# joyfang1106/MRLA

Hardware: AMD Instinct MI355X
Metric: images/sec fwd+bwd resnet50_mrlal b=256 (higher is better)
Workload: dtype bf16

## Files before the change

### include/mrla_hip.h

```cpp
#ifndef MRLA_HIP_H_
#define MRLA_HIP_H_

#include <stddef.h>
#include <stdint.h>

#ifdef __cplusplus
extern "C" {
#endif

#define MRLA_OK 0
#define MRLA_EINVAL (-1)
#define MRLA_EUNSUPPORTED (-2)
#define MRLA_EHIP (-3)

enum { MRLA_F32 = 0, MRLA_BF16 = 1, MRLA_F16 = 2 };
enum { MRLA_NCHW = 0, MRLA_NHWC = 1 };
enum { MRLA_ACT_NONE = 0, MRLA_ACT_GELU = 1 };
enum { MRLA_BN_NONE = 0, MRLA_BN_TRAIN = 1, MRLA_BN_EVAL = 2 };

#define MRLA_FWD_MOMENTS 8
#define MRLA_BWD_MOMENTS 3
#define MRLA_GEMM_MOMENTS 4

#define MRLA_ABI_VERSION 5
int mrla_abi_version(void);

int mrla_light_wgrad_rows(int b, int c, int h, int w, int dtype, int layout);

int mrla_light_mom_splits(int b, int c, int h, int w, int dtype, int layout);
int mrla_tuning_row_ranges(int mode);
int mrla_light_stats_fwd(const void* x, const void* o_prev, const float* wv , float* mom,
                         int b, int c, int h, int w, int dtype, int layout, int act, void* stream);

int mrla_light_stats_fwd_fused(const void* pre, const float* pre_sc, const float* pre_sh, const void* o_prev,
                               const float* wv, float* mom, void* x_out, int b, int c, int h, int w, int dtype,
                               int layout, void* stream);

int mrla_light_pool_fused(const void* pre, const float* pre_sc, const float* pre_sh, const void* o_prev, float* part,
                          float* mom, int b, int c, int h, int w, int dtype, int layout, void* stream);
int mrla_light_apply_fwd_fused(const void* pre, const float* pre_sc, const float* pre_sh, const void* o_prev,
                               const float* wv, const float* gate, const float* sc, const float* sh, const float* lam,
                               const float* dp, void* out, int b, int c, int h, int w, int d, int res, int dtype,
                               int layout, void* stream);

int mrla_light_gate_fwd(const float* mom, const float* wq, const float* wk, int ksize, float* gate ,
                        int b, int c, int hw, int d, void* stream);

int mrla_light_bn_fwd(const float* mom, const float* gate, const float* lam, const float* gamma, const float* beta,
                      float* running_mean, float* running_var, int bn_mode, float momentum, float eps, float* sc,
                      float* sh, float* save_mean, float* save_inv, int b, int c, int hw, int d, void* stream);

int mrla_light_apply_fwd(const void* x, const void* o_prev, const float* wv, const float* gate, const float* sc,
                         const float* sh, const float* lam, const float* dp, void* out, int b, int c, int h, int w,
                         int d, int res, int dtype, int layout, int act, void* stream);

int mrla_light_bmom_splits(int b, int c, int h, int w, int dtype, int layout);
int mrla_light_stats_bwd(const void* dout, const void* x, const void* o_prev, const float* wv, const float* mom,
                         float* bmom, int b, int c, int h, int w, int dtype, int layout, int act, void* stream);

int mrla_light_bn_bwd(const float* mom, const float* bmom, const float* gate, const float* lam, const float* gamma,
                      const float* dp, const float* save_mean, const float* save_inv, int bn_mode, float* cb,
                      float* cb_lo, float* dgamma, float* dbeta, float* dlam, int b, int c, int hw, int d,
                      void* stream);

int mrla_light_gate_bwd(const float* mom, const float* bmom, const float* gate, const float* cb, const float* cb_lo,
                        const float* dp,
                        const float* wq, const float* wk, int ksize, float* dyx, float* dwqk_part, int b, int c,
                        int hw, int d, void* stream);

int mrla_light_apply_bwd_pre_sums(int b, int c, int h, int w, int dtype, int layout);
int mrla_light_apply_bwd(const void* dout, const void* x, const void* o_prev, const float* wv, const float* gate,
                         const float* cb, const float* lam, const float* dp, const float* dyx, void* dx,
                         void* do_prev, float* dwv_part, const void* pre, const float* pre_center, float* pre_tmom, int b,
                         int c, int h, int w, int d, int res, int relu_mask, int dtype, int layout, int act, void* stream);

int mrla_light_lean_supported(int b, int c, int h, int w, int dtype, int layout);
int mrla_light_stats_bwd_fused(const void* dout, const void* pre, const float* pre_sc, const float* pre_sh,
                               const void* o_prev, const float* wv, const float* mom, float* bmom, int b, int c, int h, int w,
                               int dtype, int layout, void* stream);
int mrla_light_apply_bwd_fused(const void* dout, const void* pre, const float* pre_sc, const float* pre_sh,
                               const void* o_prev, const float* wv, const float* gate, const float* cb, const float* lam,
                               const float* dp, const float* dyx, void* dx, void* do_prev, float* dwv_part,
                               const float* pre_center, float* pre_tmom, int b, int c, int h, int w, int d, int res,
                               int dtype, int layout, void* stream);


int mrla_base_gate_fwd(const float* mom, const float* wq, const float* wk, int ksize, float* k_ring, float* p_all,
                       float* q , int b, int c, int hw, int d, int T, int t, void* stream);

int mrla_base_attend_fwd(const void* x, const float* wv, void* v_ring, const float* p_all, void* attn, float* amom,
                         int b, int c, int h, int w, int d, int T, int t, int dtype, int layout, void* stream);

int mrla_bn_stats_fwd(const float* amom, const float* pivot, const float* gamma, const float* beta, float* running_mean,
                      float* running_var, int bn_mode, float momentum, float eps, float* sc, float* sh,
                      float* save_mean, float* save_inv, int b, int c, int hw, void* stream);

int mrla_bn_stats_fwd_rows(const float* rec, const float* gamma, const float* beta, float* running_mean, float* running_var,
                           int bn_mode, float momentum, float eps, float* sc, float* sh, float* save_mean, float* save_inv,
                           int rows, int c, void* stream);

int mrla_base_tail_fwd(const void* x, const void* attn, const float* sc, const float* sh, const float* dp, void* out,
                       int b, int c, int h, int w, int dtype, int layout, void* stream);

int mrla_base_tail_stats_bwd(const void* dout, const void* attn, const float* sc, const float* sh, const float* center,
                             const float* dp, float* tmom, int b, int c, int h, int w, int dtype, int layout, void* stream);

int mrla_bn_stats_bwd(const float* tmom, const float* gamma, const float* save_mean, const float* save_inv,
                      int bn_mode, int centered, float* cb, float* dgamma, float* dbeta, int b, int c, int hw, void* stream);

int mrla_base_attend_bwd(const void* dout, const void* attn, const float* sc, const float* sh, const float* dp,
                         const float* cb, const void* v_ring, void* da_ring, float* pmom, int b, int c, int h, int w,
                         int T, int t, int dtype, int layout, void* stream);

int mrla_base_gate_bwd(const float* mom, const float* pmom, const float* p_all, const float* q, const float* k_ring,
                       float* dk_ring, const float* wq, const float* wk, int ksize, float* dyx, float* dwqk_part,
                       int b, int c, int hw, int d, int T, int t, int first_touch, void* stream);

int mrla_base_value_bwd(const void* dout, const void* x, const float* wv, const void* da_ring, const float* p_all,
                        const float* dyx, void* dx, float* dwv_part, int b, int c, int h, int w, int d, int T, int t,
                        int Tc, int res, int dtype, int layout, void* stream);

int mrla_base_tile_rows(int b, int c, int h, int w, int dtype, int layout);
int mrla_base_pmom_rows(int b, int c, int h, int w, int dtype, int layout);

int mrla_base_pool_value_fwd(const void* x, const float* pre_sc, const float* pre_sh, const void* identity,
                             const float* wv, float* mom, void* x_out, void* v_slot, int b, int c, int h, int w,
                             int dtype, int layout, void* stream);

int mrla_base_pmom_reduce(const float* part, float* pmom, int b, int c, int t, int rows, void* stream);

int mrla_base_dv_combine(const void* da_ring, const float* p_all, void* dv, int b, int c, int h, int w, int d, int T,
                         int t, int Tc, int dtype, int layout, void* stream);

int mrla_base_value_bwd_pre_sums(int b, int c, int h, int w, int dtype, int layout);
int mrla_base_value_bwd_dv(const void* dout, const void* x, const float* wv, const void* dv, const float* dyx, void* dx,
                           float* dwv_part, const void* pre, const float* pre_center, float* pre_tmom, int b, int c, int h,
                           int w, int res, int dtype, int layout, void* stream);

#define MRLA_TOKEN_PARTIALS 15

int mrla_token_norm_pool(const void* x, const void* o_prev, const float* lnx_w, const float* lnx_b, float eps,
                         float* stats, float* mom, int b, int n, int c, int dtype, void* stream);

int mrla_token_apply_fwd(const void* x, const void* o_prev, const float* stats, const float* lnx_w,
                         const float* lnx_b, const float* lno_w, const float* lno_b, const float* wv,
                         const float* gate, const float* lam, void* out, int b, int n, int c, int d, int res,
                         int dtype, void* stream);

int mrla_token_part_rows(int b, int n, int c, int dtype);
int mrla_token_apply_bwd(const void* dout, const void* x, const void* o_prev, const float* stats, const float* lnx_w,
                         const float* lnx_b, const float* lno_w, const float* lno_b, const float* wv,
                         const float* gate, const float* lam, float* dxn, float* part, float* bmom, int b, int n, int c,
                         int d, int dtype, void* stream);
int mrla_token_gate_bwd(const float* mom, const float* bmom, const float* gate, const float* wq, const float* wk,
                        int ksize, float* dyx, float* dwqk_part, float* part, int b, int n, int c, int d, int dtype,
                        void* stream);
int mrla_token_ln_bwd(const void* dout, const void* x, const void* o_prev, const float* dxn, const float* dyx,
                      const float* stats, const float* lnx_w, const float* lno_w, const float* lam, void* dx,
                      void* do_prev, int b, int n, int c, int res, int dtype, void* stream);

int mrla_token_base_supported(int b, int n, int c, int dtype);
int mrla_token_base_value_fwd(const void* x, const float* stats, const float* lnx_w, const float* lnx_b, const float* wv,
                              void* v_slot, int b, int n, int c, int dtype, void* stream);
int mrla_token_base_attend_fwd(const void* v_ring, const float* p_all, const void* x, const float* stats,
                               const float* lnx_w, const float* lnx_b, void* out, float* amom, int b, int n, int c, int d,
                               int T, int t, int dtype, void* stream);
int mrla_token_base_attend_bwd(const void* dout, const void* v_ring, void* da_ring, float* pmom_part, int b, int n, int c,
                               int T, int t, int dtype, void* stream);
int mrla_token_base_gate_bwd(const float* mom, const float* pmom, const float* p_all, const float* q, const float* k_ring,
                             float* dk_ring, const float* wq, const float* wk, int ksize, float* dyx, float* dwqk_part,
                             float* part, int b, int n, int c, int d, int T, int t, int first_touch, int dtype,
                             void* stream);
int mrla_token_base_value_bwd(const void* dout, const void* x, const float* stats, const float* lnx_w, const float* lnx_b,
                              const float* wv, const void* dv, float* dxn, float* part, int b, int n, int c, int dtype,
                              void* stream);

int mrla_bn_moment_rows(int b, int c, int h, int w, int layout);
int mrla_bn_plane_moments(const void* x, float* amom , float* pivot, int b, int c, int h, int w,
                          int dtype, int layout, void* stream);
int mrla_bn_act_fwd(const void* x, const float* sc, const float* sh, int relu, void* y, int b, int c, int h, int w,
                    int dtype, int layout, void* stream);
int mrla_bn_plane_dmoments(const void* dy, const void* x, const float* sc, const float* sh, const float* center, int relu,
                           float* tmom , int b, int c, int h, int w, int dtype,
                           int layout, void* stream);
int mrla_bn_act_bwd(const void* dy, const void* x, const float* sc, const float* sh, const float* cb , int relu,
                    void* dx, int b, int c, int h, int w, int dtype, int layout, void* stream);

int mrla_bn_pool_rows(int b, int c, int h, int w, int dtype, int layout);
int mrla_bn_relu_pool_fwd(const void* x, const float* sc, const float* sh, void* out, int b, int c, int h, int w, int dtype,
                          int layout, void* stream);
int mrla_bn_relu_pool_dmoments(const void* dp, const void* x, const float* sc, const float* sh, const float* center ,
                               float* tmom, int b, int c, int h, int w, int dtype, int layout, void* stream);
int mrla_bn_relu_pool_bwd(const void* dp, const void* x, const float* sc, const float* sh, const float* cb ,
                          void* dx, int b, int c, int h, int w, int dtype, int layout, void* stream);

int mrla_conv1x1_rows(int m, int k, int n, int dtype);
int mrla_conv1x1_plan(int m, int k, int n, int dtype, int addend, int* out);
int mrla_conv1x1_fwd(const void* x, const void* w, void* y, float* mom_part, int m, int k, int n, int dtype, void* stream);

int mrla_conv1x1_add_supported(int m, int k, int n, int dtype);
int mrla_conv1x1_fwd_add(const void* x, const void* w, const void* addend, void* y, int m, int k, int n, int dtype,
                         void* stream);

int mrla_conv1x1_addend_supported(int m, int k, int n, int sh, int sw, int dtype);
int mrla_conv1x1_fwd_addend(const void* x, const void* w, const void* addend, void* y, int m, int k, int n, int b, int h,
                            int w_, int sh, int sw, int dtype, void* stream);

int mrla_conv1x1_wgrad_rows(int m, int k, int n, int dtype);
int mrla_conv1x1_wgrad_plan(int m, int k, int n, int dtype, int* out);
int mrla_conv1x1_wgrad(const void* dy, const void* x, float* part, void* dw, int m, int k, int n, int dtype, int dw_dtype,
                       void* stream);

int mrla_weight_bank_refresh(const void* table, int entries, int max_tiles, void* stream);
int mrla_weight_bank_refresh_dt(const void* table, int entries, int max_tiles, int dtype, void* stream);

int mrla_reduce_rows(const float* in, float* out, int rows, int n, void* stream);
int mrla_reduce_rows2(const float* in1, float* out1, int rows1, int n1, const float* in2, float* out2, int rows2, int n2,
                      void* stream);



int mrla_light_tail_fwd(const void* x, const float* pre_sc, const float* pre_sh, const void* o_prev, const float* wq,
                        const float* wk, int ksize, const float* wv, const float* lam, const float* gamma,
                        const float* beta, float* running_mean, float* running_var, int bn_mode, float momentum, float eps,
                        const float* dp, float* mom, void* x_out, float* gate, float* bnbuf, void* out, int b, int c,
                        int h, int w, int d, int res, int fuse, int dtype, int layout, int act, void* stream);

int mrla_light_tail_bwd(const void* dout, const void* x, const void* o_prev, const float* wq, const float* wk, int ksize,
                        const float* wv, const float* lam, const float* gamma, const float* dp, const float* mom,
                        const float* gate, const float* bnbuf, int bn_mode, float* bmom, float* small, float* dyx,
                        float* dwqk_part, float* dwv_part, int rows, void* dx, void* do_prev, const void* pre,
                        const float* pre_sc, const float* pre_sh, const float* pre_center, float* pre_tmom, float* wsum,
                        int b, int c, int h, int w, int d, int res, int relu_mask, int dtype, int layout, int act,
                        void* stream);

int mrla_bn_fwd(const void* x, const float* records, int rec_rows, float* amom, float* pivot, int rows, const float* gamma,
                const float* beta, float* running_mean, float* running_var, int bn_mode, float momentum, float eps,
                float* bnbuf, int relu, void* y, int b, int c, int h, int w, int dtype, int layout, void* stream);

int mrla_bn_bwd(const void* dy, const void* x, const float* gamma, const float* bnbuf, float* tmom, int rows, int have_tmom,
                int bn_mode, int relu, float* small, void* dx, int b, int c, int h, int w, int dtype, int layout,
                void* stream);

int mrla_stem_fwd(const void* x, float* amom, float* pivot, int rows, const float* gamma, const float* beta,
                  float* running_mean, float* running_var, int bn_mode, float momentum, float eps, float* bnbuf, void* out,
                  int b, int c, int h, int w, int dtype, int layout, void* stream);
int mrla_stem_bwd(const void* dp, const void* x, const float* gamma, const float* bnbuf, float* tmom, int rows, int bn_mode,
                  float* small, void* dx, int b, int c, int h, int w, int dtype, int layout, void* stream);

int mrla_base_layer_fwd(const void* x, const float* pre_sc, const float* pre_sh, const void* identity, const float* wq,
                        const float* wk, int ksize, const float* wv, const float* gamma, const float* beta,
                        float* running_mean, float* running_var, int bn_mode, float momentum, float eps, const float* dp,
                        float* mom, void* x_out, void* v_ring, float* k_ring, float* p_all, float* q, void* attn,
                        float* amom, int arows, float* bnbuf, void* out, int tail, int b, int c, int h, int w, int d, int T,
                        int t, int dtype, void* stream);

int mrla_base_layer_bwd(const void* dout, const void* x, const void* attn, const float* wq, const float* wk, int ksize,
                        const float* wv, const float* gamma, const float* dp, const float* mom, const float* q,
                        const float* bnbuf, int bn_mode, const void* v_ring, void* da_ring, const float* k_ring,
                        float* dk_ring, const float* p_all, float* tmom, int trows, float* small, float* ppart, int prows,
                        float* pmom, float* dyx, float* dwqk_part, void* dv, float* dwv_part, int rows, void* dx,
                        const void* pre, const float* pre_center, float* pre_tmom, float* wsum, int tail, int first_touch,
                        int res, int b, int c, int h, int w, int d, int T, int t, int Tc, int dtype, void* stream);

int mrla_token_light_fwd(const void* x, const void* o_prev, const float* lnx_w, const float* lnx_b, const float* lno_w,
                         const float* lno_b, const float* wq, const float* wk, int ksize, const float* wv,
                         const float* lam, float eps, float* stats, float* mom, float* gate, void* out, int b, int n, int c,
                         int d, int res, int dtype, void* stream);

int mrla_token_light_bwd(const void* dout, const void* x, const void* o_prev, const float* stats, const float* lnx_w,
                         const float* lnx_b, const float* lno_w, const float* lno_b, const float* wq, const float* wk,
                         int ksize, const float* wv, const float* gate, const float* lam, const float* mom, float* dxn,
                         float* part, int prow, float* bmom, float* dyx, float* dwqk_part, void* dx, void* do_prev,
                         float* sums, int b, int n, int c, int d, int res, int dtype, void* stream);

#ifdef __cplusplus
}
#endif
#endif
```

### mrla_amd/_lib.py

```python
import ctypes
import os

_HERE = os.path.dirname(os.path.abspath(__file__))
LIB_PATH = os.environ.get("MRLA_HIP_LIB") or os.path.join(_HERE, "libmrla_hip.so")

ABI_VERSION = 5
OK, EINVAL, EUNSUPPORTED, EHIP = 0, -1, -2, -3
F32, BF16, F16 = 0, 1, 2
NCHW, NHWC = 0, 1
ACT_NONE, ACT_GELU = 0, 1
BN_NONE, BN_TRAIN, BN_EVAL = 0, 1, 2
FWD_MOMENTS, BWD_MOMENTS, TOKEN_PARTIALS, GEMM_MOMENTS = 8, 3, 15, 4

_ERR = {EINVAL: "invalid argument", EUNSUPPORTED: "unsupported shape/layout for the HIP kernels",
        EHIP: "HIP runtime error at kernel launch"}

_P, _I, _F = ctypes.c_void_p, ctypes.c_int, ctypes.c_float

SIGNATURES = {
    "mrla_abi_version": [],
    "mrla_light_wgrad_rows": [_I] * 6,
    "mrla_light_stats_fwd": [_P, _P, _P, _P, _I, _I, _I, _I, _I, _I, _I, _P],
    "mrla_light_gate_fwd": [_P, _P, _P, _I, _P, _I, _I, _I, _I, _P],
    "mrla_light_bn_fwd": [_P, _P, _P, _P, _P, _P, _P, _I, _F, _F, _P, _P, _P, _P, _I, _I, _I, _I, _P],
    "mrla_light_apply_fwd": [_P, _P, _P, _P, _P, _P, _P, _P, _P, _I, _I, _I, _I, _I, _I, _I, _I, _I, _P],
    "mrla_light_stats_bwd": [_P, _P, _P, _P, _P, _P, _I, _I, _I, _I, _I, _I, _I, _P],
    "mrla_light_bmom_splits": [_I] * 6,
    "mrla_light_mom_splits": [_I] * 6,
    "mrla_tuning_row_ranges": [_I],
    "mrla_light_bn_bwd": [_P, _P, _P, _P, _P, _P, _P, _P, _I, _P, _P, _P, _P, _P, _I, _I, _I, _I, _P],
    "mrla_light_gate_bwd": [_P, _P, _P, _P, _P, _P, _P, _P, _I, _P, _P, _I, _I, _I, _I, _P],
    "mrla_light_apply_bwd_pre_sums": [_I] * 6,
    "mrla_light_apply_bwd": [_P] * 15 + [_I] * 10 + [_P],
    "mrla_light_lean_supported": [_I] * 6,
    "mrla_light_stats_bwd_fused": [_P] * 8 + [_I] * 6 + [_P],
    "mrla_light_apply_bwd_fused": [_P] * 16 + [_I] * 8 + [_P],
    "mrla_light_pool_fused": [_P] * 6 + [_I] * 6 + [_P],
    "mrla_light_apply_fwd_fused": [_P] * 11 + [_I] * 8 + [_P],
    "mrla_light_stats_fwd_fused": [_P, _P, _P, _P, _P, _P, _P, _I, _I, _I, _I, _I, _I, _P],
    "mrla_base_tile_rows": [_I] * 6,
    "mrla_base_pmom_rows": [_I] * 6,
    "mrla_base_pool_value_fwd": [_P] * 8 + [_I] * 6 + [_P],
    "mrla_base_pmom_reduce": [_P, _P, _I, _I, _I, _I, _P],
    "mrla_base_dv_combine": [_P, _P, _P] + [_I] * 10 + [_P],
    "mrla_base_value_bwd_pre_sums": [_I] * 6,
    "mrla_base_value_bwd_dv": [_P] * 10 + [_I] * 7 + [_P],
    "mrla_base_gate_fwd": [_P, _P, _P, _I, _P, _P, _P, _I, _I, _I, _I, _I, _I, _P],
    "mrla_base_attend_fwd": [_P, _P, _P, _P, _P, _P] + [_I] * 9 + [_P],
    "mrla_bn_stats_fwd": [_P, _P, _P, _P, _P, _P, _I, _F, _F, _P, _P, _P, _P, _I, _I, _I, _P],
    "mrla_bn_stats_fwd_rows": [_P, _P, _P, _P, _P, _I, _F, _F, _P, _P, _P, _P, _I, _I, _P],
    "mrla_base_tail_fwd": [_P, _P, _P, _P, _P, _P, _I, _I, _I, _I, _I, _I, _P],
    "mrla_base_tail_stats_bwd": [_P, _P, _P, _P, _P, _P, _P, _I, _I, _I, _I, _I, _I, _P],
    "mrla_bn_stats_bwd": [_P, _P, _P, _P, _I, _I, _P, _P, _P, _I, _I, _I, _P],
    "mrla_base_attend_bwd": [_P] * 9 + [_I] * 8 + [_P],
    "mrla_base_gate_bwd": [_P, _P, _P, _P, _P, _P, _P, _P, _I, _P, _P] + [_I] * 7 + [_P],
    "mrla_base_value_bwd": [_P] * 8 + [_I] * 11 + [_P],
    "mrla_token_norm_pool": [_P, _P, _P, _P, _F, _P, _P, _I, _I, _I, _I, _P],
    "mrla_token_apply_fwd": [_P] * 11 + [_I] * 6 + [_P],
    "mrla_token_part_rows": [_I] * 4,
    "mrla_token_apply_bwd": [_P] * 14 + [_I] * 5 + [_P],
    "mrla_token_gate_bwd": [_P] * 5 + [_I] + [_P] * 3 + [_I] * 5 + [_P],
    "mrla_token_ln_bwd": [_P] * 11 + [_I] * 5 + [_P],
    "mrla_token_base_supported": [_I] * 4,
    "mrla_token_base_value_fwd": [_P] * 6 + [_I] * 4 + [_P],
    "mrla_token_base_attend_fwd": [_P] * 8 + [_I] * 7 + [_P],
    "mrla_token_base_attend_bwd": [_P] * 4 + [_I] * 6 + [_P],
    "mrla_token_base_gate_bwd": [_P] * 8 + [_I] + [_P] * 3 + [_I] * 8 + [_P],
    "mrla_token_base_value_bwd": [_P] * 9 + [_I] * 4 + [_P],
    "mrla_bn_moment_rows": [_I] * 5,
    "mrla_bn_plane_moments": [_P, _P, _P, _I, _I, _I, _I, _I, _I, _P],
    "mrla_bn_act_fwd": [_P, _P, _P, _I, _P, _I, _I, _I, _I, _I, _I, _P],
    "mrla_bn_plane_dmoments": [_P, _P, _P, _P, _P, _I, _P, _I, _I, _I, _I, _I, _I, _P],
    "mrla_bn_act_bwd": [_P, _P, _P, _P, _P, _I, _P, _I, _I, _I, _I, _I, _I, _P],
    "mrla_bn_pool_rows": [_I] * 6,
    "mrla_bn_relu_pool_fwd": [_P, _P, _P, _P, _I, _I, _I, _I, _I, _I, _P],
    "mrla_bn_relu_pool_dmoments": [_P, _P, _P, _P, _P, _P, _I, _I, _I, _I, _I, _I, _P],
    "mrla_bn_relu_pool_bwd": [_P, _P, _P, _P, _P, _P, _I, _I, _I, _I, _I, _I, _P],
    "mrla_conv1x1_rows": [_I] * 4,
    "mrla_conv1x1_plan": [_I, _I, _I, _I, _I, _P],
    "mrla_conv1x1_wgrad_plan": [_I, _I, _I, _I, _P],
    "mrla_conv1x1_fwd": [_P, _P, _P, _P, _I, _I, _I, _I, _P],
    "mrla_conv1x1_add_supported": [_I] * 4,
    "mrla_conv1x1_fwd_add": [_P, _P, _P, _P, _I, _I, _I, _I, _P],
    "mrla_conv1x1_addend_supported": [_I] * 6,
    "mrla_conv1x1_fwd_addend": [_P, _P, _P, _P] + [_I] * 9 + [_P],
    "mrla_conv1x1_wgrad_rows": [_I] * 4,
    "mrla_conv1x1_wgrad": [_P, _P, _P, _P, _I, _I, _I, _I, _I, _P],
    "mrla_weight_bank_refresh": [_P, _I, _I, _P],
    "mrla_weight_bank_refresh_dt": [_P, _I, _I, _I, _P],
    "mrla_reduce_rows": [_P, _P, _I, _I, _P],
    "mrla_reduce_rows2": [_P, _P, _I, _I, _P, _P, _I, _I, _P],
    "mrla_light_tail_fwd": [_P] * 6 + [_I] + [_P] * 6 + [_I, _F, _F] + [_P] * 6 + [_I] * 10 + [_P],
    "mrla_light_tail_bwd": [_P] * 5 + [_I] + [_P] * 7 + [_I] + [_P] * 5 + [_I] + [_P] * 8 + [_I] * 10 + [_P],
    "mrla_bn_fwd": [_P, _P, _I, _P, _P, _I, _P, _P, _P, _P, _I, _F, _F, _P, _I, _P] + [_I] * 6 + [_P],
    "mrla_bn_bwd": [_P] * 5 + [_I] * 4 + [_P, _P] + [_I] * 6 + [_P],
    "mrla_stem_fwd": [_P, _P, _P, _I, _P, _P, _P, _P, _I, _F, _F, _P, _P] + [_I] * 6 + [_P],
    "mrla_stem_bwd": [_P] * 5 + [_I, _I, _P, _P] + [_I] * 6 + [_P],
    "mrla_base_layer_fwd": [_P] * 6 + [_I] + [_P] * 5 + [_I, _F, _F] + [_P] * 9 + [_I] + [_P, _P] + [_I] * 9 + [_P],
    "mrla_base_layer_bwd": ([_P] * 5 + [_I] + [_P] * 6 + [_I] + [_P] * 6 + [_I] + [_P, _P] + [_I] + [_P] * 5 + [_I] + [_P] * 5
                            + [_I] * 12 + [_P]),
    "mrla_token_light_fwd": [_P] * 8 + [_I] + [_P, _P] + [_F] + [_P] * 4 + [_I] * 6 + [_P],
    "mrla_token_light_bwd": [_P] * 10 + [_I] + [_P] * 6 + [_I] + [_P] * 6 + [_I] * 6 + [_P],
}


class MrlaHipError(RuntimeError):
    pass


_lib = None


def load():
    global _lib
    if _lib is not None:
        return _lib
    if not os.path.exists(LIB_PATH):
        raise MrlaHipError(
            f"{LIB_PATH} not found: the MRLA HIP extension is not built. Run `python -c 'import __graft_entry__ as g; "
            "g.build()'` (or `make -C mrla_amd/csrc`) -- mrla_amd has no CPU/PyTorch fallback for its operators.")
    import torch
    lib = ctypes.CDLL(LIB_PATH)
    for name, argtypes in SIGNATURES.items():
        fn = getattr(lib, name)
        fn.argtypes = argtypes
        fn.restype = ctypes.c_int
    if lib.mrla_abi_version() != ABI_VERSION:
        raise MrlaHipError(f"libmrla_hip.so reports ABI version {lib.mrla_abi_version()}, this binding is written against "
                           f"{ABI_VERSION} (MRLA_ABI_VERSION of include/mrla_hip.h); rebuild it")
    _lib = lib
    return lib


def check(rc, what):
    if rc != OK:
        raise MrlaHipError(f"{what}: {_ERR.get(rc, 'error')} (code {rc})")


def conv1x1_plan(m, k, n, addend=False, dtype=None):
    out = (ctypes.c_int * 4)()
    rc = load().mrla_conv1x1_plan(m, k, n, BF16 if dtype is None else dtype, int(addend), ctypes.cast(out, ctypes.c_void_p))
    return tuple(out) if rc == OK else None


def conv1x1_wgrad_plan(m, k, n, dtype=None):
    out = (ctypes.c_int * 6)()
    rc = load().mrla_conv1x1_wgrad_plan(m, k, n, BF16 if dtype is None else dtype, ctypes.cast(out, ctypes.c_void_p))
    return tuple(out) if rc == OK else None


def call(name, *args):
    rc = getattr(load(), name)(*args)
    check(rc, name)
```

### mrla_amd/csrc/bnact_nhwc.hip

```cpp
#include <algorithm>

#include "mrla_device.h"
#include "mrla_kernels.h"

#ifndef MRLA_REVERSE_AFFINE
#define MRLA_REVERSE_AFFINE 1
#endif

namespace mrla {

template <typename T> struct V16 { typedef T type __attribute__((ext_vector_type(16 / sizeof(T)))); };

template <typename T>
__device__ __forceinline__ void ld16(const T* __restrict__ p, float (&v)[16 / sizeof(T)]) {
  typedef typename V16<T>::type VT;
  const VT t = *reinterpret_cast<const VT*>(p);
#pragma unroll
  for (int i = 0; i < (int)(16 / sizeof(T)); ++i) v[i] = static_cast<float>(t[i]);
}
template <typename T>
__device__ __forceinline__ void st16(T* __restrict__ p, const float (&v)[16 / sizeof(T)]) {
  typedef typename V16<T>::type VT;
  VT t;
#pragma unroll
  for (int i = 0; i < (int)(16 / sizeof(T)); ++i) t[i] = static_cast<T>(v[i]);
  *reinterpret_cast<VT*>(p) = t;
}

template <typename T, int MODE>
__global__ __launch_bounds__(kThreads) void nhwc_moments_kernel(const T* __restrict__ x, const T* __restrict__ dy,
                                                                const float* __restrict__ sc, const float* __restrict__ sh,
                                                                int relu, float* __restrict__ out ,
                                                                float* __restrict__ pivot, int C, int HW, int nsplit) {
  constexpr int VEC = 16 / sizeof(T);
  constexpr int LPC = 64 / VEC;
  constexpr int PPW = kWave / LPC;
  __shared__ float red[kWaves][2][64];
  const int lane = threadIdx.x & (kWave - 1), wave = threadIdx.x / kWave;
  const int cl = (lane % LPC) * VEC;
  const int c0 = blockIdx.x * 64 + cl;
  const bool cv = c0 < C;
  const int bs = blockIdx.y, b = bs / nsplit, sp = bs - b * nsplit;
  const int npix = HW / nsplit;
  const size_t base = ((size_t)b * HW + (size_t)sp * npix) * C;
  float scv[VEC], shv[VEC];
#pragma unroll
  for (int i = 0; i < VEC; ++i) { scv[i] = (MODE && relu && cv) ? sc[c0 + i] : 0.f; shv[i] = (MODE && relu && cv) ? sh[c0 + i] : 0.f; }
  float s1[VEC], s2[VEC], pv[VEC];
#pragma unroll
  for (int i = 0; i < VEC; ++i) { s1[i] = 0.f; s2[i] = 0.f; pv[i] = 0.f; }
  if (MODE == 0 && pivot && cv) {
    ld16<T>(x + c0, pv);
    if (bs == 0 && wave == 0 && lane < LPC) {
#pragma unroll
      for (int i = 0; i < VEC; ++i) pivot[c0 + i] = pv[i];
    }
  }
  if (MODE == 1 && pivot && cv) {
#pragma unroll
    for (int i = 0; i < VEC; ++i) pv[i] = pivot[c0 + i];
  }
  if (cv) {
    for (int p = wave * PPW + lane / LPC; p < npix; p += kWaves * PPW) {
      float xv[VEC];
      ld16<T>(x + base + (size_t)p * C + c0, xv);
      if (MODE == 0) {
#pragma unroll
        for (int i = 0; i < VEC; ++i) { const float d = xv[i] - pv[i]; s1[i] += d; s2[i] = fmaf(d, d, s2[i]); }
      } else {
        float gv[VEC];
        ld16<T>(dy + base + (size_t)p * C + c0, gv);
#pragma unroll
        for (int i = 0; i < VEC; ++i) {
          const float dz = (!relu || fmaf(scv[i], xv[i], shv[i]) > 0.f) ? gv[i] : 0.f;
          s1[i] += dz;
          s2[i] = fmaf(dz, xv[i] - pv[i], s2[i]);
        }
      }
    }
  }
#pragma unroll
  for (int i = 0; i < VEC; ++i) {
    for (int off = LPC; off < kWave; off <<= 1) {
      s1[i] += __shfl_xor(s1[i], off, kWave);
      s2[i] += __shfl_xor(s2[i], off, kWave);
    }
  }
  if (lane < LPC) {
#pragma unroll
    for (int i = 0; i < VEC; ++i) { red[wave][0][cl + i] = s1[i]; red[wave][1][cl + i] = s2[i]; }
  }
  __syncthreads();
  if (threadIdx.x < 128) {
    const int k = threadIdx.x / 64, ch = threadIdx.x % 64;
    const int c = blockIdx.x * 64 + ch;
    if (c < C) {
      float s = 0.f;
#pragma unroll
      for (int wv = 0; wv < kWaves; ++wv) s += red[wv][k][ch];
      out[((size_t)bs * C + c) * 2 + k] = s;
    }
  }
}

template <typename T, bool BWD>
__global__ __launch_bounds__(kThreads) void nhwc_affine_kernel(const T* __restrict__ x, const T* __restrict__ dy,
                                                               const float* __restrict__ a, const float* __restrict__ sc,
                                                               const float* __restrict__ sh, int relu, T* __restrict__ out,
                                                               size_t total, int C) {
  constexpr int VEC = 16 / sizeof(T);
  const size_t stride = (size_t)gridDim.x * kThreads * VEC;
  const size_t first = ((size_t)blockIdx.x * kThreads + threadIdx.x) * VEC;
  const bool fixed = (stride % C) == 0;
  float scv[VEC], shv[VEC], ev[VEC], fv[VEC], hv[VEC];
  auto load_coef = [&](int c0) {
#pragma unroll
    for (int i = 0; i < VEC; ++i) {
      scv[i] = sc[c0 + i]; shv[i] = sh[c0 + i];
      if (BWD) { ev[i] = a[(c0 + i) * 3]; fv[i] = a[(c0 + i) * 3 + 1]; hv[i] = a[(c0 + i) * 3 + 2]; }
    }
  };
  if (fixed && first < total) load_coef((int)(first % C));
  for (size_t e0 = first; e0 < total; e0 += stride) {
    if (!fixed) load_coef((int)(e0 % C));
    float xv[VEC], gv[VEC], y[VEC];
    ld16<T>(x + e0, xv);
    if (BWD) ld16<T>(dy + e0, gv);
#pragma unroll
    for (int i = 0; i < VEC; ++i) {
      const float z = fmaf(scv[i], xv[i], shv[i]);
      if (!BWD) y[i] = relu ? fmaxf(z, 0.f) : z;
      else {
        const float dz = (!relu || z > 0.f) ? gv[i] : 0.f;
        y[i] = fmaf(ev[i], dz, fmaf(fv[i], xv[i], hv[i]));
      }
    }
    st16<T>(out + e0, y);
  }
}

constexpr int kUnr = 4;

template <int N>
__device__ __forceinline__ void ldf(const float* __restrict__ p, float (&v)[N]) {
  static_assert(N % 4 == 0, "vector loads of 4 floats");
#pragma unroll
  for (int i = 0; i < N; i += 4) {
    const float4 t = *reinterpret_cast<const float4*>(p + i);
    v[i] = t.x; v[i + 1] = t.y; v[i + 2] = t.z; v[i + 3] = t.w;
  }
}

template <typename T, int MODE>
__global__ __launch_bounds__(kThreads) void nhwc_moments_flat_kernel(const T* __restrict__ x, const T* __restrict__ dy,
                                                                     const float* __restrict__ sc,
                                                                     const float* __restrict__ sh, int relu,
                                                                     const float* __restrict__ dp ,
                                                                     float* __restrict__ out, float* __restrict__ pivot,
                                                                     int C, int HW, int nsplit, int CW) {
  constexpr int VEC = 16 / sizeof(T);
  __shared__ float red[2][kThreads * VEC];
  const int t = threadIdx.x;
  const int lpc = CW / VEC;
  const int ppi = kThreads / lpc;
  const int cl = (t & (lpc - 1)) * VEC, ps = t / lpc;
  const int c0 = blockIdx.x * CW + cl;
  const int bs = blockIdx.y, b = bs / nsplit, sp = bs - b * nsplit;
  const int npix = HW / nsplit;
  const float dpb = (MODE && dp) ? dp[b] : 1.f;
  const T* xp = x + ((size_t)b * HW + (size_t)sp * npix) * C + c0;
  const T* gp = MODE ? dy + ((size_t)b * HW + (size_t)sp * npix) * C + c0 : nullptr;
  float scv[VEC], shv[VEC];
  if ((MODE == 1 && relu) || (MODE == 2 && sc)) { ldf<VEC>(sc + c0, scv); ldf<VEC>(sh + c0, shv); }
  else {
#pragma unroll
    for (int i = 0; i < VEC; ++i) { scv[i] = 0.f; shv[i] = 0.f; }
  }
  float s1[VEC], s2[VEC], pv[VEC];
#pragma unroll
  for (int i = 0; i < VEC; ++i) { s1[i] = 0.f; s2[i] = 0.f; pv[i] = 0.f; }
  if (MODE == 0 && pivot) {
    ld16<T>(x + c0, pv);
    if (bs == 0 && ps == 0) {
#pragma unroll
      for (int i = 0; i < VEC; ++i) pivot[c0 + i] = pv[i];
    }
  }
  if (MODE == 1 && pivot) ldf<VEC>(pivot + c0, pv);
  auto accumulate = [&](const float (&xv)[VEC], const float (&gv)[VEC]) {
#pragma unroll
    for (int i = 0; i < VEC; ++i) {
      if (MODE == 0) { const float d = xv[i] - pv[i]; s1[i] += d; s2[i] = fmaf(d, d, s2[i]); }
      else if (MODE == 2) {
        const float z = sc ? to_f(from_f<T>(fmaf(scv[i], xv[i], shv[i]))) : xv[i];
        s1[i] += fmaxf(to_f(from_f<T>(z + gv[i])), 0.f);
      } else {
        const float dz = (!relu || fmaf(scv[i], xv[i], shv[i]) > 0.f) ? dpb * gv[i] : 0.f;
        s1[i] += dz;
        s2[i] = fmaf(dz, xv[i] - pv[i], s2[i]);
      }
    }
  };
  constexpr int UN = MODE ? kUnr : 2 * kUnr;
  int p = ps;
  for (; p + (UN - 1) * ppi < npix; p += UN * ppi) {
    float xv[UN][VEC], gv[UN][VEC];
#pragma unroll
    for (int u = 0; u < UN; ++u) {
      ld16<T>(xp + (size_t)(p + u * ppi) * C, xv[u]);
      if (MODE) ld16<T>(gp + (size_t)(p + u * ppi) * C, gv[u]);
    }
#pragma unroll
    for (int u = 0; u < UN; ++u) accumulate(xv[u], gv[u]);
  }
  for (; p < npix; p += ppi) {
    float xv[VEC], gv[VEC];
    ld16<T>(xp + (size_t)p * C, xv);
    if (MODE) ld16<T>(gp + (size_t)p * C, gv);
    accumulate(xv, gv);
  }
#pragma unroll
  for (int i = 0; i < VEC; ++i) { red[0][t * VEC + i] = s1[i]; red[1][t * VEC + i] = s2[i]; }
  __syncthreads();
  for (int j = t; j < 2 * CW; j += kThreads) {
    const int k = j / CW, ch = j - k * CW;
    float sum = 0.f;
    for (int r = 0; r < ppi; ++r) sum += red[k][r * CW + ch];
    out[((size_t)bs * C + blockIdx.x * CW + ch) * 2 + k] = sum;
  }
}

__global__ __launch_bounds__(kThreads) void nhwc_pool_finish_kernel(const float* __restrict__ part ,
                                                                    float* __restrict__ mom , int BC, int C,
                                                                    int ns) {
  const int i = blockIdx.x * kThreads + threadIdx.x;
  if (i >= BC) return;
  const int b = i / C, c = i - b * C;
  float s = 0.f;
  for (int k = 0; k < ns; ++k) s += part[(((size_t)b * ns + k) * C + c) * 2];
  mom[(size_t)i * M_REC] = s;
}

template <typename T, bool BWD>
__global__ __launch_bounds__(kThreads) void nhwc_affine_flat_kernel(const T* __restrict__ x, const T* __restrict__ dy,
                                                                    const float* __restrict__ a,
                                                                    const float* __restrict__ sc,
                                                                    const float* __restrict__ sh, int relu,
                                                                    T* __restrict__ out, size_t total, int C, int iters) {
  constexpr int VEC = 16 / sizeof(T);
  constexpr size_t STEP = (size_t)kThreads * VEC;
  const int c0 = (int)((threadIdx.x * VEC) & (unsigned)(C - 1));
  float scv[VEC], shv[VEC], cbv[BWD ? 3 * VEC : 4];
  ldf<VEC>(sc + c0, scv);
  ldf<VEC>(sh + c0, shv);
  if constexpr (BWD) ldf<3 * VEC>(a + (size_t)c0 * 3, cbv);
  const size_t bx = MRLA_REVERSE_AFFINE ? gridDim.x - 1 - blockIdx.x : blockIdx.x;
  size_t e = bx * iters * STEP + (size_t)threadIdx.x * VEC;
  auto one = [&](const float (&xv)[VEC], const float (&gv)[VEC], size_t at) {
    float y[VEC];
#pragma unroll
    for (int i = 0; i < VEC; ++i) {
      const float z = fmaf(scv[i], xv[i], shv[i]);
      if (!BWD) y[i] = relu ? fmaxf(z, 0.f) : z;
      else {
        const float dz = (!relu || z > 0.f) ? gv[i] : 0.f;
        y[i] = fmaf(cbv[3 * i], dz, fmaf(cbv[3 * i + 1], xv[i], cbv[3 * i + 2]));
      }
    }
    st16<T>(out + at, y);
  };
  int it = 0;
  for (; it + kUnr <= iters && e + (kUnr - 1) * STEP < total; it += kUnr, e += kUnr * STEP) {
    float xv[kUnr][VEC], gv[kUnr][VEC];
#pragma unroll
    for (int u = 0; u < kUnr; ++u) {
      ld16<T>(x + e + u * STEP, xv[u]);
      if (BWD) ld16<T>(dy + e + u * STEP, gv[u]);
    }
#pragma unroll
    for (int u = 0; u < kUnr; ++u) one(xv[u], gv[u], e + u * STEP);
  }
  for (; it < iters && e < total; ++it, e += STEP) {
    float xv[VEC], gv[VEC];
    ld16<T>(x + e, xv);
    if (BWD) ld16<T>(dy + e, gv);
    one(xv, gv, e);
  }
}

int nhwc_bn_splits(int B, int C, int HW) {
  (void)C;
  static const int cand[] = {1, 2, 4, 7, 8, 14, 16, 28, 32, 49, 56, 64};
  int best = 1;
  for (int s : cand) {
    if (HW % s || (s > 1 && HW / s < 16)) continue;
    best = s;
    if ((long)B * s >= 1024) break;
  }
  return best;
}

static int flat_cw(int C, int vec) {
  if (C % 64) return 0;
  int cw = 64;
  while (cw * 2 <= kThreads * vec && C % (cw * 2) == 0) cw *= 2;
  return cw;
}

#define MRLA_DISPATCH_N(DT, CALL)        \
  switch (DT) {                          \
    case MRLA_F32:  CALL(float); break;  \
    case MRLA_BF16: CALL(bf16_t); break; \
    case MRLA_F16:  CALL(f16_t); break;  \
    default: return MRLA_EINVAL;         \
  }

int launch_nhwc_moments(const void* x, const void* dy, const float* sc, const float* sh, int relu, const float* dp,
                        float* out, float* pivot, int B, int C, int HW, int dtype, int mode, hipStream_t st) {
  const int vec = 16 / (int)dtype_size(dtype);
  if (C % vec) return MRLA_EUNSUPPORTED;
  const int ns = nhwc_bn_splits(B, C, HW);
  const int cw = flat_cw(C, vec);
  if (cw) {
    const dim3 fgrid(C / cw, B * ns);
#define CALL(TT)                                                                                                       \
  if (mode) hipLaunchKernelGGL((nhwc_moments_flat_kernel<TT, 1>), fgrid, dim3(kThreads), 0, st, (const TT*)x,          \
                               (const TT*)dy, sc, sh, relu, dp, out, pivot, C, HW, ns, cw);                            \
  else      hipLaunchKernelGGL((nhwc_moments_flat_kernel<TT, 0>), fgrid, dim3(kThreads), 0, st, (const TT*)x,          \
                               (const TT*)dy, sc, sh, relu, dp, out, pivot, C, HW, ns, cw);
    MRLA_DISPATCH_N(dtype, CALL)
#undef CALL
    return hip_status(hipGetLastError());
  }
  if (dp) return MRLA_EUNSUPPORTED;
  const dim3 grid((C + 63) / 64, B * ns);
#define CALL(TT)                                                                                                     \
  if (mode) hipLaunchKernelGGL((nhwc_moments_kernel<TT, 1>), grid, dim3(kThreads), 0, st, (const TT*)x, (const TT*)dy, \
                               sc, sh, relu, out, pivot, C, HW, ns);                                                 \
  else      hipLaunchKernelGGL((nhwc_moments_kernel<TT, 0>), grid, dim3(kThreads), 0, st, (const TT*)x, (const TT*)dy, \
                               sc, sh, relu, out, pivot, C, HW, ns);
  MRLA_DISPATCH_N(dtype, CALL)
#undef CALL
  return hip_status(hipGetLastError());
}

int launch_nhwc_pool_fused(const void* pre, const float* sc, const float* sh, const void* o, float* part, float* mom,
                           int B, int C, int HW, int dtype, hipStream_t st) {
  const int vec = 16 / (int)dtype_size(dtype);
  const int cw = flat_cw(C, vec);
  if (!cw) return MRLA_EUNSUPPORTED;
  const int ns = nhwc_bn_splits(B, C, HW);
  const dim3 fgrid(C / cw, B * ns);
#define CALL(TT)                                                                                                 \
  hipLaunchKernelGGL((nhwc_moments_flat_kernel<TT, 2>), fgrid, dim3(kThreads), 0, st, (const TT*)pre, (const TT*)o, \
                     sc, sh, 0, (const float*)nullptr, part, (float*)nullptr, C, HW, ns, cw);
  MRLA_DISPATCH_N(dtype, CALL)
#undef CALL
  hipLaunchKernelGGL(nhwc_pool_finish_kernel, dim3((B * C + kThreads - 1) / kThreads), dim3(kThreads), 0, st, part, mom,
                     B * C, C, ns);
  return hip_status(hipGetLastError());
}

int launch_nhwc_affine(const void* x, const void* dy, const float* a, const float* sc, const float* sh, int relu,
                       void* out, int B, int C, int HW, int dtype, int bwd, hipStream_t st) {
  const size_t total = (size_t)B * C * HW;
  const int vec = 16 / (int)dtype_size(dtype);
  if (C % vec) return MRLA_EUNSUPPORTED;
  const size_t want = (total / vec + kThreads - 1) / kThreads;
  if ((C & (C - 1)) == 0 && C >= vec && C <= kThreads * vec) {
    const int iters = (int)std::max<size_t>(1, std::min<size_t>((want + 4095) / 4096, 64));
    const int fgrid = (int)((want + iters - 1) / iters);
#define CALL(TT)                                                                                                       \
  if (bwd) hipLaunchKernelGGL((nhwc_affine_flat_kernel<TT, true>), dim3(fgrid), dim3(kThreads), 0, st, (const TT*)x,   \
                              (const TT*)dy, a, sc, sh, relu, (TT*)out, total, C, iters);                              \
  else     hipLaunchKernelGGL((nhwc_affine_flat_kernel<TT, false>), dim3(fgrid), dim3(kThreads), 0, st, (const TT*)x,  \
                              (const TT*)dy, a, sc, sh, relu, (TT*)out, total, C, iters);
    MRLA_DISPATCH_N(dtype, CALL)
#undef CALL
    return hip_status(hipGetLastError());
  }
  const int grid = (int)std::max<size_t>(1, std::min<size_t>(want, 256 * 16));
#define CALL(TT)                                                                                                   \
  if (bwd) hipLaunchKernelGGL((nhwc_affine_kernel<TT, true>), dim3(grid), dim3(kThreads), 0, st, (const TT*)x,     \
                              (const TT*)dy, a, sc, sh, relu, (TT*)out, total, C);                                 \
  else     hipLaunchKernelGGL((nhwc_affine_kernel<TT, false>), dim3(grid), dim3(kThreads), 0, st, (const TT*)x,    \
                              (const TT*)dy, a, sc, sh, relu, (TT*)out, total, C);
  MRLA_DISPATCH_N(dtype, CALL)
#undef CALL
  return hip_status(hipGetLastError());
}

}
```

### mrla_amd/csrc/capi.hip

```cpp
#include <algorithm>
#include <atomic>
#include <mutex>

#include "mrla_device.h"
#include "mrla_kernels.h"

namespace mrla {

hipError_t lds_opt_in(const void* kernel, size_t bytes) {
  if (bytes <= 48 * 1024) return hipSuccess;
  constexpr unsigned kSlots = 1024;
  static std::atomic<uintptr_t> keys[kSlots];
  static std::atomic<int> granted[kSlots];
  static std::mutex raise_mutex;
  int dev = 0;
  if (hipGetDevice(&dev) != hipSuccess) return hipErrorInvalidDevice;
  const uintptr_t key = reinterpret_cast<uintptr_t>(kernel) ^ ((uintptr_t)(dev + 1) << 52);
  unsigned i = (unsigned)((key >> 4) * 0x9E3779B1u) % kSlots;
  int slot = -1;
  for (unsigned probe = 0; probe < kSlots; ++probe, i = (i + 1) % kSlots) {
    uintptr_t k = keys[i].load(std::memory_order_acquire);
    if (k == 0 && keys[i].compare_exchange_strong(k, key, std::memory_order_acq_rel)) k = key;
    if (k == key) { slot = (int)i; break; }
  }
// ... 392 lines not shown

int mrla_base_pmom_rows(int b, int c, int h, int w, int dtype, int layout) {
  if (bad_dims(b, c, h, w) || bad_dtype(dtype)) return MRLA_EINVAL;
  if (layout == MRLA_NCHW) return b;
  if (layout != MRLA_NHWC) return MRLA_EINVAL;
  if (!base_nhwc_supported(c, dtype)) return MRLA_EUNSUPPORTED;
  return b * base_nhwc_pmom_tiles(b, c, h * w, dtype);
}

int mrla_base_pool_value_fwd(const void* x, const float* pre_sc, const float* pre_sh, const void* identity,
                             const float* wv, float* mom, void* x_out, void* v_slot, int b, int c, int h, int w,
                             int dtype, int layout, void* stream) {
  if (!x || !wv || !mom || !v_slot || bad_dims(b, c, h, w) || bad_dtype(dtype)) return MRLA_EINVAL;
  if ((identity == nullptr) != (x_out == nullptr)) return MRLA_EINVAL;
  if ((pre_sc == nullptr) != (pre_sh == nullptr) || (pre_sc && !identity)) return MRLA_EINVAL;
  if (layout != MRLA_NHWC) return MRLA_EUNSUPPORTED;
  return launch_light_stats_fwd_nhwc(x, identity, wv, mom, x_out, pre_sc, pre_sh, v_slot, b, c, h, w, dtype,
                                     MRLA_ACT_NONE, (hipStream_t)stream);
}

int mrla_base_pmom_reduce(const float* part, float* pmom, int b, int c, int t, int rows, void* stream) {
  if (!part || !pmom || b <= 0 || c <= 0 || t <= 0 || rows <= 0 || rows % b) return MRLA_EINVAL;
  return launch_base_pmom_reduce(part, pmom, b, c, t, rows / b, (hipStream_t)stream);
}

int mrla_base_dv_combine(const void* da_ring, const float* p_all, void* dv, int b, int c, int h, int w, int d, int T,
                         int t, int Tc, int dtype, int layout, void* stream) {
  if (!da_ring || !p_all || !dv || bad_dims(b, c, h, w) || bad_dtype(dtype) || d <= 0 || c % d || bad_ring(T, t) ||
      Tc < t || Tc > T)
    return MRLA_EINVAL;
  if (layout != MRLA_NHWC) return MRLA_EUNSUPPORTED;
  return launch_base_dv_combine_nhwc(da_ring, p_all, dv, b, c, h * w, d, T, t, Tc, dtype, (hipStream_t)stream);
}

int mrla_base_value_bwd_pre_sums(int b, int c, int h, int w, int dtype, int layout) {
  if (bad_dims(b, c, h, w) || bad_dtype(dtype)) return MRLA_EINVAL;
  if (layout != MRLA_NHWC && layout != MRLA_NCHW) return MRLA_EINVAL;
  return (layout == MRLA_NHWC && c % kWave == 0) ? 1 : MRLA_EUNSUPPORTED;
}

int mrla_base_value_bwd_dv(const void* dout, const void* x, const float* wv, const void* dv, const float* dyx, void* dx,
                           float* dwv_part, const void* pre, const float* pre_center, float* pre_tmom, int b, int c, int h,
                           int w, int res, int dtype, int layout, void* stream) {
  if (!dout || !x || !wv || !dv || !dyx || !dx || !dwv_part || bad_dims(b, c, h, w) || bad_dtype(dtype))
    return MRLA_EINVAL;
  if ((pre == nullptr) != (pre_tmom == nullptr) || (pre_tmom && !(res & 2))) return MRLA_EINVAL;
  if (layout != MRLA_NHWC) return MRLA_EUNSUPPORTED;
  if (c % kWave == 0)
    return launch_base_value_bwd_wide(dout, x, wv, dv, dyx, dx, dwv_part, pre, pre_center, pre_tmom, b, c, h, w, res, dtype,
                                      (hipStream_t)stream);
  return launch_base_value_bwd_nhwc(dout, x, wv, dv, dyx, dx, dwv_part, pre, pre_center, pre_tmom, b, c, h, w, res, dtype,
                                    (hipStream_t)stream);
}

static int token_side(int n) {
  if (n < 2) return 0;
  int s = 1;
  while ((s + 1) * (s + 1) <= n - 1) ++s;
  return s * s == n - 1 ? s : 0;
}

int mrla_token_norm_pool(const void* x, const void* o_prev, const float* lnx_w, const float* lnx_b, float eps,
                         float* stats, float* mom, int b, int n, int c, int dtype, void* stream) {
  if (!x || !lnx_w || !lnx_b || !stats || !mom || b <= 0 || c <= 0 || bad_dtype(dtype) || !token_side(n))
    return MRLA_EINVAL;
  return launch_token_norm_pool(x, o_prev, lnx_w, lnx_b, eps, stats, mom, b, n, c, dtype, (hipStream_t)stream);
}

int mrla_token_apply_fwd(const void* x, const void* o_prev, const float* stats, const float* lnx_w,
                         const float* lnx_b, const float* lno_w, const float* lno_b, const float* wv,
                         const float* gate, const float* lam, void* out, int b, int n, int c, int d, int res,
                         int dtype, void* stream) {
  if (!x || !o_prev || !stats || !lnx_w || !lnx_b || !lno_w || !lno_b || !wv || !gate || !lam || !out || b <= 0 ||
      c <= 0 || d <= 0 || c % d || bad_dtype(dtype) || !token_side(n))
    return MRLA_EINVAL;
  return launch_token_apply_fwd(x, o_prev, stats, lnx_w, lnx_b, lno_w, lno_b, wv, gate, lam, out, b, n, c,
                                token_side(n), d, res, dtype, (hipStream_t)stream);
}

int mrla_token_part_rows(int b, int n, int c, int dtype) {
  if (b <= 0 || c <= 0 || bad_dtype(dtype) || !token_side(n)) return MRLA_EINVAL;
  return b * token_bands_bwd(b, c, token_side(n));
}

int mrla_token_apply_bwd(const void* dout, const void* x, const void* o_prev, const float* stats, const float* lnx_w,
                         const float* lnx_b, const float* lno_w, const float* lno_b, const float* wv,
                         const float* gate, const float* lam, float* dxn, float* part, float* bmom, int b, int n, int c,
                         int d, int dtype, void* stream) {
  if (!dout || !x || !o_prev || !stats || !lnx_w || !lnx_b || !lno_w || !lno_b || !wv || !gate || !lam || !dxn ||
      !part || !bmom || b <= 0 || c <= 0 || d <= 0 || c % d || bad_dtype(dtype) || !token_side(n))
    return MRLA_EINVAL;
  return launch_token_apply_bwd(dout, x, o_prev, stats, lnx_w, lnx_b, lno_w, lno_b, wv, gate, lam, dxn, part, bmom, b, n,
                                c, token_side(n), d, dtype, (hipStream_t)stream);
}

int mrla_token_gate_bwd(const float* mom, const float* bmom, const float* gate, const float* wq, const float* wk,
                        int ksize, float* dyx, float* dwqk_part, float* part, int b, int n, int c, int d, int dtype,
                        void* stream) {
  if (!mom || !bmom || !gate || !wq || !wk || !dyx || !dwqk_part || !part || b <= 0 || c <= 0 || d <= 0 || c % d ||
      ksize <= 0 || !(ksize & 1) || bad_dtype(dtype) || !token_side(n))
    return MRLA_EINVAL;
  return launch_gate_bwd(mom, bmom, gate, nullptr, nullptr, nullptr, wq, wk, ksize, dyx, dwqk_part, b, c, n - 1, d,
                         (hipStream_t)stream, part, token_bands_bwd(b, c, token_side(n)));
}

int mrla_token_ln_bwd(const void* dout, const void* x, const void* o_prev, const float* dxn, const float* dyx,
                      const float* stats, const float* lnx_w, const float* lno_w, const float* lam, void* dx,
                      void* do_prev, int b, int n, int c, int res, int dtype, void* stream) {
  if (!dout || !x || !dxn || !stats || !lnx_w || !dx || b <= 0 || c <= 0 || bad_dtype(dtype) || !token_side(n) ||
      (o_prev && (!lno_w || !lam || !do_prev)))
    return MRLA_EINVAL;
  return launch_token_ln_bwd(dout, x, o_prev, dxn, dyx, stats, lnx_w, lno_w, lam, dx, do_prev, b, n, c, res, dtype,
                             (hipStream_t)stream);
}

int mrla_token_base_supported(int b, int n, int c, int dtype) {
  if (b <= 0 || c <= 0 || bad_dtype(dtype) || !token_side(n)) return MRLA_EINVAL;
  return (token_nhwc_applies(c) && base_nhwc_supported(c, dtype)) ? 1 : 0;
}

int mrla_token_base_value_fwd(const void* x, const float* stats, const float* lnx_w, const float* lnx_b, const float* wv,
                              void* v_slot, int b, int n, int c, int dtype, void* stream) {
  if (!x || !stats || !lnx_w || !lnx_b || !wv || !v_slot || b <= 0 || c <= 0 || bad_dtype(dtype) || !token_side(n))
    return MRLA_EINVAL;
  return launch_token_value_fwd_nhwc(x, stats, lnx_w, lnx_b, wv, v_slot, b, n, c, token_side(n), dtype,
                                     (hipStream_t)stream);
}

int mrla_token_base_attend_fwd(const void* v_ring, const float* p_all, const void* x, const float* stats,
                               const float* lnx_w, const float* lnx_b, void* out, float* amom, int b, int n, int c, int d,
                               int T, int t, int dtype, void* stream) {
  if (!v_ring || !p_all || !x || !stats || !lnx_w || !lnx_b || !out || !amom || b <= 0 || c <= 0 || d <= 0 || c % d ||
      bad_dtype(dtype) || !token_side(n) || bad_ring(T, t))
    return MRLA_EINVAL;
  const int rc = launch_base_attend_fwd_nhwc(v_ring, p_all, out, amom, b, c, n - 1, d, T, t, dtype, (hipStream_t)stream, c, c);
  if (rc != MRLA_OK) return rc;
  return launch_token_cls_fwd(x, stats, lnx_w, lnx_b, out, b, n, c, dtype, (hipStream_t)stream);
}

int mrla_token_base_attend_bwd(const void* dout, const void* v_ring, void* da_ring, float* pmom_part, int b, int n, int c,
                               int T, int t, int dtype, void* stream) {
  if (!dout || !v_ring || !da_ring || !pmom_part || b <= 0 || c <= 0 || bad_dtype(dtype) || !token_side(n) || bad_ring(T, t))
    return MRLA_EINVAL;
  return launch_base_attend_bwd_nhwc(dout, nullptr, nullptr, nullptr, nullptr, nullptr, v_ring, da_ring, pmom_part, b, c,
                                     n - 1, T, t, dtype, (hipStream_t)stream, c, c);
}

int mrla_token_base_gate_bwd(const float* mom, const float* pmom, const float* p_all, const float* q, const float* k_ring,
                             float* dk_ring, const float* wq, const float* wk, int ksize, float* dyx, float* dwqk_part,
                             float* part, int b, int n, int c, int d, int T, int t, int first_touch, int dtype,
                             void* stream) {
  if (!mom || !pmom || !p_all || !q || !k_ring || !dk_ring || !wq || !wk || !dyx || !dwqk_part || !part || b <= 0 ||
      c <= 0 || d <= 0 || c % d || ksize <= 0 || !(ksize & 1) || bad_dtype(dtype) || !token_side(n) || bad_ring(T, t))
    return MRLA_EINVAL;
  return launch_base_gate_bwd(mom, pmom, p_all, q, k_ring, dk_ring, wq, wk, ksize, dyx, dwqk_part, b, c, n - 1, d, T, t,
                              first_touch, (hipStream_t)stream, part, token_bands_bwd(b, c, token_side(n)));
}

int mrla_token_base_value_bwd(const void* dout, const void* x, const float* stats, const float* lnx_w, const float* lnx_b,
                              const float* wv, const void* dv, float* dxn, float* part, int b, int n, int c, int dtype,
                              void* stream) {
  if (!dout || !x || !stats || !lnx_w || !lnx_b || !wv || !dv || !dxn || !part || b <= 0 || c <= 0 || bad_dtype(dtype) ||
      !token_side(n))
    return MRLA_EINVAL;
  return launch_token_value_bwd_nhwc(dout, x, stats, lnx_w, lnx_b, wv, dv, dxn, part, b, n, c, token_side(n), dtype,
                                     (hipStream_t)stream);
}

int mrla_bn_plane_moments(const void* x, float* amom, float* pivot, int b, int c, int h, int w, int dtype, int layout,
                          void* stream) {
  if (!x || !amom || bad_dims(b, c, h, w) || bad_dtype(dtype)) return MRLA_EINVAL;
  if (layout == MRLA_NHWC)
    return launch_nhwc_moments(x, nullptr, nullptr, nullptr, 0, nullptr, amom, pivot, b, c, h * w, dtype, 0,
                               (hipStream_t)stream);
  if (layout != MRLA_NCHW) return MRLA_EINVAL;
  return launch_plane_moments(x, amom, pivot, b, c, h * w, dtype, (hipStream_t)stream);
}

int mrla_bn_act_fwd(const void* x, const float* sc, const float* sh, int relu, void* y, int b, int c, int h, int w,
                    int dtype, int layout, void* stream) {
  if (!x || !sc || !sh || !y || bad_dims(b, c, h, w) || bad_dtype(dtype)) return MRLA_EINVAL;
  if (layout == MRLA_NHWC)
    return launch_nhwc_affine(x, nullptr, nullptr, sc, sh, relu, y, b, c, h * w, dtype, 0, (hipStream_t)stream);
  if (layout != MRLA_NCHW) return MRLA_EINVAL;
  return launch_affine_act(x, nullptr, nullptr, sc, sh, relu, y, b, c, h * w, dtype, 0, (hipStream_t)stream);
}

int mrla_bn_plane_dmoments(const void* dy, const void* x, const float* sc, const float* sh, const float* center, int relu,
                           float* tmom, int b, int c, int h, int w, int dtype, int layout, void* stream) {
  if (!dy || !x || !sc || !sh || !tmom || bad_dims(b, c, h, w) || bad_dtype(dtype)) return MRLA_EINVAL;
  if (layout == MRLA_NHWC)
    return launch_nhwc_moments(x, dy, sc, sh, relu, nullptr, tmom, const_cast<float*>(center), b, c, h * w, dtype, 1,
                               (hipStream_t)stream);
  if (layout != MRLA_NCHW) return MRLA_EINVAL;
  return launch_plane_dmoments(dy, x, sc, sh, center, relu, tmom, b, c, h * w, dtype, (hipStream_t)stream);
}

int mrla_bn_act_bwd(const void* dy, const void* x, const float* sc, const float* sh, const float* cb, int relu,
                    void* dx, int b, int c, int h, int w, int dtype, int layout, void* stream) {
  if (!dy || !x || !sc || !sh || !cb || !dx || bad_dims(b, c, h, w) || bad_dtype(dtype)) return MRLA_EINVAL;
  if (layout == MRLA_NHWC)
    return launch_nhwc_affine(x, dy, cb, sc, sh, relu, dx, b, c, h * w, dtype, 1, (hipStream_t)stream);
  if (layout != MRLA_NCHW) return MRLA_EINVAL;
  return launch_affine_act(x, dy, cb, sc, sh, relu, dx, b, c, h * w, dtype, 1, (hipStream_t)stream);
}

int mrla_bn_pool_rows(int b, int c, int h, int w, int dtype, int layout) {
  if (bad_dims(b, c, h, w) || bad_dtype(dtype)) return MRLA_EINVAL;
  if (layout != MRLA_NHWC) return layout == MRLA_NCHW ? MRLA_EUNSUPPORTED : MRLA_EINVAL;
  return bn_pool_rows(b, c, h, w);
}

int mrla_bn_relu_pool_fwd(const void* x, const float* sc, const float* sh, void* out, int b, int c, int h, int w, int dtype,
                          int layout, void* stream) {
  if (!x || !sc || !sh || !out || bad_dims(b, c, h, w) || bad_dtype(dtype)) return MRLA_EINVAL;
  if (layout != MRLA_NHWC) return layout == MRLA_NCHW ? MRLA_EUNSUPPORTED : MRLA_EINVAL;
  return launch_bn_relu_pool_fwd(x, sc, sh, out, b, c, h, w, dtype, (hipStream_t)stream);
}

int mrla_bn_relu_pool_dmoments(const void* dp, const void* x, const float* sc, const float* sh, const float* center,
                               float* tmom, int b, int c, int h, int w, int dtype, int layout, void* stream) {
  if (!dp || !x || !sc || !sh || !tmom || bad_dims(b, c, h, w) || bad_dtype(dtype)) return MRLA_EINVAL;
  if (layout != MRLA_NHWC) return layout == MRLA_NCHW ? MRLA_EUNSUPPORTED : MRLA_EINVAL;
  return launch_bn_relu_pool_dmoments(dp, x, sc, sh, center, tmom, b, c, h, w, dtype, (hipStream_t)stream);
}

int mrla_bn_relu_pool_bwd(const void* dp, const void* x, const float* sc, const float* sh, const float* cb, void* dx, int b,
                          int c, int h, int w, int dtype, int layout, void* stream) {
  if (!dp || !x || !sc || !sh || !cb || !dx || bad_dims(b, c, h, w) || bad_dtype(dtype)) return MRLA_EINVAL;
  if (layout != MRLA_NHWC) return layout == MRLA_NCHW ? MRLA_EUNSUPPORTED : MRLA_EINVAL;
  return launch_bn_relu_pool_bwd(dp, x, sc, sh, cb, dx, b, c, h, w, dtype, (hipStream_t)stream);
}

int mrla_conv1x1_rows(int m, int k, int n, int dtype) {
  if (m <= 0 || k <= 0 || n <= 0 || bad_dtype(dtype)) return MRLA_EINVAL;
  if (dtype != MRLA_BF16 && dtype != MRLA_F16) return MRLA_EUNSUPPORTED;
  return conv1x1_rows(m, k, n);
}

int mrla_conv1x1_plan(int m, int k, int n, int dtype, int addend, int* out) {
  if (m <= 0 || k <= 0 || n <= 0 || bad_dtype(dtype) || !out) return MRLA_EINVAL;
  if (dtype != MRLA_BF16 && dtype != MRLA_F16) return MRLA_EUNSUPPORTED;
  return conv1x1_plan(m, k, n, addend, out);
}

int mrla_conv1x1_wgrad_plan(int m, int k, int n, int dtype, int* out) {
  if (m <= 0 || k <= 0 || n <= 0 || bad_dtype(dtype) || !out) return MRLA_EINVAL;
  if (dtype != MRLA_BF16 && dtype != MRLA_F16) return MRLA_EUNSUPPORTED;
  return conv1x1_wgrad_plan(m, k, n, out);
}

int mrla_conv1x1_fwd(const void* x, const void* w, void* y, float* mom_part, int m, int k, int n, int dtype, void* stream) {
  if (!x || !w || !y || m <= 0 || k <= 0 || n <= 0 || bad_dtype(dtype)) return MRLA_EINVAL;
  if (dtype != MRLA_BF16 && dtype != MRLA_F16) return MRLA_EUNSUPPORTED;
  return launch_conv1x1_fwd(x, w, y, mom_part, m, k, n, dtype, (hipStream_t)stream);
}

int mrla_conv1x1_add_supported(int m, int k, int n, int dtype) {
  if (m <= 0 || k <= 0 || n <= 0 || bad_dtype(dtype)) return MRLA_EINVAL;
  if (dtype != MRLA_BF16 && dtype != MRLA_F16) return MRLA_EUNSUPPORTED;
  return conv1x1_wide_rows(m, k, n) > 0 ? 1 : MRLA_EUNSUPPORTED;
}

int mrla_conv1x1_fwd_add(const void* x, const void* w, const void* addend, void* y, int m, int k, int n, int dtype,
                         void* stream) {
  if (!x || !w || !addend || !y || m <= 0 || k <= 0 || n <= 0 || bad_dtype(dtype)) return MRLA_EINVAL;
  if (dtype != MRLA_BF16 && dtype != MRLA_F16) return MRLA_EUNSUPPORTED;
  return launch_conv1x1_wide(x, w, addend, y, nullptr, m, k, n, dtype, (hipStream_t)stream);
}

static bool bad_addend_geometry(int m, int b, int h, int w, int sh, int sw) {
  return b <= 0 || h <= 0 || w <= 0 || sh <= 0 || sw <= 0 || (long long)b * h * w != (long long)m;
}

int mrla_conv1x1_addend_supported(int m, int k, int n, int sh, int sw, int dtype) {
  if (m <= 0 || k <= 0 || n <= 0 || sh <= 0 || sw <= 0 || bad_dtype(dtype)) return MRLA_EINVAL;
  if (dtype != MRLA_BF16 && dtype != MRLA_F16) return MRLA_EUNSUPPORTED;
  return conv1x1_addend_supported(m, k, n) ? 1 : MRLA_EUNSUPPORTED;
}

int mrla_conv1x1_fwd_addend(const void* x, const void* w, const void* addend, void* y, int m, int k, int n, int b, int h,
                            int w_, int sh, int sw, int dtype, void* stream) {
  if (!x || !w || !addend || !y || m <= 0 || k <= 0 || n <= 0 || bad_dtype(dtype) || bad_addend_geometry(m, b, h, w_, sh, sw))
    return MRLA_EINVAL;
  if (dtype != MRLA_BF16 && dtype != MRLA_F16) return MRLA_EUNSUPPORTED;
  return launch_conv1x1_addend(x, w, addend, y, m, k, n, b, h, w_, sh, sw, dtype, (hipStream_t)stream);
}

int mrla_conv1x1_wgrad_rows(int m, int k, int n, int dtype) {
  if (m <= 0 || k <= 0 || n <= 0 || bad_dtype(dtype)) return MRLA_EINVAL;
  if (dtype != MRLA_BF16 && dtype != MRLA_F16) return MRLA_EUNSUPPORTED;
  return conv1x1_wgrad_rows(m, k, n);
}

int mrla_conv1x1_wgrad(const void* dy, const void* x, float* part, void* dw, int m, int k, int n, int dtype, int dw_dtype,
                       void* stream) {
  if (!dy || !x || !part || !dw || m <= 0 || k <= 0 || n <= 0 || bad_dtype(dtype)) return MRLA_EINVAL;
  if (dw_dtype != MRLA_BF16 && dw_dtype != MRLA_F16 && dw_dtype != MRLA_F32) return MRLA_EINVAL;
  if ((dw_dtype == MRLA_F16 && dtype != MRLA_F16) || (dw_dtype == MRLA_BF16 && dtype == MRLA_F16)) return MRLA_EINVAL;
  if (dtype != MRLA_BF16 && dtype != MRLA_F16) return MRLA_EUNSUPPORTED;
  return launch_conv1x1_wgrad(dy, x, part, dw, dw_dtype == MRLA_F32, m, k, n, dtype, (hipStream_t)stream);
}

int mrla_weight_bank_refresh(const void* table, int entries, int max_tiles, void* stream) {
  if (!table || entries <= 0 || max_tiles <= 0) return MRLA_EINVAL;
  return launch_weight_bank_refresh((const long long*)table, entries, max_tiles, MRLA_BF16, (hipStream_t)stream);
}

int mrla_weight_bank_refresh_dt(const void* table, int entries, int max_tiles, int dtype, void* stream) {
  if (!table || entries <= 0 || max_tiles <= 0 || bad_dtype(dtype)) return MRLA_EINVAL;
  if (dtype != MRLA_BF16 && dtype != MRLA_F16) return MRLA_EUNSUPPORTED;
  return launch_weight_bank_refresh((const long long*)table, entries, max_tiles, dtype, (hipStream_t)stream);
}

int mrla_reduce_rows(const float* in, float* out, int rows, int n, void* stream) {
  if (!in || !out || rows <= 0 || n <= 0) return MRLA_EINVAL;
  return launch_reduce_rows(in, out, rows, n, (hipStream_t)stream);
}

int mrla_reduce_rows2(const float* in1, float* out1, int rows1, int n1, const float* in2, float* out2, int rows2, int n2,
                      void* stream) {
  if (!in1 || !out1 || !in2 || !out2 || rows1 <= 0 || n1 <= 0 || rows2 <= 0 || n2 <= 0) return MRLA_EINVAL;
  return launch_reduce_rows2(in1, out1, rows1, n1, in2, out2, rows2, n2, (hipStream_t)stream);
}

}
```

### mrla_amd/csrc/conv1x1_wgrad.hip

```cpp
#include <algorithm>

#include "conv1x1_elem.h"
#include "mrla_device.h"
#include "mrla_kernels.h"

namespace mrla {
namespace {

typedef short wg_s16x4 __attribute__((ext_vector_type(4)));
typedef c1_f32x16 wg_f32x16;
typedef __attribute__((address_space(3))) wg_s16x4* lds_s16x4_ptr;

constexpr int kPC = 32;
constexpr int kWgStages = 4;
constexpr int kWgWaves = 4;
#define MRLA_WG_FLAGS 0x00020000
constexpr int kWgTarget = 256;

template <int TN, int TK, int PC>
struct WgGeo {
  static constexpr int WN = (TN >= 256 && TK <= 64) ? 4 : (TK >= 256 && TN <= 64) ? 1 : 2;
  static constexpr int WK = kWgWaves / WN;
  static constexpr int WTN = TN / WN, WTK = TK / WK;
  static constexpr int BN = WTN / 32, BK = WTK / 32;
  static constexpr int NIY = TN / 64 * (PC / 32), NIX = TK / 64 * (PC / 32);
  static constexpr int YB = PC * TN * 2, XB = PC * TK * 2;
  static constexpr int SB = YB + XB;
  static_assert(BN >= 1 && BK >= 1 && BN * BK <= 8, "wave tile");
};

template <int CPR>
__device__ __forceinline__ int swz(int row) { return CPR >= 16 ? ((row & 3) << 2) : (((row >> 1) & 1) << 2); }

template <int CPR>
__device__ __forceinline__ int tr_offset(int lane, int row0, int ch0) {
  const int g = lane >> 4, q = (lane >> 2) & 3, p = lane & 3;
  const int row = row0 + 8 * (g >> 1) + q;
  const int col = ch0 + 16 * (g & 1) + 4 * p;
  return row * (CPR * 16) + ((((col >> 3) ^ swz<CPR>(row))) << 4) + ((col >> 2) & 1) * 8;
}

struct Frag {
  wg_s16x4 lo, hi;
};
template <int CPR>
__device__ __forceinline__ void frag_issue(Frag& f, unsigned addr) {
  asm volatile("ds_read_b64_tr_b16 %0, %2\n\tds_read_b64_tr_b16 %1, %2 offset:%3"
               : "=&v"(f.lo), "=&v"(f.hi)
               : "v"(addr), "n"(4 * CPR * 16));
}
template <int N>
__device__ __forceinline__ void frag_fence(Frag& f, bool wait) {
  if (wait) asm volatile("s_waitcnt lgkmcnt(%2)" : "+v"(f.lo), "+v"(f.hi) : "n"(N) : "memory");
  else asm volatile("" : "+v"(f.lo), "+v"(f.hi)::"memory");
}
template <typename T>
__device__ __forceinline__ typename Elem16<T>::x8 frag_value(const Frag& f) {
  return __builtin_bit_cast(typename Elem16<T>::x8, __builtin_shufflevector(f.lo, f.hi, 0, 1, 2, 3, 4, 5, 6, 7));
}
__device__ __forceinline__ unsigned wg_lds_addr(const void* p) {
  return (unsigned)(size_t)((__attribute__((address_space(3))) const char*)p);
}

template <typename T, int TN, int TK, int ST, int PC>
__device__ __forceinline__ void conv1x1_wgrad_body(const T* __restrict__ dY, const T* __restrict__ X,
                                                   float* __restrict__ part, int M, int N, int K, int chunks_per_wg,
                                                   int nsplits) {
#if defined(__HIP_DEVICE_COMPILE__)
  typedef WgGeo<TN, TK, PC> G;
  constexpr int CPRY = TN / 8, CPRX = TK / 8;
  extern __shared__ __align__(16) unsigned char smem_raw[];
  const int lane = threadIdx.x & (kWave - 1);
  const int wave = __builtin_amdgcn_readfirstlane(threadIdx.x / kWave);
  const int tiles_k = K / TK, tiles = (N / TN) * tiles_k;
  const int per = gridDim.x >> 3;
  const int vid = (blockIdx.x & 7) * per + (blockIdx.x >> 3);
  if (vid >= tiles * nsplits) return;
  const int split = vid / tiles, tile = vid - split * tiles;
  const int tn = tile / tiles_k, tk = tile - tn * tiles_k;
  const int n0 = tn * TN, k0 = tk * TK;
  const int chunks_total = (M + PC - 1) / PC;
  const int c_begin = split * chunks_per_wg;
  const int nch = min(chunks_per_wg, chunks_total - c_begin);

  const auto rsY = __builtin_amdgcn_make_buffer_rsrc(const_cast<T*>(dY), 0, (int)((size_t)M * N * 2), MRLA_WG_FLAGS);
  const auto rsX = __builtin_amdgcn_make_buffer_rsrc(const_cast<T*>(X), 0, (int)((size_t)M * K * 2), MRLA_WG_FLAGS);
  unsigned voffY[G::NIY], voffX[G::NIX];
#pragma unroll
  for (int i = 0; i < G::NIY; ++i) {
    const int u = wave + kWgWaves * i, row = u * (64 / CPRY) + lane / CPRY, cp = lane % CPRY;
    voffY[i] = (unsigned)(((size_t)c_begin * PC + row) * N * 2 + (n0 + ((cp ^ swz<CPRY>(row)) << 3)) * 2);
  }
#pragma unroll
  for (int i = 0; i < G::NIX; ++i) {
    const int u = wave + kWgWaves * i, row = u * (64 / CPRX) + lane / CPRX, cp = lane % CPRX;
    voffX[i] = (unsigned)(((size_t)c_begin * PC + row) * K * 2 + (k0 + ((cp ^ swz<CPRX>(row)) << 3)) * 2);
  }
  const unsigned advY = (unsigned)PC * N * 2, advX = (unsigned)PC * K * 2;
  int issued = 0;
  auto issue = [&](int stage) {
    unsigned char* sb = smem_raw + stage * G::SB;
    const unsigned kill = issued++ < nch ? 0u : 0x80000000u;
#pragma unroll
    for (int i = 0; i < G::NIY; ++i) {
      __builtin_amdgcn_raw_ptr_buffer_load_lds(rsY, (lds_void_ptr)(sb + (wave + kWgWaves * i) * 1024), 16, voffY[i] | kill, 0, 0, 0);
      voffY[i] += advY;
    }
#pragma unroll
    for (int i = 0; i < G::NIX; ++i) {
      __builtin_amdgcn_raw_ptr_buffer_load_lds(rsX, (lds_void_ptr)(sb + G::YB + (wave + kWgWaves * i) * 1024), 16, voffX[i] | kill, 0, 0, 0);
      voffX[i] += advX;
    }
  };

  const int wn = wave / G::WK, wk = wave - wn * G::WK;
  const unsigned lds0 = wg_lds_addr(smem_raw);
  unsigned offA[G::BN], offB[G::BK];
#pragma unroll
  for (int i = 0; i < G::BN; ++i) offA[i] = lds0 + tr_offset<CPRY>(lane, 0, wn * G::WTN + i * 32);
#pragma unroll
  for (int j = 0; j < G::BK; ++j) offB[j] = lds0 + G::YB + tr_offset<CPRX>(lane, 0, wk * G::WTK + j * 32);

  wg_f32x16 acc[G::BN][G::BK];
#pragma unroll
  for (int i = 0; i < G::BN; ++i)
#pragma unroll
    for (int j = 0; j < G::BK; ++j)
#pragma unroll
      for (int e = 0; e < 16; ++e) acc[i][j][e] = 0.f;

  constexpr int KSN = PC / 16, NF = 2 * (G::BN + G::BK), NI = G::NIY + G::NIX;
  static_assert(KSN % 2 == 0 && ST >= 3, "fragment double buffer / stages");
  Frag fa[2][G::BN], fb[2][G::BK];
  auto read_step = [&](int buf, unsigned sbo, int ks) {
#pragma unroll
    for (int i = 0; i < G::BN; ++i) frag_issue<CPRY>(fa[buf][i], offA[i] + sbo + ks * 16 * CPRY * 16);
#pragma unroll
    for (int j = 0; j < G::BK; ++j) frag_issue<CPRX>(fb[buf][j], offB[j] + sbo + ks * 16 * CPRX * 16);
  };
  auto mfma_step = [&](int buf) {
#pragma unroll
    for (int i = 0; i < G::BN; ++i)
#pragma unroll
      for (int j = 0; j < G::BK; ++j)
        Elem16<T>::mfma(acc[i][j], frag_value<T>(fa[buf][i]), frag_value<T>(fb[buf][j]));
  };
#pragma unroll
  for (int j = 0; j < ST - 1; ++j) issue(j);
  asm volatile("s_waitcnt vmcnt(%0)" ::"n"((ST - 2) * NI) : "memory");
  __builtin_amdgcn_s_barrier();
  asm volatile("" ::: "memory");
  read_step(0, 0, 0);
  int stage = 0, nxt = ST - 1;
  for (int c = 0; c < nch; ++c) {
    const unsigned sbo = stage * G::SB;
    stage = stage + 1 == ST ? 0 : stage + 1;
#pragma unroll
    for (int ks = 0; ks < KSN; ++ks) {
      const int cur = ks & 1;
      int pending = NF;
      if (ks + 1 < KSN) {
        read_step(cur ^ 1, sbo, ks + 1);
      } else if (c + 1 < nch) {
        asm volatile("s_waitcnt vmcnt(%0)" ::"n"((ST - 3) * NI) : "memory");
        __builtin_amdgcn_s_barrier();
        asm volatile("" ::: "memory");
        issue(nxt);
        nxt = nxt + 1 == ST ? 0 : nxt + 1;
        read_step(0, stage * G::SB, 0);
      } else {
        pending = 0;
      }
#pragma unroll
      for (int i = 0; i < G::BN; ++i) {
        if (pending) frag_fence<NF>(fa[cur][i], i == 0); else frag_fence<0>(fa[cur][i], i == 0);
      }
#pragma unroll
      for (int j = 0; j < G::BK; ++j) frag_fence<0>(fb[cur][j], false);
      mfma_step(cur);
    }
  }

  float* po = part + ((size_t)split * N + n0 + wn * G::WTN) * K + k0 + wk * G::WTK + (lane & 31);
  const int h = lane >> 5;
#pragma unroll
  for (int i = 0; i < G::BN; ++i)
#pragma unroll
    for (int j = 0; j < G::BK; ++j)
#pragma unroll
      for (int e = 0; e < 16; ++e)
        po[(size_t)(i * 32 + 8 * (e >> 2) + 4 * h + (e & 3)) * K + j * 32] = acc[i][j][e];
#endif
}

template <int TN, int TK, int ST, int PC>
__global__ __launch_bounds__(kWgWaves* kWave) void conv1x1_wgrad_kernel(const bf16_t* __restrict__ dY,
                                                                        const bf16_t* __restrict__ X,
                                                                        float* __restrict__ part, int M, int N, int K,
                                                                        int chunks_per_wg, int nsplits) {
  conv1x1_wgrad_body<bf16_t, TN, TK, ST, PC>(dY, X, part, M, N, K, chunks_per_wg, nsplits);
}
template <int TN, int TK, int ST, int PC>
__global__ __launch_bounds__(kWgWaves* kWave) void conv1x1_wgrad_f16_kernel(const f16_t* __restrict__ dY,
                                                                            const f16_t* __restrict__ X,
                                                                            float* __restrict__ part, int M, int N, int K,
                                                                            int chunks_per_wg, int nsplits) {
  conv1x1_wgrad_body<f16_t, TN, TK, ST, PC>(dY, X, part, M, N, K, chunks_per_wg, nsplits);
}

template <typename TO>
__device__ __forceinline__ void conv1x1_wgrad_reduce_body(const float* __restrict__ part, TO* __restrict__ dW, int splits,
                                                          int NK) {
  __shared__ float4 red[16][16];
  const int q = threadIdx.x & 15, g = threadIdx.x >> 4;
  const int e = blockIdx.x * 64 + q * 4;
  const float4* src = reinterpret_cast<const float4*>(part + e);
  const size_t pitch = (size_t)NK / 4;
  float4 a = {0.f, 0.f, 0.f, 0.f}, b = a;
  int s = g;
  for (; s + 16 < splits; s += 32) {
    const float4 u = src[(size_t)s * pitch], v = src[(size_t)(s + 16) * pitch];
    a.x += u.x; a.y += u.y; a.z += u.z; a.w += u.w;
    b.x += v.x; b.y += v.y; b.z += v.z; b.w += v.w;
  }
  if (s < splits) {
    const float4 u = src[(size_t)s * pitch];
    a.x += u.x; a.y += u.y; a.z += u.z; a.w += u.w;
  }
  red[g][q] = float4{a.x + b.x, a.y + b.y, a.z + b.z, a.w + b.w};
  __syncthreads();
  if (threadIdx.x < 64) {
    const int qq = threadIdx.x >> 2, cc = threadIdx.x & 3;
    float t = 0.f;
#pragma unroll
    for (int i = 0; i < 16; ++i) t += reinterpret_cast<const float*>(&red[i][qq])[cc];
    dW[blockIdx.x * 64 + threadIdx.x] = from_f<TO>(t);
  }
}
template <typename TO>
__global__ __launch_bounds__(256) void conv1x1_wgrad_reduce_kernel(const float* __restrict__ part, TO* __restrict__ dW,
                                                                   int splits, int NK) {
  conv1x1_wgrad_reduce_body<TO>(part, dW, splits, NK);
}
__global__ __launch_bounds__(256) void conv1x1_wgrad_reduce_f16_kernel(const float* __restrict__ part, f16_t* __restrict__ dW,
                                                                       int splits, int NK) {
  conv1x1_wgrad_reduce_body<f16_t>(part, dW, splits, NK);
}

struct WgPlan {
  int tn = 0, tk = 0, tiles = 0, splits = 0, chunks_per_wg = 0;
};

WgPlan wgrad_plan(int M, int K, int N) {
  WgPlan p;
  if (M <= 0 || N % 64 || K % 64 || (size_t)M * std::max(N, K) * 2 >= (size_t)1 << 31) return p;
  int tn = N % 256 == 0 ? 256 : N % 128 == 0 ? 128 : 64;
  int tk = K % 256 == 0 ? 256 : K % 128 == 0 ? 128 : 64;
  while (tn * tk > 32768) {
    if (tn >= tk) tn /= 2; else tk /= 2;
  }
  p.tn = tn; p.tk = tk;
  p.tiles = (N / tn) * (K / tk);
  const int chunks = (M + kPC - 1) / kPC;
  const int want = std::max(1, std::min(chunks, (kWgTarget + p.tiles - 1) / p.tiles));
  p.chunks_per_wg = (chunks + want - 1) / want;
  p.splits = (chunks + p.chunks_per_wg - 1) / p.chunks_per_wg;
  return p;
}

template <int TN, int TK, int ST, int PC>
int launch_tile(const WgPlan& p, const void* dy, const void* x, float* part, int M, int K, int N, int dtype, hipStream_t st) {
  typedef WgGeo<TN, TK, PC> G;
  const size_t lds = (size_t)ST * G::SB;
  const dim3 grid((p.tiles * p.splits + 7) / 8 * 8), block(kWgWaves * kWave);
  if (dtype == MRLA_F16) {
    if (lds_opt_in(reinterpret_cast<const void*>(conv1x1_wgrad_f16_kernel<TN, TK, ST, PC>), lds) != hipSuccess) return MRLA_EHIP;
    hipLaunchKernelGGL((conv1x1_wgrad_f16_kernel<TN, TK, ST, PC>), grid, block, lds, st, (const f16_t*)dy, (const f16_t*)x, part,
                       M, N, K, p.chunks_per_wg, p.splits);
  } else {
    if (lds_opt_in(reinterpret_cast<const void*>(conv1x1_wgrad_kernel<TN, TK, ST, PC>), lds) != hipSuccess) return MRLA_EHIP;
    hipLaunchKernelGGL((conv1x1_wgrad_kernel<TN, TK, ST, PC>), grid, block, lds, st, (const bf16_t*)dy, (const bf16_t*)x, part,
                       M, N, K, p.chunks_per_wg, p.splits);
  }
  return MRLA_OK;
}

}

int conv1x1_wgrad_rows(int M, int K, int N) {
  const WgPlan p = wgrad_plan(M, K, N);
  return p.tiles ? p.splits : MRLA_EUNSUPPORTED;
}

int conv1x1_wgrad_plan(int M, int K, int N, int* out) {
  const WgPlan p = wgrad_plan(M, K, N);
  if (!p.tiles) return MRLA_EUNSUPPORTED;
  out[0] = p.chunks_per_wg; out[1] = kWgStages; out[2] = p.tn; out[3] = p.tk; out[4] = p.splits; out[5] = p.tiles;
  return MRLA_OK;
}

int launch_conv1x1_wgrad(const void* dy, const void* x, float* part, void* dw, int dw_f32, int M, int K, int N, int dtype,
                         hipStream_t st) {
  const WgPlan p = wgrad_plan(M, K, N);
  if (!p.tiles || (dtype != MRLA_BF16 && dtype != MRLA_F16)) return MRLA_EUNSUPPORTED;
  int rc = MRLA_EUNSUPPORTED;
#define MRLA_WG_TILE(A, B) \
  if (p.tn == A && p.tk == B) rc = launch_tile<A, B, kWgStages, kPC>(p, dy, x, part, M, K, N, dtype, st);
  MRLA_WG_TILE(64, 64) MRLA_WG_TILE(64, 128) MRLA_WG_TILE(64, 256) MRLA_WG_TILE(128, 64) MRLA_WG_TILE(128, 128)
  MRLA_WG_TILE(128, 256) MRLA_WG_TILE(256, 64) MRLA_WG_TILE(256, 128)
#undef MRLA_WG_TILE
  if (rc != MRLA_OK) return rc;
  const int NK = N * K;
  if (dw_f32)
    hipLaunchKernelGGL(conv1x1_wgrad_reduce_kernel<float>, dim3(NK / 64), dim3(256), 0, st, part, (float*)dw, p.splits, NK);
  else if (dtype == MRLA_F16)
    hipLaunchKernelGGL(conv1x1_wgrad_reduce_f16_kernel, dim3(NK / 64), dim3(256), 0, st, part, (f16_t*)dw, p.splits, NK);
  else
    hipLaunchKernelGGL(conv1x1_wgrad_reduce_kernel<bf16_t>, dim3(NK / 64), dim3(256), 0, st, part, (bf16_t*)dw, p.splits, NK);
  return hip_status(hipGetLastError());
}

}
```

### mrla_amd/csrc/mrla_device.h

```cpp
#pragma once
#include <hip/hip_runtime.h>
#include <stdint.h>

namespace mrla {

typedef __bf16 bf16_t;
typedef _Float16 f16_t;

typedef uint32_t u32x4 __attribute__((ext_vector_type(4)));

constexpr int kWave = 64;
constexpr int kThreads = 256;
constexpr int kWaves = kThreads / kWave;

enum { M_SX = 0, M_SV = 1, M_SO = 2, M_SVV = 3, M_SVO = 4, M_SOO = 5, M_N = 6, M_PV = 6, M_PO = 7, M_REC = 8 };
enum { D_D = 0, D_DV = 1, D_DO = 2, D_N = 3 };
constexpr int kTokPartLnxW = 10, kTokPartLnxB = 11, kTokPartHat = 14, kTokParts = 15;

struct RawMoments { double sv, so, svv, svo, soo; };
__device__ __forceinline__ RawMoments raw_moments(const float* __restrict__ m, double n) {
  const double pv = m[M_PV], po = m[M_PO], a = m[M_SV], b = m[M_SO];
  RawMoments r;
  r.sv = a + n * pv;
  r.so = b + n * po;
  r.svv = (double)m[M_SVV] + 2.0 * pv * a + n * pv * pv;
  r.svo = (double)m[M_SVO] + pv * b + po * a + n * pv * po;
  r.soo = (double)m[M_SOO] + 2.0 * po * b + n * po * po;
  return r;
}
__device__ __forceinline__ void rebase_moments(float (&a)[M_N], float n, float pv, float po, float qv, float qo) {
  const float dv = pv - qv, d_o = po - qo;
  a[M_SVV] += 2.f * dv * a[M_SV] + n * dv * dv;
  a[M_SOO] += 2.f * d_o * a[M_SO] + n * d_o * d_o;
  a[M_SVO] += d_o * a[M_SV] + dv * a[M_SO] + n * dv * d_o;
  a[M_SV] += n * dv;
  a[M_SO] += n * d_o;
}

template <typename T> __device__ __forceinline__ float to_f(T v) { return static_cast<float>(v); }
template <typename T> __device__ __forceinline__ T from_f(float v) { return static_cast<T>(v); }

__device__ __forceinline__ float lane_prev(float v) {
  return __int_as_float(__builtin_amdgcn_update_dpp(0, __float_as_int(v), 0x138, 0xf, 0xf, false));
}
__device__ __forceinline__ float lane_next(float v) {
  return __int_as_float(__builtin_amdgcn_update_dpp(0, __float_as_int(v), 0x130, 0xf, 0xf, false));
}

#define MRLA_DPP_ADD(v, ctrl, row_mask, bank_mask) \
  (v) += __int_as_float(__builtin_amdgcn_update_dpp(0, __float_as_int(v), (ctrl), (row_mask), (bank_mask), true))

__device__ __forceinline__ float seg_sum(float v, int lane, int ws) {
  if (ws >= 8) {
    MRLA_DPP_ADD(v, 0x111, 0xf, 0xf);
    MRLA_DPP_ADD(v, 0x112, 0xf, 0xf);
    MRLA_DPP_ADD(v, 0x114, 0xf, 0xf);
    if (ws >= 16) MRLA_DPP_ADD(v, 0x118, 0xf, 0xf);
    if (ws >= 32) MRLA_DPP_ADD(v, 0x142, 0xa, 0xf);
    if (ws >= 64) MRLA_DPP_ADD(v, 0x143, 0xc, 0xf);
    return v;
  }
  for (int off = 1; off < ws; off <<= 1) {
    const float t = __shfl_xor(v, off, kWave);
    v += t;
  }
  return v;
}

__device__ __forceinline__ float wave_sum(float v) {
  MRLA_DPP_ADD(v, 0x111, 0xf, 0xf);
  MRLA_DPP_ADD(v, 0x112, 0xf, 0xf);
  MRLA_DPP_ADD(v, 0x114, 0xf, 0xf);
  MRLA_DPP_ADD(v, 0x118, 0xf, 0xf);
  MRLA_DPP_ADD(v, 0x142, 0xa, 0xf);
  MRLA_DPP_ADD(v, 0x143, 0xc, 0xf);
  return __int_as_float(__builtin_amdgcn_readlane(__float_as_int(v), 63));
}
__device__ __forceinline__ double wave_sum(double v) {
#pragma unroll
  for (int off = kWave / 2; off > 0; off >>= 1) v += __shfl_xor(v, off, kWave);
  return v;
}

__device__ __forceinline__ float erf_f(float a) {
  const float t = fminf(fabsf(a), 10.0f), s = t * t;
  float r = fmaf(-1.72853470e-5f, t, 3.83197126e-4f);
  const float q = fmaf(-3.88396438e-3f, t, 2.42546219e-2f);
  r = fmaf(r, s, q);
  r = fmaf(r, t, -1.06777877e-1f);
  r = fmaf(r, t, -6.34846687e-1f);
  r = fmaf(r, t, -1.28717512e-1f);
  r = fmaf(r, t, -t);
  const float big = copysignf(1.0f - __expf(r), a);
  float p = -5.96761703e-4f;
  p = fmaf(p, s, 4.99119423e-3f);
  p = fmaf(p, s, -2.67681349e-2f);
  p = fmaf(p, s, 1.12819925e-1f);
  p = fmaf(p, s, -3.76125336e-1f);
  p = fmaf(p, s, 1.28379166e-1f);
  const float small = fmaf(p, a, a);
  return t > 0.927734375f ? big : small;
}

__device__ __forceinline__ float gelu_f(float u) { return 0.5f * u * (1.0f + erf_f(u * 0.70710678118654752440f)); }
__device__ __forceinline__ float gelu_grad_f(float u) {
  const float cdf = 0.5f * (1.0f + erf_f(u * 0.70710678118654752440f));
  const float pdf = 0.39894228040143267794f * __expf(-0.5f * u * u);
  return cdf + u * pdf;
}

template <typename T>
__device__ __forceinline__ void slab_load(T* __restrict__ dst, const T* __restrict__ src, int n, int tid) {
  constexpr int VEC = 16 / sizeof(T);
  if ((reinterpret_cast<uintptr_t>(src) & 15) == 0) {
    const int nv = n / VEC;
    const u32x4* __restrict__ s4 = reinterpret_cast<const u32x4*>(src);
    u32x4* __restrict__ d4 = reinterpret_cast<u32x4*>(dst);
#pragma unroll 2
    for (int i = tid; i < nv; i += kThreads) d4[i] = __builtin_nontemporal_load(&s4[i]);
    for (int i = nv * VEC + tid; i < n; i += kThreads) dst[i] = src[i];
  } else {
    for (int i = tid; i < n; i += kThreads) dst[i] = src[i];
  }
}

typedef __attribute__((address_space(3))) void* lds_void_ptr;

template <typename T>
__device__ __forceinline__ void slab_prefetch(T* __restrict__ dst, const T* __restrict__ src, int n, int tid) {
  const int bytes = n * (int)sizeof(T);
  if ((reinterpret_cast<uintptr_t>(src) & 15) == 0 && (bytes & 15) == 0) {
    const int lane = tid & (kWave - 1), wave = tid / kWave;
    const char* s = reinterpret_cast<const char*>(src);
    char* d = reinterpret_cast<char*>(dst);
    const int nchunks = (bytes + 1023) >> 10;
    for (int ch = wave; ch < nchunks; ch += kWaves) {
      const int off = (ch << 10) + (lane << 4);
      if (off < bytes)
        __builtin_amdgcn_global_load_lds(reinterpret_cast<const void*>(s + off),
                                         (lds_void_ptr)(d + (ch << 10)), 16, 0, 0);
    }
  } else {
    slab_load(dst, src, n, tid);
  }
}

__device__ __forceinline__ void wait_async_copies() { asm volatile("s_waitcnt vmcnt(0)" ::: "memory"); }

template <typename T>
__device__ __forceinline__ void slab_store(T* __restrict__ dst, const T* __restrict__ src, int n, int tid) {
  constexpr int VEC = 16 / sizeof(T);
  if ((reinterpret_cast<uintptr_t>(dst) & 15) == 0) {
    const int nv = n / VEC;
    const u32x4* __restrict__ s4 = reinterpret_cast<const u32x4*>(src);
    u32x4* __restrict__ d4 = reinterpret_cast<u32x4*>(dst);
#pragma unroll 2
    for (int i = tid; i < nv; i += kThreads) d4[i] = s4[i];
    for (int i = nv * VEC + tid; i < n; i += kThreads) dst[i] = src[i];
  } else {
    for (int i = tid; i < n; i += kThreads) dst[i] = src[i];
  }
}

}
```

### mrla_amd/csrc/mrla_kernels.h

```cpp
#pragma once
#include <hip/hip_runtime.h>
#include <stddef.h>
#include <stdint.h>

#include "../../include/mrla_hip.h"

namespace mrla {

constexpr int kMaxTasksPerWave = 4;

struct SlabGeo {
  int B, C, H, W, HW;
  int CP;
  int slabs;
  int WS;
  int PW;
  int NG;
  int NB;
  int RB;
  int BG;
  int astride;
};

inline size_t dtype_size(int dtype) { return dtype == MRLA_F32 ? 4 : 2; }

inline int hip_status(hipError_t e) { return e == hipSuccess ? MRLA_OK : MRLA_EHIP; }

hipError_t lds_opt_in(const void* kernel, size_t bytes);

int make_slab_geo(SlabGeo* g, int B, int C, int H, int W, int dtype, int arrays, int bg_hint);

int launch_light_stats_fwd_nchw(const void* x, const void* o, const float* wv, float* mom, void* xout,
                                const float* psc, const float* psh, const SlabGeo& g, int dtype, int act,
                                hipStream_t st);
int launch_light_apply_fwd_nchw(const void* x, const void* o, const float* wv, const float* gate, const float* sc,
                                const float* sh, const float* lam, const float* dp, void* out, const SlabGeo& g,
                                int d, int res, int dtype, int act, hipStream_t st);
int launch_light_stats_bwd_nchw(const void* dout, const void* x, const void* o, const float* wv, const float* mom,
                                float* bmom, const SlabGeo& g, int dtype, int act, hipStream_t st);
int launch_light_apply_bwd_nchw(const void* dout, const void* x, const void* o, const float* wv, const float* gate,
                                const float* cb, const float* lam, const float* dp, const float* dyx, void* dx,
                                void* dprev, float* dwv_part, const SlabGeo& g, int d, int res, int relu, int dtype,
                                int act, hipStream_t st);

int launch_gate_fwd(const float* mom, const float* wq, const float* wk, int ks, float* gate, int B, int C, int HW,
                    int d, hipStream_t st);
int launch_bn_fwd(const float* mom, const float* gate, const float* lam, const float* gamma, const float* beta,
                  float* run_mean, float* run_var, int training, float momentum, float eps, float* sc, float* sh,
                  float* save_mean, float* save_inv, int B, int C, int HW, int d, hipStream_t st);
int launch_bn_bwd(const float* mom, const float* bmom, const float* gate, const float* lam, const float* gamma,
                  const float* dp, const float* save_mean, const float* save_inv, int training, float* cb, float* cb_lo,
                  float* dgamma, float* dbeta, float* dlam, int B, int C, int HW, int d, hipStream_t st);
int launch_gate_bwd(const float* mom, const float* bmom, const float* gate, const float* cb, const float* cb_lo,
                    const float* dp, const float* wq, const float* wk, int ks, float* dyx, float* dwqk_part, int B, int C, int HW,
                    int d, hipStream_t st, float* tok_part = nullptr, int tok_bands = 0);
int nhwc_set_row_cut_mode(int mode);
int nhwc_wgrad_ranges(int B, int C, int H, int W);
int nhwc_bmom_ranges(int B, int C, int H, int W);
int nhwc_mom_ranges(int B, int C, int H, int W);
int launch_reduce_rows(const float* in, float* out, int rows, int n, hipStream_t st);
int launch_fold_rows(float* buf, int rows, int n, hipStream_t st);
int launch_reduce_rows2(const float* in1, float* out1, int rows1, int n1, const float* in2, float* out2, int rows2, int n2,
                        hipStream_t st);


int launch_base_gate_fwd(const float* mom, const float* wq, const float* wk, int ks, float* Kring, float* Pall,
                         float* q, int B, int C, int HW, int d, int T, int t, hipStream_t st);
int launch_base_attend_fwd(const void* x, const float* wv, void* Vring, const float* Pall, void* attn, float* amom,
                           const SlabGeo& g, int d, int T, int t, int dtype, hipStream_t st);
int launch_plain_bn_fwd(const float* amom, const float* gamma, const float* beta, float* run_mean, float* run_var,
                        int training, float momentum, float eps, float* sc, float* sh, float* save_mean,
                        float* save_inv, const float* pivot, int B, int C, int HW, hipStream_t st);
int launch_plain_bn_fwd_rec(const float* rec, const float* gamma, const float* beta, float* run_mean, float* run_var,
                            int training, float momentum, float eps, float* sc, float* sh, float* save_mean,
                            float* save_inv, int R, int C, hipStream_t st);
int launch_plain_bn_bwd(const float* tmom, const float* gamma, const float* save_mean, const float* save_inv,
                        int training, int centered, float* cb, float* dgamma, float* dbeta, int B, int C, int HW,
                        hipStream_t st);
int launch_base_tail_fwd(const void* x, const void* attn, const float* sc, const float* sh, const float* dp, void* out,
                         int B, int C, int HW, int dtype, hipStream_t st);
int launch_base_tail_stats_bwd(const void* dout, const void* attn, const float* sc, const float* sh, const float* dp,
                               float* tmom, const SlabGeo& g, int dtype, hipStream_t st);
int launch_base_attend_bwd(const void* dout, const void* attn, const float* sc, const float* sh, const float* dp,
                           const float* cb, const void* Vring, void* dAring, float* pmom, const SlabGeo& g, int T,
                           int t, int dtype, hipStream_t st);
int launch_base_gate_bwd(const float* mom, const float* pmom, const float* Pall, const float* q, const float* Kring,
                         float* dKring, const float* wq, const float* wk, int ks, float* dyx, float* dwqk_part, int B,
                         int C, int HW, int d, int T, int t, int first_touch, hipStream_t st, float* tok_part = nullptr,
                         int tok_bands = 0);
int launch_base_value_bwd(const void* dout, const void* x, const float* wv, const void* dAring, const float* Pall,
                          const float* dyx, void* dx, float* dwv_part, const SlabGeo& g, int d, int T, int t, int Tc,
                          int res, int dtype, hipStream_t st);


bool token_nhwc_applies(int C);
int token_bands(int B, int C, int side);
int token_bands_bwd(int B, int C, int side);
int launch_token_apply_fwd_nhwc(const void* x, const void* o, const float* stats, const float* wx, const float* bx,
                                const float* wo, const float* bo, const float* wv, const float* gate, const float* lam,
                                void* out, int B, int n, int C, int side, int d, int res, int dtype, hipStream_t st);
int launch_token_apply_bwd_nhwc(const void* dout, const void* x, const void* o, const float* stats, const float* wx,
                                const float* bx, const float* wo, const float* bo, const float* wv, const float* gate,
                                const float* lam, float* dxn, float* part, float* bmom, int B, int n, int C, int side,
                                int d, int dtype, hipStream_t st);

bool base_nhwc_supported(int C, int dtype);
int base_nhwc_tiles(int B, int C, int HW, int dtype);
int base_nhwc_pmom_tiles(int B, int C, int HW, int dtype);
int launch_base_attend_fwd_nhwc(const void* Vring, const float* Pall, void* attn, float* amom_part, int B, int C, int HW,
                                int d, int T, int t, int dtype, hipStream_t st, int ext_gap = 0, int ext_off = 0);
int launch_base_dv_combine_nhwc(const void* dAring, const float* Pall, void* dv, int B, int C, int HW, int d, int T,
                                int t, int Tc, int dtype, hipStream_t st);
int launch_base_tail_fwd_nhwc(const void* x, const void* attn, const float* sc, const float* sh, const float* dp,
                              void* out, int B, int C, int HW, int dtype, hipStream_t st);
int launch_base_attend_bwd_nhwc(const void* dout, const void* attn, const float* sc, const float* sh, const float* dp,
                                const float* cb, const void* Vring, void* dAring, float* pmom_part, int B, int C, int HW,
                                int T, int t, int dtype, hipStream_t st, int ext_gap = 0, int ext_off = 0);
int launch_base_pmom_reduce(const float* part, float* pmom, int B, int C, int t, int tiles, hipStream_t st);
int launch_base_value_bwd_wide(const void* dout, const void* x, const float* wv, const void* dv, const float* dyx, void* dx,
                               float* dwv_part, const void* pre, const float* pre_center, float* pre_tmom, int B, int C,
                               int H, int W, int res, int dtype, hipStream_t st);
int launch_base_value_bwd_nhwc(const void* dout, const void* x, const float* wv, const void* dv, const float* dyx,
                               void* dx, float* dwv_part, const void* pre, const float* pre_center, float* pre_tmom, int B,
                               int C, int H, int W, int res, int dtype, hipStream_t st);


int launch_token_value_fwd_nhwc(const void* x, const float* stats, const float* wx, const float* bx, const float* wv,
                                void* vslot, int B, int n, int C, int side, int dtype, hipStream_t st);
int launch_token_cls_fwd(const void* x, const float* stats, const float* wx, const float* bx, void* out, int B, int n,
                         int C, int dtype, hipStream_t st);
int launch_token_value_bwd_nhwc(const void* dout, const void* x, const float* stats, const float* wx, const float* bx,
                                const float* wv, const void* dv, float* dxn, float* part, int B, int n, int C, int side,
                                int dtype, hipStream_t st);
int launch_token_norm_pool(const void* x, const void* o, const float* wx, const float* bx, float eps, float* stats,
                           float* mom, int B, int n, int C, int dtype, hipStream_t st);
int launch_token_apply_fwd(const void* x, const void* o, const float* stats, const float* wx, const float* bx,
                           const float* wo, const float* bo, const float* wv, const float* gate, const float* lam,
                           void* out, int B, int n, int C, int side, int d, int res, int dtype, hipStream_t st);
int launch_token_apply_bwd(const void* dout, const void* x, const void* o, const float* stats, const float* wx,
                           const float* bx, const float* wo, const float* bo, const float* wv, const float* gate,
                           const float* lam, float* dxn, float* part, float* bmom, int B, int n, int C, int side, int d,
                           int dtype, hipStream_t st);
int launch_token_ln_bwd(const void* dout, const void* x, const void* o, const float* dxn, const float* dyx,
                        const float* stats, const float* wx, const float* wo, const float* lam, void* dx, void* dprev, int B,
                        int n, int C, int res, int dtype, hipStream_t st);


int launch_plane_moments(const void* x, float* amom, float* pivot, int B, int C, int HW, int dtype, hipStream_t st);
int launch_plane_dmoments(const void* dy, const void* x, const float* sc, const float* sh, const float* center, int relu,
                          float* tmom, int B, int C, int HW, int dtype, hipStream_t st);
int launch_affine_act(const void* x, const void* dy, const float* a, const float* sc, const float* sh, int relu,
                      void* out, int B, int C, int HW, int dtype, int bwd, hipStream_t st);


int nhwc_images_per_group(int B, int C, int W);
int conv1x1_rows(int M, int K, int N);
int conv1x1_plan(int M, int K, int N, int add, int* out);
int launch_conv1x1_fwd(const void* x, const void* w, void* y, float* part, int M, int K, int N, int dtype, hipStream_t st);
int conv1x1_addend_supported(int M, int K, int N);
int launch_conv1x1_addend(const void* x, const void* w, const void* addend, void* y, int M, int K, int N, int b, int h, int wd,
                          int sh, int sw, int dtype, hipStream_t st);
int bn_pool_rows(int B, int C, int H, int W);
int launch_bn_relu_pool_fwd(const void* x, const float* sc, const float* sh, void* out, int B, int C, int H, int W,
                            int dtype, hipStream_t st);
int launch_bn_relu_pool_dmoments(const void* dp, const void* x, const float* sc, const float* sh, const float* center,
                                 float* tmom, int B, int C, int H, int W, int dtype, hipStream_t st);
int launch_bn_relu_pool_bwd(const void* dp, const void* x, const float* sc, const float* sh, const float* cb, void* dx,
                            int B, int C, int H, int W, int dtype, hipStream_t st);
int conv1x1_wide_rows(int M, int K, int N);
int conv1x1_wide_plan(int M, int K, int N, int add, int* out);
int launch_conv1x1_wide(const void* x, const void* w, const void* addend, void* y, float* part, int M, int K, int N,
                        int dtype, hipStream_t st);
int launch_conv1x1_wide_sparse(const void* x, const void* w, const void* addend, void* y, int M, int K, int N, int b, int h,
                               int wd, int sh, int sw, int dtype, hipStream_t st);
int conv1x1_kstream_supported(int M, int K, int N);
int conv1x1_kstream_stages(int M, int K, int N);
int conv1x1_kstream_rows(int M, int K, int N);
int launch_conv1x1_kstream(const void* x, const void* w, void* y, float* part, int M, int K, int N, int dtype, hipStream_t st);
int launch_conv1x1_kstream_addend(const void* x, const void* w, const void* addend, void* y, int M, int K, int N, int b, int h,
                                  int wd, int sh, int sw, int dtype, hipStream_t st);
int conv1x1_wgrad_rows(int M, int K, int N);
int conv1x1_wgrad_plan(int M, int K, int N, int* out);
int launch_conv1x1_wgrad(const void* dy, const void* x, float* part, void* dw, int dw_f32, int M, int K, int N, int dtype,
                         hipStream_t st);
int launch_weight_bank_refresh(const long long* table, int entries, int max_tiles, int dtype, hipStream_t st);
int launch_light_stats_fwd_wide(const void* x, const void* o, const float* wv, float* mom, void* xout, const float* psc,
                                const float* psh, void* vout, int B, int C, int H, int W, int dtype, int act,
                                hipStream_t st, bool fused_no_x = false, int mom_ranges = 1);
int launch_light_apply_fwd_wide(const void* x, const void* o, const float* wv, const float* gate, const float* sc,
                                const float* sh, const float* lam, const float* dp, void* out, int B, int C, int H,
                                int W, int d, int res, int dtype, int act, hipStream_t st);
int launch_light_apply_fwd_pre_wide(const void* pre, const void* o, const float* psc, const float* psh, const float* wv,
                                    const float* gate, const float* sc, const float* sh, const float* lam,
                                    const float* dp, void* out, int B, int C, int H, int W, int d, int res, int dtype,
                                    hipStream_t st);
int launch_light_apply_bwd_wide(const void* dout, const void* x, const void* o, const float* wv, const float* gate,
                                const float* cb, const float* lam, const float* dp, const float* dyx, void* dx,
                                void* dprev, float* dwv_part, const void* pre, const float* pre_center, float* pre_tmom,
                                int B, int C, int H, int W, int d, int res, int relu, int dtype, int act, hipStream_t st);
int launch_light_stats_bwd_wide(const void* dout, const void* x, const void* o, const float* wv, const float* mom,
                                float* bmom, int B, int C, int H, int W, int dtype, int act, hipStream_t st);
int light_lean_supported(int B, int C, int H, int W, int dtype);
int launch_light_stats_bwd_lean_wide(const void* dout, const void* pre, const void* o, const float* wv, const float* psc,
                                     const float* psh, const float* mom, float* bmom, int B, int C, int H, int W, int dtype,
                                     hipStream_t st);
int launch_light_apply_bwd_lean_wide(const void* dout, const void* pre, const void* o, const float* wv, const float* psc,
                                     const float* psh, const float* gate, const float* cb, const float* lam,
                                     const float* dp, const float* dyx, void* dx, void* dprev, float* dwv_part,
                                     const float* pre_center, float* pre_tmom, int B, int C, int H, int W, int d, int res,
                                     int dtype, hipStream_t st);
int launch_light_stats_fwd_nhwc(const void* x, const void* o, const float* wv, float* mom, void* xout,
                                const float* psc, const float* psh, void* vout, int B, int C, int H, int W, int dtype,
                                int act, hipStream_t st, bool fused_no_x = false, int mom_ranges = 1);
int launch_light_apply_fwd_nhwc(const void* x, const void* o, const float* wv, const float* gate, const float* sc,
                                const float* sh, const float* lam, const float* dp, void* out, int B, int C, int H,
                                int W, int d, int res, int dtype, int act, hipStream_t st);
int launch_light_stats_bwd_nhwc(const void* dout, const void* x, const void* o, const float* wv, const float* mom,
                                float* bmom, int B, int C, int H, int W, int dtype, int act, hipStream_t st);
int launch_light_apply_bwd_nhwc(const void* dout, const void* x, const void* o, const float* wv, const float* gate,
                                const float* cb, const float* lam, const float* dp, const float* dyx, void* dx,
                                void* dprev, float* dwv_part, const void* pre, const float* pre_center, float* pre_tmom,
                                int B, int C, int H, int W, int d, int res, int relu, int dtype, int act, hipStream_t st);
int nhwc_bn_splits(int B, int C, int HW);
int launch_nhwc_pool_fused(const void* pre, const float* sc, const float* sh, const void* o, float* part, float* mom,
                           int B, int C, int HW, int dtype, hipStream_t st);
int launch_light_apply_fwd_pre_nhwc(const void* pre, const void* o, const float* psc, const float* psh, const float* wv,
                                    const float* gate, const float* sc, const float* sh, const float* lam,
                                    const float* dp, void* out, int B, int C, int H, int W, int d, int res, int dtype,
                                    hipStream_t st);
int launch_nhwc_moments(const void* x, const void* dy, const float* sc, const float* sh, int relu, const float* dp,
                        float* out, float* pivot, int B, int C, int HW, int dtype, int mode, hipStream_t st);
int launch_nhwc_affine(const void* x, const void* dy, const float* a, const float* sc, const float* sh, int relu,
                       void* out, int B, int C, int HW, int dtype, int bwd, hipStream_t st);

}
```

### mrla_amd/csrc/sequences.hip

```cpp
#include "mrla_kernels.h"

#define MRLA_TRY(call)          \
  do {                          \
    const int rc_ = (call);     \
    if (rc_ != MRLA_OK) return rc_; \
  } while (0)

extern "C" {

int mrla_light_tail_fwd(const void* x, const float* pre_sc, const float* pre_sh, const void* o_prev, const float* wq,
                        const float* wk, int ksize, const float* wv, const float* lam, const float* gamma,
                        const float* beta, float* running_mean, float* running_var, int bn_mode, float momentum, float eps,
                        const float* dp, float* mom, void* x_out, float* gate, float* bnbuf, void* out, int b, int c,
                        int h, int w, int d, int res, int fuse, int dtype, int layout, int act, void* stream) {
  if (bn_mode != MRLA_BN_NONE && !bnbuf) return MRLA_EINVAL;
  if (fuse && ((fuse == 1 && !x_out) || act != MRLA_ACT_NONE)) return MRLA_EINVAL;
  const void* xt = x;
  if (fuse == 2) {
    if (mrla_light_lean_supported(b, c, h, w, dtype, layout) != 1) return MRLA_EUNSUPPORTED;
    MRLA_TRY(mrla_light_stats_fwd_fused(x, pre_sc, pre_sh, o_prev, wv, mom, nullptr, b, c, h, w, dtype, layout, stream));
    xt = nullptr;
  } else if (fuse) {
    MRLA_TRY(mrla_light_stats_fwd_fused(x, pre_sc, pre_sh, o_prev, wv, mom, x_out, b, c, h, w, dtype, layout, stream));
    xt = x_out;
  } else {
    MRLA_TRY(mrla_light_stats_fwd(x, o_prev, wv, mom, b, c, h, w, dtype, layout, act, stream));
  }
  MRLA_TRY(mrla_light_gate_fwd(mom, wq, wk, ksize, gate, b, c, h * w, d, stream));
  const float *sc = nullptr, *sh = nullptr;
  if (bn_mode != MRLA_BN_NONE) {
    MRLA_TRY(mrla_light_bn_fwd(mom, gate, lam, gamma, beta, running_mean, running_var, bn_mode, momentum, eps, bnbuf,
                               bnbuf + c, bnbuf + 2 * (size_t)c, bnbuf + 3 * (size_t)c, b, c, h * w, d, stream));
    sc = bnbuf;
    sh = bnbuf + c;
  }
  if (fuse == 2)
    return mrla_light_apply_fwd_fused(x, pre_sc, pre_sh, o_prev, wv, gate, sc, sh, lam, dp, out, b, c, h, w, d, res, dtype,
                                      layout, stream);
  return mrla_light_apply_fwd(xt, o_prev, wv, gate, sc, sh, lam, dp, out, b, c, h, w, d, res, dtype, layout, act, stream);
}

int mrla_light_tail_bwd(const void* dout, const void* x, const void* o_prev, const float* wq, const float* wk, int ksize,
                        const float* wv, const float* lam, const float* gamma, const float* dp, const float* mom,
                        const float* gate, const float* bnbuf, int bn_mode, float* bmom, float* small, float* dyx,
                        float* dwqk_part, float* dwv_part, int rows, void* dx, void* do_prev, const void* pre,
                        const float* pre_sc, const float* pre_sh, const float* pre_center, float* pre_tmom, float* wsum,
                        int b, int c, int h, int w, int d, int res, int relu_mask, int dtype, int layout, int act,
                        void* stream) {
  if (!small || !wsum || rows <= 0 || ksize <= 0) return MRLA_EINVAL;
  const bool has_bn = bn_mode != MRLA_BN_NONE;
  if (has_bn && (!bnbuf || !gamma)) return MRLA_EINVAL;
  const size_t C = (size_t)c;
  float *cb = small, *dgamma = small + 4 * C, *dbeta = small + 5 * C, *dlam = small + 6 * C, *cb_lo = small + 7 * C;
  const bool lean = x == nullptr;
  if (lean && (!pre || !relu_mask || act != MRLA_ACT_NONE)) return MRLA_EINVAL;
  if (lean) MRLA_TRY(mrla_light_stats_bwd_fused(dout, pre, pre_sc, pre_sh, o_prev, wv, mom, bmom, b, c, h, w, dtype, layout, stream));
  else MRLA_TRY(mrla_light_stats_bwd(dout, x, o_prev, wv, mom, bmom, b, c, h, w, dtype, layout, act, stream));
  MRLA_TRY(mrla_light_bn_bwd(mom, bmom, gate, lam, has_bn ? gamma : nullptr, dp, has_bn ? bnbuf + 2 * C : nullptr,
                             has_bn ? bnbuf + 3 * C : nullptr, bn_mode, cb, cb_lo, has_bn ? dgamma : nullptr,
                             has_bn ? dbeta : nullptr, lam ? dlam : nullptr, b, c, h * w, d, stream));
  MRLA_TRY(mrla_light_gate_bwd(mom, bmom, gate, cb, cb_lo, dp, wq, wk, ksize, dyx, dwqk_part, b, c, h * w, d, stream));
  if (lean)
    MRLA_TRY(mrla_light_apply_bwd_fused(dout, pre, pre_sc, pre_sh, o_prev, wv, gate, cb, lam, dp, dyx, dx, do_prev, dwv_part,
                                        pre_center, pre_tmom, b, c, h, w, d, res, dtype, layout, stream));
  else
    MRLA_TRY(mrla_light_apply_bwd(dout, x, o_prev, wv, gate, cb, lam, dp, dyx, dx, do_prev, dwv_part, pre, pre_center,
                                  pre_tmom, b, c, h, w, d, res, relu_mask, dtype, layout, act, stream));
  return mrla_reduce_rows2(dwv_part, wsum, rows, c * 9, dwqk_part, wsum + 9 * C, b, 2 * ksize, stream);
}

int mrla_bn_fwd(const void* x, const float* records, int rec_rows, float* amom, float* pivot, int rows, const float* gamma,
                const float* beta, float* running_mean, float* running_var, int bn_mode, float momentum, float eps,
                float* bnbuf, int relu, void* y, int b, int c, int h, int w, int dtype, int layout, void* stream) {
  if (!bnbuf || (bn_mode != MRLA_BN_TRAIN && bn_mode != MRLA_BN_EVAL)) return MRLA_EINVAL;
  const size_t C = (size_t)c;
  if (records) {
    if (bn_mode != MRLA_BN_TRAIN) return MRLA_EINVAL;
    MRLA_TRY(mrla_bn_stats_fwd_rows(records, gamma, beta, running_mean, running_var, bn_mode, momentum, eps, bnbuf,
                                    bnbuf + C, bnbuf + 2 * C, bnbuf + 3 * C, rec_rows, c, stream));
  } else {
    if (!amom || rows <= 0 || ((long)b * h * w) % rows) return MRLA_EINVAL;
    const bool train = bn_mode == MRLA_BN_TRAIN;
    if (train) MRLA_TRY(mrla_bn_plane_moments(x, amom, pivot, b, c, h, w, dtype, layout, stream));
    MRLA_TRY(mrla_bn_stats_fwd(amom, train ? pivot : nullptr, gamma, beta, running_mean, running_var, bn_mode, momentum,
                               eps, bnbuf, bnbuf + C, bnbuf + 2 * C, bnbuf + 3 * C, rows, c, (int)((long)b * h * w / rows),
                               stream));
  }
  if (!y) return MRLA_OK;
  return mrla_bn_act_fwd(x, bnbuf, bnbuf + C, relu, y, b, c, h, w, dtype, layout, stream);
}

int mrla_bn_bwd(const void* dy, const void* x, const float* gamma, const float* bnbuf, float* tmom, int rows, int have_tmom,
                int bn_mode, int relu, float* small, void* dx, int b, int c, int h, int w, int dtype, int layout,
                void* stream) {
  if (!bnbuf || !tmom || !small || rows <= 0 || ((long)b * h * w) % rows) return MRLA_EINVAL;
  const size_t C = (size_t)c;
  if (!have_tmom)
    MRLA_TRY(mrla_bn_plane_dmoments(dy, x, bnbuf, bnbuf + C, bnbuf + 2 * C, relu, tmom, b, c, h, w, dtype, layout, stream));
  MRLA_TRY(mrla_bn_stats_bwd(tmom, gamma, bnbuf + 2 * C, bnbuf + 3 * C, bn_mode, 1, small, small + 3 * C, small + 4 * C, rows,
                             c, (int)((long)b * h * w / rows), stream));
  return mrla_bn_act_bwd(dy, x, bnbuf, bnbuf + C, small, relu, dx, b, c, h, w, dtype, layout, stream);
}

int mrla_stem_fwd(const void* x, float* amom, float* pivot, int rows, const float* gamma, const float* beta,
                  float* running_mean, float* running_var, int bn_mode, float momentum, float eps, float* bnbuf, void* out,
                  int b, int c, int h, int w, int dtype, int layout, void* stream) {
  if (!bnbuf || !amom || rows <= 0 || ((long)b * h * w) % rows || (bn_mode != MRLA_BN_TRAIN && bn_mode != MRLA_BN_EVAL))
    return MRLA_EINVAL;
  const size_t C = (size_t)c;
  const bool train = bn_mode == MRLA_BN_TRAIN;
  if (train) MRLA_TRY(mrla_bn_plane_moments(x, amom, pivot, b, c, h, w, dtype, layout, stream));
  MRLA_TRY(mrla_bn_stats_fwd(amom, train ? pivot : nullptr, gamma, beta, running_mean, running_var, bn_mode, momentum, eps,
                             bnbuf, bnbuf + C, bnbuf + 2 * C, bnbuf + 3 * C, rows, c, (int)((long)b * h * w / rows), stream));
  return mrla_bn_relu_pool_fwd(x, bnbuf, bnbuf + C, out, b, c, h, w, dtype, layout, stream);
}

int mrla_stem_bwd(const void* dp, const void* x, const float* gamma, const float* bnbuf, float* tmom, int rows, int bn_mode,
                  float* small, void* dx, int b, int c, int h, int w, int dtype, int layout, void* stream) {
  if (!bnbuf || !tmom || !small || rows <= 0 || ((long)b * h * w) % rows) return MRLA_EINVAL;
  const size_t C = (size_t)c;
  MRLA_TRY(mrla_bn_relu_pool_dmoments(dp, x, bnbuf, bnbuf + C, bnbuf + 2 * C, tmom, b, c, h, w, dtype, layout, stream));
  MRLA_TRY(mrla_bn_stats_bwd(tmom, gamma, bnbuf + 2 * C, bnbuf + 3 * C, bn_mode, 1, small, small + 3 * C, small + 4 * C, rows, c,
                             (int)((long)b * h * w / rows), stream));
  if (!dx) return MRLA_OK;
  return mrla_bn_relu_pool_bwd(dp, x, bnbuf, bnbuf + C, small, dx, b, c, h, w, dtype, layout, stream);
}

int mrla_base_layer_fwd(const void* x, const float* pre_sc, const float* pre_sh, const void* identity, const float* wq,
                        const float* wk, int ksize, const float* wv, const float* gamma, const float* beta,
                        float* running_mean, float* running_var, int bn_mode, float momentum, float eps, const float* dp,
                        float* mom, void* x_out, void* v_ring, float* k_ring, float* p_all, float* q, void* attn,
                        float* amom, int arows, float* bnbuf, void* out, int tail, int b, int c, int h, int w, int d, int T,
                        int t, int dtype, void* stream) {
  if (!v_ring || t <= 0 || t > T || arows <= 0 || (tail && (!bnbuf || !out))) return MRLA_EINVAL;
  const size_t C = (size_t)c, slot = (size_t)b * h * w * C * mrla::dtype_size(dtype);
  void* v_slot = (char*)v_ring + (size_t)(t - 1) * slot;
  MRLA_TRY(mrla_base_pool_value_fwd(x, pre_sc, pre_sh, identity, wv, mom, x_out, v_slot, b, c, h, w, dtype, MRLA_NHWC, stream));
  MRLA_TRY(mrla_base_gate_fwd(mom, wq, wk, ksize, k_ring, p_all, q, b, c, h * w, d, T, t, stream));
  MRLA_TRY(mrla_base_attend_fwd(nullptr, wv, v_ring, p_all, attn, amom, b, c, h, w, d, T, t, dtype, MRLA_NHWC, stream));
  if (!tail) return MRLA_OK;
  if (((long)b * h * w) % arows) return MRLA_EINVAL;
  MRLA_TRY(mrla_bn_stats_fwd(amom, nullptr, gamma, beta, running_mean, running_var, bn_mode, momentum, eps, bnbuf, bnbuf + C,
                             bnbuf + 2 * C, bnbuf + 3 * C, arows, c, (int)((long)b * h * w / arows), stream));
  return mrla_base_tail_fwd(identity ? x_out : x, attn, bnbuf, bnbuf + C, dp, out, b, c, h, w, dtype, MRLA_NHWC, stream);
}

int mrla_base_layer_bwd(const void* dout, const void* x, const void* attn, const float* wq, const float* wk, int ksize,
                        const float* wv, const float* gamma, const float* dp, const float* mom, const float* q,
                        const float* bnbuf, int bn_mode, const void* v_ring, void* da_ring, const float* k_ring,
                        float* dk_ring, const float* p_all, float* tmom, int trows, float* small, float* ppart, int prows,
                        float* pmom, float* dyx, float* dwqk_part, void* dv, float* dwv_part, int rows, void* dx,
                        const void* pre, const float* pre_center, float* pre_tmom, float* wsum, int tail, int first_touch,
                        int res, int b, int c, int h, int w, int d, int T, int t, int Tc, int dtype, void* stream) {
  if (!wsum || rows <= 0 || prows <= 0 || ksize <= 0) return MRLA_EINVAL;
  const size_t C = (size_t)c;
  const float *sc = nullptr, *sh = nullptr, *cb = nullptr;
  if (tail) {
    if (!bnbuf || !small || !tmom || trows <= 0 || ((long)b * h * w) % trows) return MRLA_EINVAL;
    sc = bnbuf;
    sh = bnbuf + C;
    cb = small;
    MRLA_TRY(mrla_base_tail_stats_bwd(dout, attn, sc, sh, bnbuf + 2 * C, dp, tmom, b, c, h, w, dtype, MRLA_NHWC, stream));
    MRLA_TRY(mrla_bn_stats_bwd(tmom, gamma, bnbuf + 2 * C, bnbuf + 3 * C, bn_mode, 1, small, small + 3 * C, small + 4 * C,
                               trows, c, (int)((long)b * h * w / trows), stream));
  }
  MRLA_TRY(mrla_base_attend_bwd(dout, attn, sc, sh, dp, cb, v_ring, da_ring, ppart, b, c, h, w, T, t, dtype, MRLA_NHWC, stream));
  MRLA_TRY(mrla_base_pmom_reduce(ppart, pmom, b, c, t, prows, stream));
  MRLA_TRY(mrla_base_gate_bwd(mom, pmom, p_all, q, k_ring, dk_ring, wq, wk, ksize, dyx, dwqk_part, b, c, h * w, d, T, t,
                              first_touch, stream));
  MRLA_TRY(mrla_base_dv_combine(da_ring, p_all, dv, b, c, h, w, d, T, t, Tc, dtype, MRLA_NHWC, stream));
  MRLA_TRY(mrla_base_value_bwd_dv(dout, x, wv, dv, dyx, dx, dwv_part, pre, pre_center, pre_tmom, b, c, h, w, res, dtype,
                                  MRLA_NHWC, stream));
  return mrla_reduce_rows2(dwv_part, wsum, rows, c * 9, dwqk_part, wsum + 9 * C, b, 2 * ksize, stream);
}

int mrla_token_light_fwd(const void* x, const void* o_prev, const float* lnx_w, const float* lnx_b, const float* lno_w,
                         const float* lno_b, const float* wq, const float* wk, int ksize, const float* wv,
                         const float* lam, float eps, float* stats, float* mom, float* gate, void* out, int b, int n, int c,
                         int d, int res, int dtype, void* stream) {
  MRLA_TRY(mrla_token_norm_pool(x, o_prev, lnx_w, lnx_b, eps, stats, mom, b, n, c, dtype, stream));
  MRLA_TRY(mrla_light_gate_fwd(mom, wq, wk, ksize, gate, b, c, n - 1, d, stream));
  return mrla_token_apply_fwd(x, o_prev, stats, lnx_w, lnx_b, lno_w, lno_b, wv, gate, lam, out, b, n, c, d, res, dtype,
                              stream);
}

int mrla_token_light_bwd(const void* dout, const void* x, const void* o_prev, const float* stats, const float* lnx_w,
                         const float* lnx_b, const float* lno_w, const float* lno_b, const float* wq, const float* wk,
                         int ksize, const float* wv, const float* gate, const float* lam, const float* mom, float* dxn,
                         float* part, int prow, float* bmom, float* dyx, float* dwqk_part, void* dx, void* do_prev,
                         float* sums, int b, int n, int c, int d, int res, int dtype, void* stream) {
  if (!sums || prow <= 0 || ksize <= 0) return MRLA_EINVAL;
  MRLA_TRY(mrla_token_apply_bwd(dout, x, o_prev, stats, lnx_w, lnx_b, lno_w, lno_b, wv, gate, lam, dxn, part, bmom, b, n, c,
                                d, dtype, stream));
  MRLA_TRY(mrla_token_gate_bwd(mom, bmom, gate, wq, wk, ksize, dyx, dwqk_part, part, b, n, c, d, dtype, stream));
  MRLA_TRY(mrla_token_ln_bwd(dout, x, o_prev, dxn, dyx, stats, lnx_w, lno_w, lam, dx, do_prev, b, n, c, res, dtype, stream));
  const size_t np = (size_t)c * MRLA_TOKEN_PARTIALS;
  return mrla_reduce_rows2(part, sums, prow, (int)np, dwqk_part, sums + np, b, 2 * ksize, stream);
}

}
```

### mrla_amd/functional.py

```python
import contextlib
import ctypes
import threading
import weakref
from math import log

import torch

from . import _lib as L

_DT = {torch.float32: L.F32, torch.bfloat16: L.BF16, torch.float16: L.F16}


def k_size_for(c):
    t = int(abs((log(c, 2) + 1) / 2.0))
    return t if t % 2 else t + 1


class KernelTimer:

    def __init__(self, names=None):
        self.names = None if names is None else set(names)
        self.records = []

    def summary(self):
        out = {}
        for name, nbytes, e0, e1, alg, path in self.records:
            d = out.setdefault(name, dict(launches=0, ms=0.0, bytes=0, bytes_alg=0, bytes_path=0))
            d["launches"] += 1
            d["ms"] += e0.elapsed_time(e1)
            d["bytes"] += nbytes
            d["bytes_alg"] += nbytes if alg is None else alg
            d["bytes_path"] += path
        return out


TIMER = None
SEQUENCES = True


LEAN = False


SHORTCUT_ADDEND = True


def _seq():
    return SEQUENCES and TIMER is None


def _seq_call(name, *args):
    L.call(name, *args)


def _call(name, nbytes, *args, entry=None, alg=None, path=0):
    t = TIMER
    if t is not None and (t.names is None or name in t.names):
        e0, e1 = torch.cuda.Event(enable_timing=True), torch.cuda.Event(enable_timing=True)
        e0.record()
        L.call(entry or name, *args)
        e1.record()
        t.records.append((name, nbytes, e0, e1, alg, path))
    else:
        L.call(entry or name, *args)


def _ptr(t):
    return t.data_ptr() if t is not None else None


class _Bookkeeping:
    def __init__(self, n_drop_paths, bank=None):
        self.counters, self.n_dp, self.table, self.key, self.next = [], int(n_drop_paths), None, None, 0
        self.bank = bank

    def drop_path_row(self, batch, drop_prob, device):
        key = (batch, float(drop_prob), str(device))
        if self.table is None or self.key != key or self.next >= self.n_dp:
            keep = 1.0 - drop_prob
            self.table = torch.floor(keep + torch.rand((self.n_dp, batch), dtype=torch.float32, device=device)) / keep
            self.key, self.next = key, 0
        row = self.table[self.next]
        self.next += 1
        return row


_TLS = threading.local()


def current_bookkeeping():
    return getattr(_TLS, "book", None)


@contextlib.contextmanager
def batched_bookkeeping(n_drop_paths=0, bank=None):
    prev, book = current_bookkeeping(), _Bookkeeping(n_drop_paths, bank)
    _TLS.book = book
    try:
        yield book
    finally:
        _TLS.book = prev
        if book.counters:
            torch._foreach_add_(book.counters, 1)


def bump_batch_counter(bn):
    momentum = bn.momentum
    if bn.num_batches_tracked is not None:
        book = current_bookkeeping()
        if book is not None and momentum is not None:
            book.counters.append(bn.num_batches_tracked)
        else:
            bn.num_batches_tracked.add_(1)
            if momentum is None:
                momentum = 1.0 / float(bn.num_batches_tracked)
    return momentum


_raw_stream = getattr(torch._C, "_cuda_getCurrentRawStream", None)
_graph_task = getattr(torch._C, "_current_graph_task_id", None)


def _graph_task_id():
    return _graph_task() if _graph_task is not None else -1


def _stream():
    if _raw_stream is not None:
        return _raw_stream(torch.cuda.current_device())
    return torch.cuda.current_stream().cuda_stream


def _f32(t):
    if t is None:
        return None
    t = t.detach()
    if t.dtype != torch.float32:
        t = t.float()
    return t.contiguous()


def _grad_like(g, shape, stride):
    g = g.contiguous()
    dims = [(n, s) for n, s in zip(shape, stride) if n > 1]
    expect, row_major = 1, True
    for n, s in reversed(dims):
        row_major &= s == expect
        expect *= n
    if row_major:
        return g.as_strided(shape, stride)
    return torch.empty_strided(shape, stride, dtype=g.dtype, device=g.device).copy_(g.view(shape))


def _on_device(fn):
    import functools

    @functools.wraps(fn)
    def wrapped(ctx, x, *args):
        if isinstance(x, torch.Tensor) and x.is_cuda and x.device.index != torch.cuda.current_device():
            with torch.cuda.device(x.device):
                return fn(ctx, x, *args)
        return fn(ctx, x, *args)
    return wrapped


class _RunningStats:

    def __init__(self, rm, rv, c, what):
        for t in (rm, rv):
            if t is None or not t.is_cuda or t.numel() != c:
                raise L.MrlaHipError(f"{what}: running statistics must be CUDA tensors with {c} elements")
        self.src = (rm, rv)
        ok = all(t.dtype == torch.float32 and t.is_contiguous() for t in (rm, rv))
        self.rm, self.rv = (rm, rv) if ok else (rm.detach().float().contiguous(), rv.detach().float().contiguous())
        self.copy_back = not ok

    def finish(self, updated):
        if self.copy_back and updated:
            with torch.no_grad():
                self.src[0].copy_(self.rm)
                self.src[1].copy_(self.rv)


def _require_cuda(x, what):
    if not x.is_cuda:
        raise L.MrlaHipError(f"{what}: got a {x.device} tensor. mrla_amd runs only on an AMD GPU through libmrla_hip.so; "
                             "the CPU restatement lives in oracle/ and is test infrastructure, not a fallback.")
    if x.dtype not in _DT:
        raise L.MrlaHipError(f"{what}: unsupported dtype {x.dtype}")


_CL = torch.channels_last


def _layout_of(x, want=None):
    if want is None:
        if x.is_contiguous():
            return L.NCHW, x
        if x.dim() == 4 and x.is_contiguous(memory_format=_CL):
            return L.NHWC, x
        return L.NCHW, x.contiguous()
    if want == L.NHWC:
        return L.NHWC, x.contiguous(memory_format=_CL)
    return L.NCHW, x.contiguous()


class _DeferredBnBox:
    __slots__ = ("ptr", "shape", "tmom", "rows", "center", "ref", "version")

    def __init__(self):
        self.ptr = self.shape = self.tmom = self.rows = self.ref = self.version = None
        self.center = None

    def put(self, dpre, tmom, rows):
        if (dpre.numel() // dpre.shape[1]) % rows:
            tmom, rows = tmom.sum(0, keepdim=True, dtype=torch.float64).float(), 1
        self.ptr, self.shape, self.tmom, self.rows = dpre.data_ptr(), tuple(dpre.shape), tmom, rows
        self.ref, self.version = weakref.ref(dpre), dpre._version

    def take(self, dy):
        alive = self.ref() if self.ref is not None else None
        ok = (self.tmom is not None and alive is not None and dy.data_ptr() == self.ptr and tuple(dy.shape) == self.shape
              and dy._version == self.version)
        tmom, rows = self.tmom, self.rows
        self.ptr = self.shape = self.tmom = self.rows = self.ref = self.version = None
        return (tmom, rows) if ok else None


class LightConfig:
    __slots__ = ("d", "bn_mode", "momentum", "eps", "res", "act", "fuse", "pre_affine", "pre_box", "infer")

    def __init__(self, d, bn_mode=L.BN_NONE, momentum=0.1, eps=1e-5, res=0, act=L.ACT_NONE, fuse=False, pre_affine=None,
                 pre_box=None):
        self.d, self.bn_mode, self.momentum, self.eps, self.res, self.act = d, bn_mode, momentum, eps, res, act
        self.pre_affine = pre_affine
        self.pre_box = pre_box
        self.infer = False
        self.fuse = fuse


class _LightFn(torch.autograd.Function):

    @staticmethod
    @_on_device
    def forward(ctx, x, o_prev, wq, wk, wv, lam, gamma, beta, running_mean, running_var, dp, cfg):
        _require_cuda(x, "mrla light forward")
        layout, xc = _layout_of(x)
        b, c, h, w = xc.shape
        d = cfg.d
        via_nhwc = layout == L.NCHW and L.load().mrla_light_wgrad_rows(b, c, h, w, _DT[xc.dtype], L.NCHW) == L.EUNSUPPORTED
        if via_nhwc:
            layout, xc = L.NHWC, xc.contiguous(memory_format=_CL)
        if c % d:
            raise L.MrlaHipError(f"channels ({c}) not divisible by dim_perhead ({d})")
        oc = None
        if o_prev is not None:
            if o_prev.shape != x.shape or o_prev.dtype != x.dtype:
                raise L.MrlaHipError("o_prev must match x in shape and dtype")
            oc = _layout_of(o_prev, layout)[1]
        dt = _DT[xc.dtype]
        dev = xc.device
        wq32, wk32 = _f32(wq).reshape(-1), _f32(wk).reshape(-1)
        wv32 = _f32(wv).reshape(c, 9)
        lam32 = _f32(lam).reshape(-1) if lam is not None else None
        dp32 = _f32(dp).reshape(-1) if dp is not None else None
        ks = wq32.numel()
        G = c // d
        st = _stream()

        msplits = L.load().mrla_light_mom_splits(b, c, h, w, dt, layout)
        L.check(min(msplits, 0), "mrla_light_mom_splits")
        mom = torch.empty((msplits, b, c, L.FWD_MOMENTS), dtype=torch.float32, device=dev)
        if cfg.fuse and (oc is None or cfg.act != L.ACT_NONE):
            raise L.MrlaHipError("the fused relu(pre + o_prev) producer needs o_prev and no activation on V")
        if (cfg.fuse and layout == L.NHWC and cfg.bn_mode != L.BN_TRAIN and c % 64 == 0
                and cfg.infer):
            psc, psh = cfg.pre_affine if cfg.pre_affine is not None else (None, None)
            rows = L.load().mrla_bn_moment_rows(b, c, h, w, layout)
            part = torch.empty((rows, c, 2), dtype=torch.float32, device=dev)
            _call("mrla_light_pool_fused", xc.numel() * xc.element_size() * 2, _ptr(xc), _ptr(psc), _ptr(psh), _ptr(oc),
                  _ptr(part), _ptr(mom), b, c, h, w, dt, layout, st)
            gate = torch.empty((b, G), dtype=torch.float32, device=dev)
            _call("mrla_light_gate_fwd", 0, _ptr(mom), _ptr(wq32), _ptr(wk32), ks, _ptr(gate), b, c, h * w, d, st)
            bnbuf = None
            if cfg.bn_mode != L.BN_NONE:
                gamma32, beta32 = _f32(gamma), _f32(beta)
                rs = _RunningStats(running_mean, running_var, c, "mrla light forward")
                bnbuf = torch.empty((4, c), dtype=torch.float32, device=dev)
                _call("mrla_light_bn_fwd", 0, _ptr(mom), _ptr(gate), _ptr(lam32), _ptr(gamma32), _ptr(beta32),
                       _ptr(rs.rm), _ptr(rs.rv), cfg.bn_mode, float(cfg.momentum), float(cfg.eps),
                       _ptr(bnbuf[0]), _ptr(bnbuf[1]), _ptr(bnbuf[2]), _ptr(bnbuf[3]), b, c, h * w, d, st)
            out = torch.empty_like(xc)
            _call("mrla_light_apply_fwd_fused", xc.numel() * xc.element_size() * 3, _ptr(xc), _ptr(psc), _ptr(psh),
                  _ptr(oc), _ptr(wv32), _ptr(gate), _ptr(bnbuf[0]) if bnbuf is not None else None,
                  _ptr(bnbuf[1]) if bnbuf is not None else None, _ptr(lam32), _ptr(dp32), _ptr(out), b, c, h, w, d,
                  cfg.res, dt, layout, st, path=xc.numel() * xc.element_size() * 3)
            return out.contiguous() if via_nhwc else out
        pre = None
        lean = bool(LEAN and cfg.fuse and not via_nhwc and L.load().mrla_light_lean_supported(b, c, h, w, dt, layout) == 1)
        nb = xc.numel() * xc.element_size()
        if _seq():
            psc = psh = None
            if cfg.fuse:
                pre, xc = xc, (None if lean else torch.empty_like(xc))
                psc, psh = cfg.pre_affine if cfg.pre_affine is not None else (None, None)
            gate = torch.empty((b, G), dtype=torch.float32, device=dev)
            bnbuf = gamma32 = beta32 = rs = None
            if cfg.bn_mode != L.BN_NONE:
                gamma32, beta32 = _f32(gamma), _f32(beta)
                rs = _RunningStats(running_mean, running_var, c, "mrla light forward")
                bnbuf = torch.empty((4, c), dtype=torch.float32, device=dev)
            out = torch.empty_like(oc if lean else xc)
            _seq_call("mrla_light_tail_fwd", _ptr(pre if cfg.fuse else xc), _ptr(psc), _ptr(psh), _ptr(oc), _ptr(wq32),
                      _ptr(wk32), ks, _ptr(wv32), _ptr(lam32), _ptr(gamma32), _ptr(beta32),
                      _ptr(rs.rm) if rs is not None else None, _ptr(rs.rv) if rs is not None else None, cfg.bn_mode,
                      float(cfg.momentum), float(cfg.eps), _ptr(dp32), _ptr(mom), _ptr(xc) if (cfg.fuse and not lean) else None,
                      _ptr(gate), _ptr(bnbuf), _ptr(out), b, c, h, w, d, cfg.res, (2 if lean else int(cfg.fuse)), dt, layout,
                      cfg.act, st)
            if rs is not None:
                rs.finish(cfg.bn_mode == L.BN_TRAIN)
        else:
            if cfg.fuse:
                pre, xc = xc, (None if lean else torch.empty_like(xc))
                psc, psh = cfg.pre_affine if cfg.pre_affine is not None else (None, None)
                _call("mrla_light_stats_fwd_fused", nb * (2 if lean else 3), _ptr(pre), _ptr(psc), _ptr(psh),
                      _ptr(oc), _ptr(wv32), _ptr(mom), _ptr(xc), b, c, h, w, dt, layout, st)
            else:
                _call("mrla_light_stats_fwd", xc.numel() * xc.element_size() * (2 if oc is not None else 1), _ptr(xc),
                      _ptr(oc), _ptr(wv32), _ptr(mom), b, c, h, w, dt, layout, cfg.act, st)
            gate = torch.empty((b, G), dtype=torch.float32, device=dev)
            _call("mrla_light_gate_fwd", 0, _ptr(mom), _ptr(wq32), _ptr(wk32), ks, _ptr(gate), b, c, h * w, d, st)
            bnbuf = gamma32 = None
            if cfg.bn_mode != L.BN_NONE:
                gamma32, beta32 = _f32(gamma), _f32(beta)
                rs = _RunningStats(running_mean, running_var, c, "mrla light forward")
                bnbuf = torch.empty((4, c), dtype=torch.float32, device=dev)
                _call("mrla_light_bn_fwd", 0, _ptr(mom), _ptr(gate), _ptr(lam32), _ptr(gamma32), _ptr(beta32),
                       _ptr(rs.rm), _ptr(rs.rv), cfg.bn_mode, float(cfg.momentum), float(cfg.eps),
                       _ptr(bnbuf[0]), _ptr(bnbuf[1]), _ptr(bnbuf[2]), _ptr(bnbuf[3]), b, c, h * w, d, st)
                rs.finish(cfg.bn_mode == L.BN_TRAIN)
            if lean:
                out = torch.empty_like(oc)
                _call("mrla_light_apply_fwd_fused", nb * 3, _ptr(pre), _ptr(psc), _ptr(psh), _ptr(oc), _ptr(wv32), _ptr(gate),
                      _ptr(bnbuf[0]) if bnbuf is not None else None, _ptr(bnbuf[1]) if bnbuf is not None else None,
                      _ptr(lam32), _ptr(dp32), _ptr(out), b, c, h, w, d, cfg.res, dt, layout, st, path=nb * 3)
            else:
                out = torch.empty_like(xc)
# ... 717 lines not shown
        else:
            tmom = torch.empty((rows, c, 2), dtype=torch.float32, device=dev)
        small = torch.empty((5, c), dtype=torch.float32, device=dev)
        dx = torch.empty_like(xc)
        mode = L.BN_TRAIN if ctx.training else L.BN_EVAL
        if _seq():
            _seq_call("mrla_bn_bwd", _ptr(dy), _ptr(xc), _ptr(gamma32), _ptr(bnbuf), _ptr(tmom), rows, int(handed is not None),
                      mode, ctx.relu, _ptr(small), _ptr(dx), b, c, h, w, dt, layout, st)
        else:
            if handed is None:
                _call("mrla_bn_plane_dmoments", xc.numel() * es * 2, _ptr(dy), _ptr(xc), _ptr(bnbuf[0]), _ptr(bnbuf[1]),
                      _ptr(bnbuf[2]), ctx.relu, _ptr(tmom), b, c, h, w, dt, layout, st)
            cb = small[:3].view(c, 3)
            _call("mrla_bn_stats_bwd", 0, _ptr(tmom), _ptr(gamma32), _ptr(bnbuf[2]), _ptr(bnbuf[3]), mode, 1, _ptr(cb),
                  _ptr(small[3]), _ptr(small[4]), rows, c, b * h * w // rows, st)
            _call("mrla_bn_act_bwd", xc.numel() * es * 3, _ptr(dy), _ptr(xc), _ptr(bnbuf[0]), _ptr(bnbuf[1]), _ptr(cb), ctx.relu,
                  _ptr(dx), b, c, h, w, dt, layout, st)
        return dx, small[3].to(ctx.gdtype), small[4].to(ctx.gdtype), None, None, None, None, None, None, None, None, None


def bn_act(x, bn, relu, defer=False, pre_moments=None):
    if (type(bn) is torch.nn.BatchNorm2d and bn.affine and bn.track_running_stats and x.is_cuda and x.dim() == 4
            and x.dtype in _DT and (x.is_contiguous() or x.is_contiguous(memory_format=_CL))):
        training = bn.training
        momentum = bump_batch_counter(bn) if training else bn.momentum
        if defer:
            box = _DeferredBnBox()
            y, buf = _BnActFn.apply(x, bn.weight, bn.bias, bn.running_mean, bn.running_var, training, momentum or 0.0,
                                    bn.eps, False, True, pre_moments, box)
            y._mrla_affine = (buf[0], buf[1])
            y._mrla_bn_box = box
            return y
        return _BnActFn.apply(x, bn.weight, bn.bias, bn.running_mean, bn.running_var, training, momentum or 0.0, bn.eps,
                              relu, False, pre_moments)
    y = bn(x)
    return torch.relu(y) if relu else y


class _BnReluPoolFn(torch.autograd.Function):

    @staticmethod
    @_on_device
    def forward(ctx, x, gamma, beta, running_mean, running_var, training, momentum, eps):
        _require_cuda(x, "fused bn/relu/maxpool forward")
        layout, xc = _layout_of(x, L.NHWC)
        b, c, h, w = xc.shape
        dt, dev, st = _DT[xc.dtype], xc.device, _stream()
        gamma32, beta32 = _f32(gamma), _f32(beta)
        rs = _RunningStats(running_mean, running_var, c, "fused bn/relu/maxpool forward")
        bnbuf = torch.empty((4, c), dtype=torch.float32, device=dev)
        rows = L.load().mrla_bn_moment_rows(b, c, h, w, layout)
        amom = torch.empty((rows, c, 2), dtype=torch.float32, device=dev)
        pivot = torch.empty((c,), dtype=torch.float32, device=dev) if training else None
        ho, wo = (h - 1) // 2 + 1, (w - 1) // 2 + 1
        out = torch.empty((b, c, ho, wo), dtype=xc.dtype, device=dev, memory_format=_CL)
        mode = L.BN_TRAIN if training else L.BN_EVAL
        if _seq():
            _seq_call("mrla_stem_fwd", _ptr(xc), _ptr(amom), _ptr(pivot), rows, _ptr(gamma32), _ptr(beta32), _ptr(rs.rm),
                      _ptr(rs.rv), mode, float(momentum), float(eps), _ptr(bnbuf), _ptr(out), b, c, h, w, dt, layout, st)
        else:
            if training:
                _call("mrla_bn_plane_moments", xc.numel() * xc.element_size(), _ptr(xc), _ptr(amom), _ptr(pivot), b, c, h, w, dt,
                      layout, st)
            _call("mrla_bn_stats_fwd", 0, _ptr(amom), _ptr(pivot), _ptr(gamma32), _ptr(beta32), _ptr(rs.rm), _ptr(rs.rv),
                   mode, float(momentum), float(eps), _ptr(bnbuf[0]), _ptr(bnbuf[1]), _ptr(bnbuf[2]), _ptr(bnbuf[3]), rows, c,
                   b * h * w // rows, st)
            _call("mrla_bn_relu_pool_fwd", (xc.numel() + out.numel()) * xc.element_size(), _ptr(xc), _ptr(bnbuf[0]),
                  _ptr(bnbuf[1]), _ptr(out), b, c, h, w, dt, layout, st)
        rs.finish(training)
        ctx.training, ctx.gdtype = training, gamma.dtype
        ctx.save_for_backward(xc, gamma32, bnbuf)
        return out

    @staticmethod
    @_on_device
    def backward(ctx, dp):
        xc, gamma32, bnbuf = ctx.saved_tensors
        b, c, h, w = xc.shape
        dt, dev, st = _DT[xc.dtype], xc.device, _stream()
        if dp.dtype != xc.dtype:
            dp = dp.to(xc.dtype)
        dp = _layout_of(dp, L.NHWC)[1]
        es = xc.element_size()
        rows = L.load().mrla_bn_pool_rows(b, c, h, w, dt, L.NHWC)
        L.check(min(rows, 0), "mrla_bn_pool_rows")
        tmom = torch.empty((rows, c, 2), dtype=torch.float32, device=dev)
        small = torch.empty((5, c), dtype=torch.float32, device=dev)
        dx = torch.empty_like(xc) if ctx.needs_input_grad[0] else None
        mode = L.BN_TRAIN if ctx.training else L.BN_EVAL
        if _seq():
            _seq_call("mrla_stem_bwd", _ptr(dp), _ptr(xc), _ptr(gamma32), _ptr(bnbuf), _ptr(tmom), rows, mode, _ptr(small),
                      _ptr(dx), b, c, h, w, dt, L.NHWC, st)
        else:
            _call("mrla_bn_relu_pool_dmoments", (xc.numel() + dp.numel()) * es, _ptr(dp), _ptr(xc), _ptr(bnbuf[0]), _ptr(bnbuf[1]),
                  _ptr(bnbuf[2]), _ptr(tmom), b, c, h, w, dt, L.NHWC, st)
            cb = small[:3].view(c, 3)
            _call("mrla_bn_stats_bwd", 0, _ptr(tmom), _ptr(gamma32), _ptr(bnbuf[2]), _ptr(bnbuf[3]), mode, 1, _ptr(cb),
                  _ptr(small[3]), _ptr(small[4]), rows, c, b * h * w // rows, st)
            if dx is not None:
                _call("mrla_bn_relu_pool_bwd", (2 * xc.numel() + dp.numel()) * es, _ptr(dp), _ptr(xc), _ptr(bnbuf[0]),
                      _ptr(bnbuf[1]), _ptr(cb), _ptr(dx), b, c, h, w, dt, L.NHWC, st)
        return dx, small[3].to(ctx.gdtype), small[4].to(ctx.gdtype), None, None, None, None, None


def bn_relu_maxpool(x, bn, pool):
    def _pair(v):
        return tuple(v) if isinstance(v, (tuple, list)) else (v, v)
    if (type(bn) is torch.nn.BatchNorm2d and bn.affine and bn.track_running_stats and type(pool) is torch.nn.MaxPool2d
            and _pair(pool.kernel_size) == (3, 3) and _pair(pool.stride) == (2, 2) and _pair(pool.padding) == (1, 1)
            and _pair(pool.dilation) == (1, 1) and not pool.ceil_mode and not pool.return_indices
            and x.is_cuda and x.dim() == 4 and x.dtype in _DT and x.is_contiguous(memory_format=_CL)
            and x.data_ptr() % 16 == 0
            and L.load().mrla_bn_pool_rows(x.shape[0], x.shape[1], x.shape[2], x.shape[3], _DT[x.dtype], L.NHWC) > 0):
        training = bn.training
        momentum = bump_batch_counter(bn) if training else bn.momentum
        return _BnReluPoolFn.apply(x, bn.weight, bn.bias, bn.running_mean, bn.running_var, training, momentum or 0.0, bn.eps)
    return pool(bn_act(x, bn, relu=True))


class WeightBank:

    def __init__(self, convs):
        self.convs = [c for c in convs if self.eligible(c)]
        self.key = self.sig = None
        self.dtype = torch.bfloat16
        self.captured = False
        self.entries = {}

    def invalidate(self):
        self.key = None

    @staticmethod
    def eligible(conv):
        return (type(conv) is torch.nn.Conv2d and conv.kernel_size == (1, 1)
                and conv.padding == (0, 0) and conv.dilation == (1, 1) and conv.groups == 1 and conv.bias is None
                and conv.in_channels % 64 == 0 and conv.out_channels % 64 == 0)

    def _build(self, live, dtype):
        dev = live[0].weight.device
        total = sum(c.weight.numel() for c in live)
        self.dtype = dtype
        self.flat = torch.empty((2, total), dtype=dtype, device=dev)
        rows, off, self.entries, self.max_tiles = [], 0, {}, 1
        for c in live:
            n, k = c.out_channels, c.in_channels
            w16, w16t = self.flat[0, off:off + n * k].view(n, k), self.flat[1, off:off + n * k].view(k, n)
            rows.append([c.weight.data_ptr(), w16.data_ptr(), w16t.data_ptr(), (n << 32) | k])
            self.entries[id(c)] = (w16, w16t)
            self.max_tiles = max(self.max_tiles, (n // 64) * (k // 64))
            off += n * k
        self.table = torch.tensor(rows, dtype=torch.int64).to(dev)
        self.n = len(rows)

    def refresh(self, dtype=None):
        if dtype is None:
            dtype = torch.get_autocast_dtype("cuda") if torch.is_autocast_enabled("cuda") else torch.bfloat16
            if dtype not in (torch.bfloat16, torch.float16):
                dtype = torch.bfloat16
        elif dtype not in (torch.bfloat16, torch.float16):
            raise ValueError(f"WeightBank.refresh: dtype must be torch.bfloat16 or torch.float16, got {dtype}")
        live = [c for c in self.convs if c.weight.is_cuda and c.weight.dtype == torch.float32
                and (c.weight.is_contiguous() or c.weight.is_contiguous(memory_format=_CL))]
        if not live:
            self.entries = {}
            return self
        sig = (dtype,) + tuple((id(c), c.weight.data_ptr()) for c in live)
        capturing = torch.cuda.is_current_stream_capturing()
        if sig != self.sig:
            if capturing:
                raise L.MrlaHipError("WeightBank: first use (or moved parameters, or a change of dtype) inside a HIP graph "
                                     "capture; run one forward of the model eagerly before capturing it (in the precision of the capture)")
            self._build(live, dtype)
            self.sig, self.key = sig, None
        key = tuple(c.weight._version for c in live)
        self.captured = self.captured or capturing
        if key != self.key or self.captured or torch.is_grad_enabled():
            with torch.cuda.device(self.table.device):
                L.call("mrla_weight_bank_refresh_dt", _ptr(self.table), self.n, self.max_tiles, _DT[self.dtype], _stream())
            self.key = key
        return self

    def get(self, conv, dtype=torch.bfloat16):
        return self.entries.get(id(conv)) if dtype == self.dtype else None


class _Conv1x1Fn(torch.autograd.Function):

    @staticmethod
    @_on_device
    def forward(ctx, x, w, want_moments, passthrough=False, w16=None, w16t=None, sub=None):
        ctx.set_materialize_grads(False)
        ctx.sub = tuple(sub) if (passthrough and sub is not None) else None
        b, k, h, wd = x.shape
        n = w.shape[0]
        m = b * h * wd
        dev, st = x.device, _stream()
        ctx.wshape, ctx.wstride, ctx.wdtype = w.shape, w.stride(), w.dtype
        if w16 is not None:
            w = w16
        else:
            w = w.reshape(n, k)
            if not w.is_contiguous():
                w = w.contiguous()
        part = None
        rows = L.load().mrla_conv1x1_rows(m, k, n, _DT[x.dtype])
        if rows >= 0:
            y = torch.empty((b, n, h, wd), dtype=x.dtype, device=dev, memory_format=_CL)
            if want_moments and rows > 0:
                part = torch.empty((rows, n, L.GEMM_MOMENTS), dtype=torch.float32, device=dev)
            _call("mrla_conv1x1_fwd", (x.numel() + y.numel()) * x.element_size(), _ptr(x), _ptr(w), _ptr(y), _ptr(part), m, k,
                  n, _DT[x.dtype], st)
        else:
            y = torch.nn.functional.conv2d(x, w.view(n, k, 1, 1))
        ctx.save_for_backward(x, w, w16t)
        if part is None:
            part = torch.empty(0, device=dev)
        ctx.mark_non_differentiable(part)
        if ctx.sub is not None:
            return y, part, x[:, :, ::ctx.sub[0], ::ctx.sub[1]].contiguous(memory_format=_CL)
        if passthrough:
            return y, part, x
        return y, part

    @staticmethod
    @_on_device
    def backward(ctx, dy, _dpart=None, d_through=None):
        x, w, w16t = ctx.saved_tensors
        sub = ctx.sub
        sh, sw = sub if sub is not None else (1, 1)
        if dy is None:
            if d_through is not None and sub is not None:
                d_through = _scatter_subsample(d_through, x.shape, sh, sw, _CL)
            return (d_through if ctx.needs_input_grad[0] else None), None, None, None, None, None, None
        dy = dy.contiguous(memory_format=_CL)
        n, k = w.shape
        b, _, h, wd = x.shape
        m = b * h * wd
        lib, dt = L.load(), _DT[x.dtype]
        need_x, need_w = ctx.needs_input_grad[0], ctx.needs_input_grad[1]
        gx = gw = None
        same = dy.dtype == x.dtype and dy.data_ptr() % 16 == 0
        if d_through is not None and (d_through.dtype != x.dtype or not d_through.is_contiguous(memory_format=_CL)
                                      or d_through.data_ptr() % 16):
            d_through = d_through.to(x.dtype).contiguous(memory_format=_CL)
        if need_x and same and lib.mrla_conv1x1_rows(m, n, k, dt) >= 0:
            gx = torch.empty_like(x)
            wt = w16t if w16t is not None else w.t().contiguous()
            if d_through is not None and SHORTCUT_ADDEND and lib.mrla_conv1x1_addend_supported(m, n, k, sh, sw, dt) == 1:
                _call("mrla_conv1x1_bwd_data", (dy.numel() + gx.numel() + d_through.numel()) * x.element_size(), _ptr(dy),
                      _ptr(wt), _ptr(d_through), _ptr(gx), m, n, k, b, h, wd, sh, sw, dt, _stream(),
                      entry="mrla_conv1x1_fwd_addend")
                d_through = None
            elif d_through is not None and lib.mrla_conv1x1_add_supported(m, n, k, dt) == 1:
                if sub is not None:
                    d_through, sub = _scatter_subsample(d_through, x.shape, sh, sw, _CL), None
                _call("mrla_conv1x1_bwd_data", (dy.numel() + 2 * gx.numel()) * x.element_size(), _ptr(dy), _ptr(wt),
                      _ptr(d_through), _ptr(gx), m, n, k, dt, _stream(), entry="mrla_conv1x1_fwd_add")
                d_through = None
            else:
                _call("mrla_conv1x1_bwd_data", (dy.numel() + gx.numel()) * x.element_size(), _ptr(dy), _ptr(wt), _ptr(gx),
                      None, m, n, k, dt, _stream(), entry="mrla_conv1x1_fwd")
            need_x = False
        if need_w and same and w.dtype == x.dtype and ctx.wdtype in (x.dtype, torch.float32):
            rows = lib.mrla_conv1x1_wgrad_rows(m, k, n, dt)
            if rows > 0:
                part = torch.empty((rows, n, k), dtype=torch.float32, device=x.device)
                gw = torch.empty((n, k), dtype=ctx.wdtype, device=x.device)
                _call("mrla_conv1x1_wgrad", (dy.numel() + x.numel()) * x.element_size(), _ptr(dy), _ptr(x), _ptr(part),
                      _ptr(gw), m, k, n, dt, _DT[ctx.wdtype], _stream())
                need_w = False
        if need_x or need_w:
            gx2, gw2, _ = torch.ops.aten.convolution_backward(dy, x, w.view(n, k, 1, 1), None, (1, 1), (0, 0), (1, 1), False,
                                                              (0, 0), 1, [need_x, need_w, False])
            gx = gx2 if need_x else gx
            gw = gw2.reshape(n, k) if need_w else gw
        if d_through is not None and ctx.needs_input_grad[0]:
            if sub is not None:
                d_through = _scatter_subsample(d_through, x.shape, sh, sw, _CL)
            gx = gx + d_through
        if gw is not None:
            gw = _grad_like(gw.to(ctx.wdtype), ctx.wshape, ctx.wstride)
        return gx, gw, None, None, None, None, None


def _scatter_subsample(g, shape, sh, sw, fmt):
    dx = torch.empty(shape, dtype=g.dtype, device=g.device, memory_format=fmt).zero_()
    dx[:, :, ::sh, ::sw] = g
    return dx


class _SubsampleFn(torch.autograd.Function):

    @staticmethod
    def forward(ctx, x, sh, sw):
        ctx.shape, ctx.s = x.shape, (sh, sw)
        ctx.fmt = _CL if x.is_contiguous(memory_format=_CL) and not x.is_contiguous() else torch.contiguous_format
        return x[:, :, ::sh, ::sw].contiguous(memory_format=ctx.fmt)

    @staticmethod
    def backward(ctx, g):
        return _scatter_subsample(g, ctx.shape, ctx.s[0], ctx.s[1], ctx.fmt), None, None


def _strided_1x1(conv):
    return (type(conv) is torch.nn.Conv2d and conv.kernel_size == (1, 1) and conv.stride != (1, 1)
            and conv.padding == (0, 0) and conv.dilation == (1, 1) and conv.groups == 1 and conv.bias is None)


def conv1x1_applies(conv, x, strided=False):
    if not (type(conv) is torch.nn.Conv2d and conv.kernel_size == (1, 1) and (strided or conv.stride == (1, 1))
            and conv.padding == (0, 0) and conv.dilation == (1, 1) and conv.groups == 1 and conv.bias is None):
        return False
    if not (x.is_cuda and x.dim() == 4 and x.dtype in ((torch.bfloat16,) if strided else (torch.bfloat16, torch.float16))
            and x.is_contiguous(memory_format=_CL)
            and x.data_ptr() % 16 == 0):
        return False
    b, k, h, w = x.shape
    if k != conv.in_channels:
        return False
    if strided and strided != "pre":
        h, w = (h + conv.stride[0] - 1) // conv.stride[0], (w + conv.stride[1] - 1) // conv.stride[1]
    lib, m, n, dt = L.load(), b * h * w, conv.out_channels, _DT[x.dtype]
    if lib.mrla_conv1x1_rows(m, k, n, dt) >= 0:
        return True
    return torch.is_grad_enabled() and conv.weight.requires_grad and lib.mrla_conv1x1_wgrad_rows(m, k, n, dt) > 0


def shortcut_subsample(downsample, x):
    if not (isinstance(downsample, torch.nn.Sequential) and len(downsample) == 2 and _strided_1x1(downsample[0])):
        return None
    if not (torch.is_tensor(x) and x.dim() == 4 and conv1x1_applies(downsample[0], x, True)):
        return None
    return tuple(downsample[0].stride)


def conv_bn_act(x, conv, bn, relu, defer=False, passthrough=False, subsample=None, presampled=False):
    def second(t):
        return _SubsampleFn.apply(t, subsample[0], subsample[1]) if subsample is not None else t

    fused_bn = (type(bn) is torch.nn.BatchNorm2d and bn.affine and bn.track_running_stats)
    strided = (_strided_1x1(conv) and not passthrough and x.dim() == 4
               and conv1x1_applies(conv, x, "pre" if presampled else True))
    if strided or conv1x1_applies(conv, x):
        if strided and not presampled:
            x = _SubsampleFn.apply(x, conv.stride[0], conv.stride[1])
        wt, w16, w16t = conv.weight, None, None
        if wt.dtype != x.dtype:
            book = current_bookkeeping()
            held = book.bank.get(conv, x.dtype) if (book is not None and book.bank is not None and wt.dtype == torch.float32) else None
            if held is not None:
                w16, w16t = held
            else:
                wt = wt.to(x.dtype)
        if passthrough and torch.is_grad_enabled() and x.requires_grad:
            y, part, through = _Conv1x1Fn.apply(x, wt, bool(fused_bn and bn.training), True, w16, w16t, subsample)
            return bn_act(y, bn, relu, defer, pre_moments=part if part.numel() else None), through
        y, part = _Conv1x1Fn.apply(x, wt, bool(fused_bn and bn.training), False, w16, w16t)
        out = bn_act(y, bn, relu, defer, pre_moments=part if part.numel() else None)
        return (out, second(x)) if passthrough else out
    if presampled:
        return bn_act(torch.nn.functional.conv2d(x, conv.weight), bn, relu, defer)
    if _strided_1x1(conv) and not passthrough and x.dim() == 4 and x.is_cuda:
        xs = _SubsampleFn.apply(x, conv.stride[0], conv.stride[1])
        return bn_act(torch.nn.functional.conv2d(xs, conv.weight), bn, relu, defer)
    out = bn_act(conv(x), bn, relu, defer)
    return (out, second(x)) if passthrough else out
```

Baseline: 8424.

## Fuse BN-activation backward into 1x1 conv weight-gradient kernel

```diff
diff --git a/include/mrla_hip.h b/include/mrla_hip.h
--- a/include/mrla_hip.h
+++ b/include/mrla_hip.h
@@ -211,6 +211,11 @@
 int mrla_conv1x1_wgrad(const void* dy, const void* x, float* part, void* dw, int m, int k, int n, int dtype, int dw_dtype,
                        void* stream);
 
+int mrla_conv1x1_wgrad_bn_supported(int m, int k, int n, int dtype);
+int mrla_conv1x1_wgrad_bn(const void* g, const void* xb, const float* sc, const float* sh, const float* cb , int relu,
+                          void* dy_out, const void* x, float* part, void* dw, int m, int k, int n, int dtype, int dw_dtype,
+                          void* stream);
+
 int mrla_weight_bank_refresh(const void* table, int entries, int max_tiles, void* stream);
 int mrla_weight_bank_refresh_dt(const void* table, int entries, int max_tiles, int dtype, void* stream);
 
diff --git a/mrla_amd/_lib.py b/mrla_amd/_lib.py
--- a/mrla_amd/_lib.py
+++ b/mrla_amd/_lib.py
@@ -86,6 +86,8 @@
     "mrla_conv1x1_fwd_addend": [_P, _P, _P, _P] + [_I] * 9 + [_P],
     "mrla_conv1x1_wgrad_rows": [_I] * 4,
     "mrla_conv1x1_wgrad": [_P, _P, _P, _P, _I, _I, _I, _I, _I, _P],
+    "mrla_conv1x1_wgrad_bn_supported": [_I] * 4,
+    "mrla_conv1x1_wgrad_bn": [_P, _P, _P, _P, _P, _I, _P, _P, _P, _P, _I, _I, _I, _I, _I, _P],
     "mrla_weight_bank_refresh": [_P, _I, _I, _P],
     "mrla_weight_bank_refresh_dt": [_P, _I, _I, _I, _P],
     "mrla_reduce_rows": [_P, _P, _I, _I, _P],
diff --git a/mrla_amd/csrc/bnact_nhwc.hip b/mrla_amd/csrc/bnact_nhwc.hip
--- a/mrla_amd/csrc/bnact_nhwc.hip
+++ b/mrla_amd/csrc/bnact_nhwc.hip
@@ -1,4 +1,5 @@
 #include <algorithm>
+#include <type_traits>
 
 #include "mrla_device.h"
 #include "mrla_kernels.h"
@@ -133,6 +134,7 @@
       else {
         const float dz = (!relu || z > 0.f) ? gv[i] : 0.f;
         y[i] = fmaf(ev[i], dz, fmaf(fv[i], xv[i], hv[i]));
+        if constexpr (sizeof(T) == 2 && !std::is_same<T, bf16_t>::value) y[i] = as_f32_result(y[i]);
       }
     }
     st16<T>(out + e0, y);
@@ -265,6 +267,7 @@
       else {
         const float dz = (!relu || z > 0.f) ? gv[i] : 0.f;
         y[i] = fmaf(cbv[3 * i], dz, fmaf(cbv[3 * i + 1], xv[i], cbv[3 * i + 2]));
+        if constexpr (sizeof(T) == 2 && !std::is_same<T, bf16_t>::value) y[i] = as_f32_result(y[i]);
       }
     }
     st16<T>(out + at, y);
diff --git a/mrla_amd/csrc/capi.hip b/mrla_amd/csrc/capi.hip
--- a/mrla_amd/csrc/capi.hip
+++ b/mrla_amd/csrc/capi.hip
@@ -718,6 +718,26 @@
   return launch_conv1x1_wgrad(dy, x, part, dw, dw_dtype == MRLA_F32, m, k, n, dtype, (hipStream_t)stream);
 }
 
+int mrla_conv1x1_wgrad_bn_supported(int m, int k, int n, int dtype) {
+  if (m <= 0 || k <= 0 || n <= 0 || bad_dtype(dtype)) return MRLA_EINVAL;
+  if (dtype != MRLA_BF16 && dtype != MRLA_F16) return MRLA_EUNSUPPORTED;
+  return conv1x1_wgrad_bn_supported(m, k, n);
+}
+
+int mrla_conv1x1_wgrad_bn(const void* g, const void* xb, const float* sc, const float* sh, const float* cb, int relu,
+                          void* dy_out, const void* x, float* part, void* dw, int m, int k, int n, int dtype, int dw_dtype,
+                          void* stream) {
+  if (!g || !xb || !sc || !sh || !cb || !dy_out || !x || !part || !dw || m <= 0 || k <= 0 || n <= 0 || bad_dtype(dtype))
+    return MRLA_EINVAL;
+  if (dw_dtype != MRLA_BF16 && dw_dtype != MRLA_F16 && dw_dtype != MRLA_F32) return MRLA_EINVAL;
+  if ((dw_dtype == MRLA_F16 && dtype != MRLA_F16) || (dw_dtype == MRLA_BF16 && dtype == MRLA_F16)) return MRLA_EINVAL;
+  if (dtype != MRLA_BF16 && dtype != MRLA_F16) return MRLA_EUNSUPPORTED;
+  if (((uintptr_t)sc | (uintptr_t)sh | (uintptr_t)cb) & 15) return MRLA_EINVAL;
+  if (dy_out == g || dy_out == xb) return MRLA_EINVAL;
+  return launch_conv1x1_wgrad_bn(g, xb, sc, sh, cb, relu, dy_out, x, part, dw, dw_dtype == MRLA_F32, m, k, n, dtype,
+                                 (hipStream_t)stream);
+}
+
 int mrla_weight_bank_refresh(const void* table, int entries, int max_tiles, void* stream) {
   if (!table || entries <= 0 || max_tiles <= 0) return MRLA_EINVAL;
   return launch_weight_bank_refresh((const long long*)table, entries, max_tiles, MRLA_BF16, (hipStream_t)stream);
diff --git a/mrla_amd/csrc/conv1x1_wgrad.hip b/mrla_amd/csrc/conv1x1_wgrad.hip
--- a/mrla_amd/csrc/conv1x1_wgrad.hip
+++ b/mrla_amd/csrc/conv1x1_wgrad.hip
@@ -1,4 +1,5 @@
 #include <algorithm>
+#include <type_traits>
 
 #include "conv1x1_elem.h"
 #include "mrla_device.h"
@@ -62,13 +63,37 @@
   return (unsigned)(size_t)((__attribute__((address_space(3))) const char*)p);
 }
 
-template <typename T, int TN, int TK, int ST, int PC>
+struct WgBnArgs {
+  const void* xb;
+  const float *cb, *sc, *sh;
+  void* dy_out;
+  int relu;
+};
+
+__device__ __forceinline__ void wg_read16(u32x4& v, unsigned addr) {
+  asm volatile("ds_read_b128 %0, %1" : "=&v"(v) : "v"(addr));
+}
+template <int OFF>
+__device__ __forceinline__ void wg_read16_at(u32x4& v, unsigned addr) {
+  asm volatile("ds_read_b128 %0, %1 offset:%2" : "=&v"(v) : "v"(addr), "n"(OFF));
+}
+__device__ __forceinline__ void wg_write16(unsigned addr, const u32x4& v) {
+  asm volatile("ds_write_b128 %0, %1" ::"v"(addr), "v"(v) : "memory");
+}
+__device__ __forceinline__ void wg_fence16(u32x4& v, bool wait) {
+  if (wait) asm volatile("s_waitcnt lgkmcnt(0)" : "+v"(v) : : "memory");
+  else asm volatile("" : "+v"(v) : : "memory");
+}
+
+template <typename T, int TN, int TK, int ST, int PC, bool BN>
 __device__ __forceinline__ void conv1x1_wgrad_body(const T* __restrict__ dY, const T* __restrict__ X,
                                                    float* __restrict__ part, int M, int N, int K, int chunks_per_wg,
-                                                   int nsplits) {
+                                                   int nsplits, const WgBnArgs& bn) {
 #if defined(__HIP_DEVICE_COMPILE__)
   typedef WgGeo<TN, TK, PC> G;
   constexpr int CPRY = TN / 8, CPRX = TK / 8;
+  constexpr int SB = G::SB + (BN ? G::YB : 0);
+  static_assert(G::SB < 65536, "ds offset field");
   extern __shared__ __align__(16) unsigned char smem_raw[];
   const int lane = threadIdx.x & (kWave - 1);
   const int wave = __builtin_amdgcn_readfirstlane(threadIdx.x / kWave);
@@ -97,13 +122,17 @@
     voffX[i] = (unsigned)(((size_t)c_begin * PC + row) * K * 2 + (k0 + ((cp ^ swz<CPRX>(row)) << 3)) * 2);
   }
   const unsigned advY = (unsigned)PC * N * 2, advX = (unsigned)PC * K * 2;
+  const auto rsB = __builtin_amdgcn_make_buffer_rsrc(const_cast<void*>(BN ? bn.xb : nullptr), 0,
+                                                     BN ? (int)((size_t)M * N * 2) : 0, MRLA_WG_FLAGS);
   int issued = 0;
   auto issue = [&](int stage) {
-    unsigned char* sb = smem_raw + stage * G::SB;
+    unsigned char* sb = smem_raw + stage * SB;
     const unsigned kill = issued++ < nch ? 0u : 0x80000000u;
 #pragma unroll
     for (int i = 0; i < G::NIY; ++i) {
       __builtin_amdgcn_raw_ptr_buffer_load_lds(rsY, (lds_void_ptr)(sb + (wave + kWgWaves * i) * 1024), 16, voffY[i] | kill, 0, 0, 0);
+      if constexpr (BN)
+        __builtin_amdgcn_raw_ptr_buffer_load_lds(rsB, (lds_void_ptr)(sb + G::SB + (wave + kWgWaves * i) * 1024), 16, voffY[i] | kill, 0, 0, 0);
       voffY[i] += advY;
     }
 #pragma unroll
@@ -129,8 +158,80 @@
 #pragma unroll
       for (int e = 0; e < 16; ++e) acc[i][j][e] = 0.f;
 
-  constexpr int KSN = PC / 16, NF = 2 * (G::BN + G::BK), NI = G::NIY + G::NIX;
-  static_assert(KSN % 2 == 0 && ST >= 3, "fragment double buffer / stages");
+  float cbv[BN ? 24 : 1], scv[BN ? 8 : 1], shv[BN ? 8 : 1];
+  unsigned tbase[BN ? G::NIY : 1], toff = 0;
+  const auto rsO = __builtin_amdgcn_make_buffer_rsrc(BN ? bn.dy_out : nullptr, 0, BN ? (int)((size_t)M * N * 2) : 0,
+                                                     MRLA_WG_FLAGS);
+  const unsigned tlimit = (unsigned)((size_t)M * N * 2);
+  const unsigned skill = tk == 0 ? 0u : 0x80000000u;
+  if constexpr (BN) {
+    const int row0 = wave * (64 / CPRY) + lane / CPRY;
+    const int cch = n0 + (((lane % CPRY) ^ swz<CPRY>(row0)) << 3);
+#pragma unroll
+    for (int i = 0; i < G::NIY; ++i) tbase[i] = voffY[i];
+    const float4* c4 = reinterpret_cast<const float4*>(bn.cb + (size_t)cch * 3);
+    const float4* s4 = reinterpret_cast<const float4*>(bn.sc + cch);
+    const float4* h4 = reinterpret_cast<const float4*>(bn.sh + cch);
+#pragma unroll
+    for (int q = 0; q < 6; ++q) {
+      const float4 v = c4[q];
+      cbv[4 * q] = v.x; cbv[4 * q + 1] = v.y; cbv[4 * q + 2] = v.z; cbv[4 * q + 3] = v.w;
+    }
+#pragma unroll
+    for (int q = 0; q < 2; ++q) {
+      const float4 u = s4[q], v = h4[q];
+      scv[4 * q] = u.x; scv[4 * q + 1] = u.y; scv[4 * q + 2] = u.z; scv[4 * q + 3] = u.w;
+      shv[4 * q] = v.x; shv[4 * q + 1] = v.y; shv[4 * q + 2] = v.z; shv[4 * q + 3] = v.w;
+    }
+#pragma unroll
+    for (int q = 0; q < 24; ++q) asm volatile("" : "+v"(cbv[q]));
+#pragma unroll
+    for (int q = 0; q < 8; ++q) asm volatile("" : "+v"(scv[q]), "+v"(shv[q]));
+  }
+  const int relu = BN ? bn.relu : 0;
+  auto rewrite = [&](unsigned sbo) {
+    u32x4 gq[G::NIY], xq[G::NIY];
+    const unsigned at = lds0 + sbo + wave * 1024 + lane * 16;
+#pragma unroll
+    for (int i = 0; i < G::NIY; ++i) {
+      wg_read16(gq[i], at + i * (kWgWaves * 1024));
+      wg_read16_at<G::SB>(xq[i], at + i * (kWgWaves * 1024));
+    }
+#pragma unroll
+    for (int i = 0; i < G::NIY; ++i) {
+      wg_fence16(gq[i], i == 0);
+      wg_fence16(xq[i], false);
+    }
+#pragma unroll
+    for (int i = 0; i < G::NIY; ++i) {
+      const unsigned off = tbase[i] + toff;
+      const bool live = off < tlimit;
+      u32x4 o;
+#pragma unroll
+      for (int w = 0; w < 4; ++w) {
+        const float gv[2] = {Elem16<T>::lo(gq[i][w]), Elem16<T>::hi(gq[i][w])};
+        const float xv[2] = {Elem16<T>::lo(xq[i][w]), Elem16<T>::hi(xq[i][w])};
+        float y[2];
+#pragma unroll
+        for (int e = 0; e < 2; ++e) {
+          const int j = 2 * w + e;
+          const float z = fmaf(scv[j], xv[e], shv[j]);
+          const float dz = (!relu || z > 0.f) ? gv[e] : 0.f;
+          y[e] = fmaf(cbv[3 * j], dz, fmaf(cbv[3 * j + 1], xv[e], cbv[3 * j + 2]));
+          if constexpr (!std::is_same<T, bf16_t>::value) y[e] = as_f32_result(y[e]);
+        }
+        o[w] = live ? Elem16<T>::pack(y[0], y[1]) : 0u;
+      }
+      wg_write16(at + i * (kWgWaves * 1024), o);
+      __builtin_amdgcn_raw_buffer_store_b128(o, rsO, (live ? off : 0x80000000u) | skill, 0, 0);
+    }
+    toff += advY;
+    asm volatile("s_waitcnt lgkmcnt(0)" ::: "memory");
+  };
+
+  constexpr int KSN = PC / 16, NF = 2 * (G::BN + G::BK), NI = (BN ? 2 : 1) * G::NIY + G::NIX;
+  constexpr int W_NEXT = (ST - 3) * NI + (BN && ST > 3 ? G::NIY : 0);
+  static_assert(KSN % 2 == 0 && ST >= 3 && W_NEXT < 64 && (ST - 2) * NI < 64, "fragment double buffer / stages / vmcnt immediate");
   Frag fa[2][G::BN], fb[2][G::BK];
   auto read_step = [&](int buf, unsigned sbo, int ks) {
 #pragma unroll
@@ -148,12 +249,13 @@
 #pragma unroll
   for (int j = 0; j < ST - 1; ++j) issue(j);
   asm volatile("s_waitcnt vmcnt(%0)" ::"n"((ST - 2) * NI) : "memory");
+  if constexpr (BN) rewrite(0);
   __builtin_amdgcn_s_barrier();
   asm volatile("" ::: "memory");
   read_step(0, 0, 0);
   int stage = 0, nxt = ST - 1;
   for (int c = 0; c < nch; ++c) {
-    const unsigned sbo = stage * G::SB;
+    const unsigned sbo = stage * SB;
     stage = stage + 1 == ST ? 0 : stage + 1;
 #pragma unroll
     for (int ks = 0; ks < KSN; ++ks) {
@@ -162,12 +264,13 @@
       if (ks + 1 < KSN) {
         read_step(cur ^ 1, sbo, ks + 1);
       } else if (c + 1 < nch) {
-        asm volatile("s_waitcnt vmcnt(%0)" ::"n"((ST - 3) * NI) : "memory");
+        asm volatile("s_waitcnt vmcnt(%0)" ::"n"(W_NEXT) : "memory");
+        if constexpr (BN) rewrite(stage * SB);
         __builtin_amdgcn_s_barrier();
         asm volatile("" ::: "memory");
         issue(nxt);
         nxt = nxt + 1 == ST ? 0 : nxt + 1;
-        read_step(0, stage * G::SB, 0);
+        read_step(0, stage * SB, 0);
       } else {
         pending = 0;
       }
@@ -198,14 +301,29 @@
                                                                         const bf16_t* __restrict__ X,
                                                                         float* __restrict__ part, int M, int N, int K,
                                                                         int chunks_per_wg, int nsplits) {
-  conv1x1_wgrad_body<bf16_t, TN, TK, ST, PC>(dY, X, part, M, N, K, chunks_per_wg, nsplits);
+  conv1x1_wgrad_body<bf16_t, TN, TK, ST, PC, false>(dY, X, part, M, N, K, chunks_per_wg, nsplits, WgBnArgs{});
 }
 template <int TN, int TK, int ST, int PC>
 __global__ __launch_bounds__(kWgWaves* kWave) void conv1x1_wgrad_f16_kernel(const f16_t* __restrict__ dY,
                                                                             const f16_t* __restrict__ X,
                                                                             float* __restrict__ part, int M, int N, int K,
                                                                             int chunks_per_wg, int nsplits) {
-  conv1x1_wgrad_body<f16_t, TN, TK, ST, PC>(dY, X, part, M, N, K, chunks_per_wg, nsplits);
+  conv1x1_wgrad_body<f16_t, TN, TK, ST, PC, false>(dY, X, part, M, N, K, chunks_per_wg, nsplits, WgBnArgs{});
+}
+template <int TN, int TK, int ST, int PC>
+__global__ __launch_bounds__(kWgWaves* kWave) void conv1x1_wgrad_bn_kernel(const bf16_t* __restrict__ g,
+                                                                           const bf16_t* __restrict__ X,
+                                                                           float* __restrict__ part, int M, int N, int K,
+                                                                           int chunks_per_wg, int nsplits, WgBnArgs bn) {
+  conv1x1_wgrad_body<bf16_t, TN, TK, ST, PC, true>(g, X, part, M, N, K, chunks_per_wg, nsplits, bn);
+}
+template <int TN, int TK, int ST, int PC>
+__global__ __launch_bounds__(kWgWaves* kWave) void conv1x1_wgrad_bn_f16_kernel(const f16_t* __restrict__ g,
+                                                                               const f16_t* __restrict__ X,
+                                                                               float* __restrict__ part, int M, int N,
+                                                                               int K, int chunks_per_wg, int nsplits,
+                                                                               WgBnArgs bn) {
+  conv1x1_wgrad_body<f16_t, TN, TK, ST, PC, true>(g, X, part, M, N, K, chunks_per_wg, nsplits, bn);
 }
 
 template <typename TO>
@@ -269,10 +387,25 @@
 }
 
 template <int TN, int TK, int ST, int PC>
-int launch_tile(const WgPlan& p, const void* dy, const void* x, float* part, int M, int K, int N, int dtype, hipStream_t st) {
+int launch_tile(const WgPlan& p, const void* dy, const void* x, float* part, int M, int K, int N, int dtype, hipStream_t st,
+                const WgBnArgs* bn = nullptr) {
   typedef WgGeo<TN, TK, PC> G;
+  const dim3 grid((p.tiles * p.splits + 7) / 8 * 8), block(kWgWaves * kWave);
+  if (bn) {
+    const size_t lds = (size_t)ST * (G::SB + G::YB);
+    static_assert((size_t)ST * (G::SB + G::YB) <= 160 * 1024, "LDS of a CU");
+    if (dtype == MRLA_F16) {
+      if (lds_opt_in(reinterpret_cast<const void*>(conv1x1_wgrad_bn_f16_kernel<TN, TK, ST, PC>), lds) != hipSuccess) return MRLA_EHIP;
+      hipLaunchKernelGGL((conv1x1_wgrad_bn_f16_kernel<TN, TK, ST, PC>), grid, block, lds, st, (const f16_t*)dy, (const f16_t*)x,
+                         part, M, N, K, p.chunks_per_wg, p.splits, *bn);
+    } else {
+      if (lds_opt_in(reinterpret_cast<const void*>(conv1x1_wgrad_bn_kernel<TN, TK, ST, PC>), lds) != hipSuccess) return MRLA_EHIP;
+      hipLaunchKernelGGL((conv1x1_wgrad_bn_kernel<TN, TK, ST, PC>), grid, block, lds, st, (const bf16_t*)dy, (const bf16_t*)x,
+                         part, M, N, K, p.chunks_per_wg, p.splits, *bn);
+    }
+    return MRLA_OK;
+  }
   const size_t lds = (size_t)ST * G::SB;
-  const dim3 grid((p.tiles * p.splits + 7) / 8 * 8), block(kWgWaves * kWave);
   if (dtype == MRLA_F16) {
     if (lds_opt_in(reinterpret_cast<const void*>(conv1x1_wgrad_f16_kernel<TN, TK, ST, PC>), lds) != hipSuccess) return MRLA_EHIP;
     hipLaunchKernelGGL((conv1x1_wgrad_f16_kernel<TN, TK, ST, PC>), grid, block, lds, st, (const f16_t*)dy, (const f16_t*)x, part,
@@ -299,13 +432,20 @@
   return MRLA_OK;
 }
 
-int launch_conv1x1_wgrad(const void* dy, const void* x, float* part, void* dw, int dw_f32, int M, int K, int N, int dtype,
-                         hipStream_t st) {
+int conv1x1_wgrad_bn_supported(int M, int K, int N) {
+  const WgPlan p = wgrad_plan(M, K, N);
+  if (!p.tiles) return MRLA_EUNSUPPORTED;
+  const int ktiles = K / p.tk;
+  return ktiles == 1 || (ktiles == 2 && N <= 512) ? 1 : MRLA_EUNSUPPORTED;
+}
+
+static int launch_wgrad(const void* dy, const void* x, float* part, void* dw, int dw_f32, int M, int K, int N, int dtype,
+                        hipStream_t st, const WgBnArgs* bn) {
   const WgPlan p = wgrad_plan(M, K, N);
   if (!p.tiles || (dtype != MRLA_BF16 && dtype != MRLA_F16)) return MRLA_EUNSUPPORTED;
   int rc = MRLA_EUNSUPPORTED;
 #define MRLA_WG_TILE(A, B) \
-  if (p.tn == A && p.tk == B) rc = launch_tile<A, B, kWgStages, kPC>(p, dy, x, part, M, K, N, dtype, st);
+  if (p.tn == A && p.tk == B) rc = launch_tile<A, B, kWgStages, kPC>(p, dy, x, part, M, K, N, dtype, st, bn);
   MRLA_WG_TILE(64, 64) MRLA_WG_TILE(64, 128) MRLA_WG_TILE(64, 256) MRLA_WG_TILE(128, 64) MRLA_WG_TILE(128, 128)
   MRLA_WG_TILE(128, 256) MRLA_WG_TILE(256, 64) MRLA_WG_TILE(256, 128)
 #undef MRLA_WG_TILE
@@ -320,4 +460,17 @@
   return hip_status(hipGetLastError());
 }
 
-}
+int launch_conv1x1_wgrad(const void* dy, const void* x, float* part, void* dw, int dw_f32, int M, int K, int N, int dtype,
+                         hipStream_t st) {
+  return launch_wgrad(dy, x, part, dw, dw_f32, M, K, N, dtype, st, nullptr);
+}
+
+int launch_conv1x1_wgrad_bn(const void* g, const void* xb, const float* sc, const float* sh, const float* cb, int relu,
+                            void* dy_out, const void* x, float* part, void* dw, int dw_f32, int M, int K, int N, int dtype,
+                            hipStream_t st) {
+  if (conv1x1_wgrad_bn_supported(M, K, N) != 1) return MRLA_EUNSUPPORTED;
+  const WgBnArgs bn{xb, cb, sc, sh, dy_out, relu};
+  return launch_wgrad(g, x, part, dw, dw_f32, M, K, N, dtype, st, &bn);
+}
+
+}
diff --git a/mrla_amd/csrc/mrla_device.h b/mrla_amd/csrc/mrla_device.h
--- a/mrla_amd/csrc/mrla_device.h
+++ b/mrla_amd/csrc/mrla_device.h
@@ -37,6 +37,10 @@
   a[M_SO] += n * d_o;
 }
 
+__device__ __forceinline__ float as_f32_result(float v) {
+  asm("" : "+v"(v));
+  return v;
+}
 template <typename T> __device__ __forceinline__ float to_f(T v) { return static_cast<float>(v); }
 template <typename T> __device__ __forceinline__ T from_f(float v) { return static_cast<T>(v); }
 
diff --git a/mrla_amd/csrc/mrla_kernels.h b/mrla_amd/csrc/mrla_kernels.h
--- a/mrla_amd/csrc/mrla_kernels.h
+++ b/mrla_amd/csrc/mrla_kernels.h
@@ -183,6 +183,10 @@
 int conv1x1_wgrad_plan(int M, int K, int N, int* out);
 int launch_conv1x1_wgrad(const void* dy, const void* x, float* part, void* dw, int dw_f32, int M, int K, int N, int dtype,
                          hipStream_t st);
+int conv1x1_wgrad_bn_supported(int M, int K, int N);
+int launch_conv1x1_wgrad_bn(const void* g, const void* xb, const float* sc, const float* sh, const float* cb, int relu,
+                            void* dy_out, const void* x, float* part, void* dw, int dw_f32, int M, int K, int N, int dtype,
+                            hipStream_t st);
 int launch_weight_bank_refresh(const long long* table, int entries, int max_tiles, int dtype, hipStream_t st);
 int launch_light_stats_fwd_wide(const void* x, const void* o, const float* wv, float* mom, void* xout, const float* psc,
                                 const float* psh, void* vout, int B, int C, int H, int W, int dtype, int act,
diff --git a/mrla_amd/csrc/sequences.hip b/mrla_amd/csrc/sequences.hip
--- a/mrla_amd/csrc/sequences.hip
+++ b/mrla_amd/csrc/sequences.hip
@@ -99,6 +99,7 @@
     MRLA_TRY(mrla_bn_plane_dmoments(dy, x, bnbuf, bnbuf + C, bnbuf + 2 * C, relu, tmom, b, c, h, w, dtype, layout, stream));
   MRLA_TRY(mrla_bn_stats_bwd(tmom, gamma, bnbuf + 2 * C, bnbuf + 3 * C, bn_mode, 1, small, small + 3 * C, small + 4 * C, rows,
                              c, (int)((long)b * h * w / rows), stream));
+  if (!dx) return MRLA_OK;
   return mrla_bn_act_bwd(dy, x, bnbuf, bnbuf + C, small, relu, dx, b, c, h, w, dtype, layout, stream);
 }
 
diff --git a/mrla_amd/functional.py b/mrla_amd/functional.py
--- a/mrla_amd/functional.py
+++ b/mrla_amd/functional.py
@@ -42,6 +42,9 @@
 
 
 SHORTCUT_ADDEND = True
+
+
+WGRAD_BN = True
 
 
 def _seq():
@@ -1365,6 +1368,119 @@
         return _scatter_subsample(g, ctx.shape, ctx.s[0], ctx.s[1], ctx.fmt), None, None
 
 
+class _SubCtx:
+
+    def __init__(self):
+        self.saved_tensors, self.needs_input_grad = (), ()
+
+    def set_materialize_grads(self, flag):
+        pass
+
+    def save_for_backward(self, *tensors):
+        self.saved_tensors = tensors
+
+    def mark_non_differentiable(self, *tensors):
+        pass
+
+
+class _ConvBnFn(torch.autograd.Function):
+
+    @staticmethod
+    @_on_device
+    def forward(ctx, x, w, gamma, beta, running_mean, running_var, training, momentum, eps, relu, defer, box, passthrough,
+                w16, w16t, sub):
+        ctx.set_materialize_grads(False)
+        ca, cb = _SubCtx(), _SubCtx()
+        res = _Conv1x1Fn.apply(x, w, bool(training), passthrough, w16, w16t, sub)
+        n, k = w.shape[0], x.shape[1]
+        ca.sub = tuple(sub) if (passthrough and sub is not None) else None
+        ca.wshape, ca.wstride, ca.wdtype = w.shape, w.stride(), w.dtype
+        ca.saved_tensors = (x, w16 if w16 is not None else w.reshape(n, k).contiguous(), w16t)
+        y, part = res[0], res[1]
+        out = _BnActFn.forward(cb, y, gamma, beta, running_mean, running_var, training, momentum, eps, relu, defer,
+                               part if part.numel() else None, box)
+        ctx.save_for_backward(*ca.saved_tensors, *cb.saved_tensors)
+        ca.saved_tensors = cb.saved_tensors = ()
+        ctx.ca, ctx.cb, ctx.defer, ctx.nthrough = ca, cb, bool(defer), len(res) - 2
+        if defer:
+            ctx.mark_non_differentiable(out[1])
+            return (y, out[1]) + tuple(res[2:])
+        return (out,) + tuple(res[2:]) if len(res) > 2 else out
+
+    @staticmethod
+    @_on_device
+    def backward(ctx, dy, *rest):
+        saved = ctx.saved_tensors
+        ca, cb = ctx.ca, ctx.cb
+        ca.saved_tensors, cb.saved_tensors = saved[:3], saved[3:]
+        try:
+            return _ConvBnFn._backward(ctx, dy, rest, saved)
+        finally:
+            ca.saved_tensors = cb.saved_tensors = ()
+
+    @staticmethod
+    def _backward(ctx, dy, rest, saved):
+        d_through = rest[-1] if ctx.nthrough else None
+        ca, cb = ctx.ca, ctx.cb
+        ca.needs_input_grad = (ctx.needs_input_grad[0], ctx.needs_input_grad[1])
+        x, w, _ = saved[:3]
+        y, gamma32, bnbuf = saved[3:]
+        tail = (None,) * 12
+        if dy is None:
+            gx = _Conv1x1Fn.backward(ca, None, None, d_through)[0]
+            return (gx, None, None, None) + tail
+        n, k = w.shape
+        b, _, h, wd = x.shape
+        m = b * h * wd
+        lib, dt = L.load(), _DT[x.dtype]
+        g = dy if dy.is_contiguous(memory_format=_CL) else None
+        fused = (WGRAD_BN and TIMER is None and ctx.needs_input_grad[1] and g is not None and g.dtype == y.dtype
+                 and g.data_ptr() % 16 == 0 and cb.layout == L.NHWC and w.dtype == x.dtype
+                 and ca.wdtype in (x.dtype, torch.float32) and lib.mrla_conv1x1_wgrad_bn_supported(m, k, n, dt) == 1)
+        if not fused:
+            dyc, dgamma, dbeta = _BnActFn.backward(cb, dy)[:3]
+            gx, gw = _Conv1x1Fn.backward(ca, dyc, None, d_through)[:2]
+            return (gx, gw, dgamma, dbeta) + tail
+        dev, st = x.device, _stream()
+        rows = cb.rows
+        handed = cb.box.take(g) if cb.box is not None else None
+        if handed is not None:
+            tmom, rows = handed
+        else:
+            tmom = torch.empty((rows, n, 2), dtype=torch.float32, device=dev)
+        small = torch.empty((5, n), dtype=torch.float32, device=dev)
+        mode = L.BN_TRAIN if cb.training else L.BN_EVAL
+        if SEQUENCES:
+            _seq_call("mrla_bn_bwd", _ptr(g), _ptr(y), _ptr(gamma32), _ptr(bnbuf), _ptr(tmom), rows, int(handed is not None),
+                      mode, cb.relu, _ptr(small), None, b, n, h, wd, dt, L.NHWC, st)
+        else:
+            if handed is None:
+                L.call("mrla_bn_plane_dmoments", _ptr(g), _ptr(y), _ptr(bnbuf[0]), _ptr(bnbuf[1]), _ptr(bnbuf[2]), cb.relu,
+                       _ptr(tmom), b, n, h, wd, dt, L.NHWC, st)
+            L.call("mrla_bn_stats_bwd", _ptr(tmom), _ptr(gamma32), _ptr(bnbuf[2]), _ptr(bnbuf[3]), mode, 1, _ptr(small),
+                   _ptr(small[3]), _ptr(small[4]), rows, n, m // rows, st)
+        prow = lib.mrla_conv1x1_wgrad_rows(m, k, n, dt)
+        part = torch.empty((prow, n, k), dtype=torch.float32, device=dev)
+        gw = torch.empty((n, k), dtype=ca.wdtype, device=dev)
+        dyc = torch.empty_like(y)
+        L.call("mrla_conv1x1_wgrad_bn", _ptr(g), _ptr(y), _ptr(bnbuf[0]), _ptr(bnbuf[1]), _ptr(small), cb.relu, _ptr(dyc),
+               _ptr(x), _ptr(part), _ptr(gw), m, k, n, dt, _DT[ca.wdtype], st)
+        ca.needs_input_grad = (ctx.needs_input_grad[0], False)
+        gx = _Conv1x1Fn.backward(ca, dyc, None, d_through)[0]
+        gw = _grad_like(gw, ca.wshape, ca.wstride)
+        return (gx, gw, small[3].to(cb.gdtype), small[4].to(cb.gdtype)) + tail
+
+
+def _conv_bn_fused(conv, bn, x, fused_bn):
+    if not (WGRAD_BN and TIMER is None and fused_bn and torch.is_grad_enabled() and conv.weight.requires_grad):
+        return False
+    if x.dtype != torch.bfloat16:
+        return False
+    b, k, h, w = x.shape
+    lib, m, n, dt = L.load(), b * h * w, conv.out_channels, _DT[x.dtype]
+    return lib.mrla_conv1x1_rows(m, k, n, dt) >= 0 and lib.mrla_conv1x1_wgrad_bn_supported(m, k, n, dt) == 1
+
+
 def _strided_1x1(conv):
     return (type(conv) is torch.nn.Conv2d and conv.kernel_size == (1, 1) and conv.stride != (1, 1)
             and conv.padding == (0, 0) and conv.dilation == (1, 1) and conv.groups == 1 and conv.bias is None)
@@ -1415,6 +1531,21 @@
                 w16, w16t = held
             else:
                 wt = wt.to(x.dtype)
+        if _conv_bn_fused(conv, bn, x, fused_bn):
+            training = bn.training
+            momentum = bump_batch_counter(bn) if training else bn.momentum
+            box = _DeferredBnBox() if defer else None
+            through = passthrough and x.requires_grad
+            res = _ConvBnFn.apply(x, wt, bn.weight, bn.bias, bn.running_mean, bn.running_var, training, momentum or 0.0,
+                                  bn.eps, relu, defer, box, through, w16, w16t, subsample if through else None)
+            res = res if isinstance(res, tuple) else (res,)
+            out = res[0]
+            if defer:
+                out._mrla_affine = (res[1][0], res[1][1])
+                out._mrla_bn_box = box
+            if not passthrough:
+                return out
+            return out, (res[-1] if through else second(x))
         if passthrough and torch.is_grad_enabled() and x.requires_grad:
             y, part, through = _Conv1x1Fn.apply(x, wt, bool(fused_bn and bn.training), True, w16, w16t, subsample)
             return bn_act(y, bn, relu, defer, pre_moments=part if part.numel() else None), through
```

Result: faster. 8579, median of 6 (+1.8%).
